# PaddlePaddle/Paddle

Hardware: AMD Instinct MI355X
Metric: tokens/sec (whole node) GPT-3-6.7B Fleet sharding-3 (higher is better)
Workload: dtype bf16; 1 GPU; model=gpt3-6.7b, global_batch=12, seq_len=2048, parallelism=sharding3_dp1

## Files before the change

csrc/bindings.cpp:

```cpp
#include <torch/extension.h>
#include <c10/hip/HIPStream.h>

#include "kernels/api.h"

namespace pa {
void mfma_probe(const void* a, const void* bt, float* c, hipStream_t s);
void mfma_probe32(const void* a, const void* bt, float* c, hipStream_t s);
void mfma_probe_fp8mx(const void* a, const void* bt, float* c, int sa, int sb,
                      hipStream_t s);
}

namespace pa_lt {
std::tuple<torch::Tensor, torch::Tensor> fc1_gelu_fwd(
    const torch::Tensor& x, const torch::Tensor& w, const torch::Tensor& bias);
std::tuple<torch::Tensor, torch::Tensor> fc2_dgrad_dgelu(
    const torch::Tensor& dy, const torch::Tensor& w2, const torch::Tensor& z);
int64_t lt_epilogue_probe(int64_t m, int64_t n, int64_t k, int64_t epi);
}

namespace {

using torch::Tensor;

hipStream_t cur_stream() {
  return (hipStream_t)c10::hip::getCurrentHIPStream().stream();
}

int dt_of(const Tensor& t) {
  switch (t.scalar_type()) {
    case torch::kBFloat16: return pa::kBF16;
    case torch::kFloat: return pa::kF32;
    default: TORCH_CHECK(false, "unsupported dtype ", t.scalar_type(),
                         " (native kernels take bfloat16 or float32)");
  }
  return -1;
}

#define CHECK_IN(t) \
  TORCH_CHECK(t.is_cuda() && t.is_contiguous(), #t " must be contiguous GPU tensor")

#define CHECK_LIKE(t, x)                                                      \
  TORCH_CHECK(t.is_cuda() && t.is_contiguous() &&                             \
              t.scalar_type() == x.scalar_type(),                             \
              #t " must be a contiguous GPU tensor with the dtype of " #x)
#define CHECK_SAME(t, x)                                                      \
  do { CHECK_LIKE(t, x);                                                      \
       TORCH_CHECK(t.numel() == x.numel(), #t " must have the size of " #x);  \
  } while (0)
#define CHECK_VEC(t, x, d)                                                    \
  do { CHECK_LIKE(t, x);                                                      \
       TORCH_CHECK(t.numel() == (d), #t " must have ", (d), " elements");     \
  } while (0)
#define CHECK_STAT(t, n)                                                      \
  TORCH_CHECK(t.is_cuda() && t.is_contiguous() &&                             \
              t.scalar_type() == torch::kFloat && t.numel() == (n),           \
              #t " must be a contiguous fp32 GPU tensor with ", (n), " elements")

static void check_rows(const Tensor& x, const char* op) {
  TORCH_CHECK(x.dim() >= 1 && x.numel() > 0, op, ": empty input");
  TORCH_CHECK(x.size(-1) % 8 == 0, op, ": D must be a multiple of 8");
}

std::vector<Tensor> layer_norm_fwd(const Tensor& x, const Tensor& w,
                                   const c10::optional<Tensor>& b, double eps) {
  CHECK_IN(x);
  check_rows(x, "layer_norm");
  int64_t d = x.size(-1), n = x.numel() / d;
  CHECK_VEC(w, x, d);
  if (b.has_value()) CHECK_VEC((*b), x, d);
  auto y = torch::empty_like(x);
  auto mean = torch::empty({n}, x.options().dtype(torch::kFloat));
  auto rstd = torch::empty({n}, x.options().dtype(torch::kFloat));
  pa::layer_norm_fwd(x.const_data_ptr(), w.const_data_ptr(),
                     b.has_value() ? b->const_data_ptr() : nullptr,
                     y.mutable_data_ptr(), mean.mutable_data_ptr<float>(),
                     rstd.mutable_data_ptr<float>(), n, d, (float)eps, dt_of(x),
                     cur_stream());
  return {y, mean, rstd};
}

std::vector<Tensor> layer_norm_bwd(const Tensor& dy, const Tensor& x,
                                   const Tensor& w, const Tensor& mean,
                                   const Tensor& rstd, bool has_bias) {
  CHECK_IN(x);
  check_rows(x, "layer_norm_bwd");
  int64_t d = x.size(-1), n = x.numel() / d;
  CHECK_SAME(dy, x); CHECK_VEC(w, x, d);
  CHECK_STAT(mean, n); CHECK_STAT(rstd, n);
  auto dx = torch::empty_like(x);
  auto dw = torch::zeros({d}, x.options().dtype(torch::kFloat));
  auto db = torch::zeros({d}, x.options().dtype(torch::kFloat));
  pa::layer_norm_bwd_dx(dy.const_data_ptr(), x.const_data_ptr(), w.const_data_ptr(),
                        mean.const_data_ptr<float>(), rstd.const_data_ptr<float>(),
                        dx.mutable_data_ptr(), n, d, dt_of(x), cur_stream());
  auto ws = torch::empty({(int64_t)2 * pa::ln_dwdb_chunks(n, d) * d},
                         x.options().dtype(torch::kFloat));
  pa::layer_norm_bwd_dwdb(dy.const_data_ptr(), x.const_data_ptr(),
                          mean.const_data_ptr<float>(), rstd.const_data_ptr<float>(),
                          dw.mutable_data_ptr<float>(), db.mutable_data_ptr<float>(),
                          n, d, dt_of(x), cur_stream(), ws.mutable_data_ptr<float>());
  return {dx, dw, db};
}

std::vector<Tensor> rms_norm_fwd(const Tensor& x, const c10::optional<Tensor>& residual,
                                 const Tensor& w, double eps) {
  CHECK_IN(x);
  check_rows(x, "rms_norm");
  int64_t d = x.size(-1), n = x.numel() / d;
  CHECK_VEC(w, x, d);
  auto y = torch::empty_like(x);
  auto rstd = torch::empty({n}, x.options().dtype(torch::kFloat));
  Tensor res_out;
  const void* resp = nullptr;
  void* res_outp = nullptr;
  if (residual.has_value()) {
    CHECK_SAME((*residual), x);
    res_out = torch::empty_like(x);
    resp = residual->const_data_ptr();
    res_outp = res_out.mutable_data_ptr();
  }
  pa::rms_norm_fwd(x.const_data_ptr(), resp, w.const_data_ptr(),
                   y.mutable_data_ptr(), res_outp, rstd.mutable_data_ptr<float>(),
                   n, d, (float)eps, dt_of(x), cur_stream());
  if (residual.has_value()) return {y, rstd, res_out};
  return {y, rstd};
}

std::vector<Tensor> rms_norm_bwd(const Tensor& dy, const Tensor& x, const Tensor& w,
                                 const Tensor& rstd) {
  CHECK_IN(x);
  check_rows(x, "rms_norm_bwd");
  int64_t d = x.size(-1), n = x.numel() / d;
  CHECK_SAME(dy, x); CHECK_VEC(w, x, d); CHECK_STAT(rstd, n);
  auto dx = torch::empty_like(x);
  auto dw = torch::zeros({d}, x.options().dtype(torch::kFloat));
  pa::rms_norm_bwd_dx(dy.const_data_ptr(), x.const_data_ptr(), w.const_data_ptr(),
                      rstd.const_data_ptr<float>(), dx.mutable_data_ptr(), n, d,
                      dt_of(x), cur_stream());
  auto ws = torch::empty({(int64_t)2 * pa::ln_dwdb_chunks(n, d) * d},
                         x.options().dtype(torch::kFloat));
  pa::rms_norm_bwd_dw(dy.const_data_ptr(), x.const_data_ptr(),
                      rstd.const_data_ptr<float>(), dw.mutable_data_ptr<float>(),
                      n, d, dt_of(x), cur_stream(), ws.mutable_data_ptr<float>());
  return {dx, dw};
}

std::vector<Tensor> softmax_ce_fwd(const Tensor& logits, const Tensor& labels,
                                   int64_t ignore_index) {
  CHECK_IN(logits); CHECK_IN(labels);
  TORCH_CHECK(logits.dim() >= 1 && logits.numel() > 0, "softmax_ce: empty logits");
  int64_t v = logits.size(-1), n = logits.numel() / v;
  TORCH_CHECK(labels.scalar_type() == torch::kLong && labels.numel() == n,
              "softmax_ce: labels must be int64 with one entry per row");
  auto loss = torch::empty({n}, logits.options().dtype(torch::kFloat));
  auto lse = torch::empty({n}, logits.options().dtype(torch::kFloat));
  pa::softmax_ce_fwd(logits.const_data_ptr(), labels.const_data_ptr<int64_t>(),
                     loss.mutable_data_ptr<float>(), lse.mutable_data_ptr<float>(),
                     n, v, ignore_index, dt_of(logits), cur_stream());
  return {loss, lse};
}

Tensor softmax_ce_bwd(const Tensor& dloss, const Tensor& logits,
                      const Tensor& labels, const Tensor& lse, int64_t ignore_index) {
  CHECK_IN(logits); CHECK_IN(labels);
  TORCH_CHECK(logits.dim() >= 1 && logits.numel() > 0, "softmax_ce_bwd: empty logits");
  int64_t v = logits.size(-1), n = logits.numel() / v;
  TORCH_CHECK(labels.scalar_type() == torch::kLong && labels.numel() == n,
              "softmax_ce_bwd: labels must be int64 with one entry per row");
  CHECK_STAT(dloss, n); CHECK_STAT(lse, n);
  auto dlogits = torch::empty_like(logits);
  pa::softmax_ce_bwd(dloss.const_data_ptr<float>(), logits.const_data_ptr(),
                     labels.const_data_ptr<int64_t>(), lse.const_data_ptr<float>(),
                     dlogits.mutable_data_ptr(), n, v, ignore_index, dt_of(logits),
                     cur_stream());
  return dlogits;
}

Tensor bias_gelu_fwd(const Tensor& x, const c10::optional<Tensor>& bias) {
  CHECK_IN(x);
  check_rows(x, "bias_gelu");
  int64_t d = x.size(-1), n = x.numel() / d;
  if (bias.has_value()) CHECK_VEC((*bias), x, d);
  auto y = torch::empty_like(x);
  pa::bias_gelu_fwd(x.const_data_ptr(), bias.has_value() ? bias->const_data_ptr() : nullptr,
                    y.mutable_data_ptr(), n, d, dt_of(x), cur_stream());
  return y;
}

Tensor bias_gelu_bwd(const Tensor& dy, const Tensor& x, const c10::optional<Tensor>& bias) {
  CHECK_IN(x);
  check_rows(x, "bias_gelu_bwd");
  int64_t d = x.size(-1), n = x.numel() / d;
  CHECK_SAME(dy, x);
  if (bias.has_value()) CHECK_VEC((*bias), x, d);
  auto dx = torch::empty_like(x);
  pa::bias_gelu_bwd(dy.const_data_ptr(), x.const_data_ptr(),
                    bias.has_value() ? bias->const_data_ptr() : nullptr,
                    dx.mutable_data_ptr(), n, d, dt_of(x), cur_stream());
  return dx;
}

Tensor swiglu_fwd(const Tensor& x) {
  CHECK_IN(x);
  TORCH_CHECK(x.dim() >= 1 && x.numel() > 0, "swiglu: empty input");
  int64_t d2 = x.size(-1), n = x.numel() / d2, d = d2 / 2;
  TORCH_CHECK(d2 % 16 == 0, "swiglu: last dim must be a multiple of 16");
  auto sizes = x.sizes().vec();
  sizes.back() = d;
  auto y = torch::empty(sizes, x.options());
  pa::swiglu_fwd(x.const_data_ptr(), y.mutable_data_ptr(), n, d, dt_of(x), cur_stream());
  return y;
}

Tensor swiglu_bwd(const Tensor& dy, const Tensor& x) {
  CHECK_IN(x);
  TORCH_CHECK(x.dim() >= 1 && x.numel() > 0, "swiglu_bwd: empty input");
  int64_t d2 = x.size(-1), n = x.numel() / d2, d = d2 / 2;
  TORCH_CHECK(d2 % 16 == 0, "swiglu_bwd: last dim must be a multiple of 16");
  CHECK_LIKE(dy, x);
  TORCH_CHECK(dy.numel() == n * d, "swiglu_bwd: dy must have half the size of x");
  auto dx = torch::empty_like(x);
  pa::swiglu_bwd(dy.const_data_ptr(), x.const_data_ptr(), dx.mutable_data_ptr(),
                 n, d, dt_of(x), cur_stream());
  return dx;
}

Tensor rope_fwd(const Tensor& x, const Tensor& cos_t, const Tensor& sin_t,
                int64_t pos_offset, bool conj) {
  CHECK_IN(x); CHECK_IN(cos_t); CHECK_IN(sin_t);
  TORCH_CHECK(x.dim() == 4, "rope expects [B,S,H,D]");
  int64_t b = x.size(0), sl = x.size(1), h = x.size(2), dh = x.size(3);
  TORCH_CHECK(dh % 2 == 0 && (dh / 2) % 4 == 0 && x.numel() > 0,
              "rope: head_dim/2 must be multiple of 4");
  TORCH_CHECK(pos_offset >= 0, "rope: pos_offset must be >= 0");
  TORCH_CHECK(cos_t.scalar_type() == torch::kFloat &&
              sin_t.scalar_type() == torch::kFloat &&
              cos_t.dim() == 2 && sin_t.dim() == 2 &&
              cos_t.size(1) == dh / 2 && sin_t.size(1) == dh / 2 &&
              cos_t.size(0) >= sl + pos_offset && sin_t.size(0) >= sl + pos_offset,
              "rope: cos/sin must be fp32 [>= seq_len + pos_offset, head_dim/2]");
  auto y = torch::empty_like(x);
  pa::rope_fwd(x.const_data_ptr(), cos_t.const_data_ptr<float>(),
               sin_t.const_data_ptr<float>(), y.mutable_data_ptr(), b, sl, h, dh,
               pos_offset, conj, dt_of(x), cur_stream());
  return y;
}

Tensor colsum(const Tensor& x) {
  CHECK_IN(x);
  TORCH_CHECK(x.dim() >= 1 && x.numel() > 0, "colsum: empty input");
  int64_t d = x.size(-1), n = x.numel() / d;
  auto out = torch::zeros({d}, x.options().dtype(torch::kFloat));
  pa::colsum(x.const_data_ptr(), out.mutable_data_ptr<float>(), n, d, dt_of(x),
             cur_stream());
  return out;
}

Tensor weight_only_gemv(const Tensor& x, const Tensor& qweight,
                        const Tensor& scale, const c10::optional<Tensor>& bias) {
  CHECK_IN(x); CHECK_IN(qweight); CHECK_IN(scale);
  TORCH_CHECK(qweight.scalar_type() == torch::kChar, "qweight must be int8");
  int64_t k = x.size(-1), m = x.numel() / k, n = qweight.size(0);
  TORCH_CHECK(qweight.size(1) == k && k % 8 == 0);
  auto sizes = x.sizes().vec();
  sizes.back() = n;
  auto out = torch::empty(sizes, x.options());
  const void* bp = bias.has_value() ? bias->const_data_ptr() : nullptr;
  pa::weight_only_gemv(x.const_data_ptr(), qweight.const_data_ptr(),
                       scale.const_data_ptr<float>(), bp,
                       out.mutable_data_ptr(), m, n, k, dt_of(x), cur_stream());
  return out;
}

void adamw(Tensor& master, c10::optional<Tensor> param_out, const Tensor& grad,
           Tensor& m, Tensor& v, double lr, double beta1, double beta2,
           double eps, double wd, double beta1_pow, double beta2_pow,
           double grad_scale) {
  CHECK_IN(master); CHECK_IN(grad); CHECK_IN(m); CHECK_IN(v);
  int64_t numel = master.numel();
  TORCH_CHECK(master.scalar_type() == torch::kFloat &&
              m.scalar_type() == torch::kFloat && v.scalar_type() == torch::kFloat,
              "adamw: master, m and v must be fp32");
  TORCH_CHECK(grad.numel() == numel && m.numel() == numel && v.numel() == numel,
              "adamw: grad, m and v must have the size of master");
  bool bf16out = false;
  void* pout = nullptr;
  if (param_out.has_value()) {
    TORCH_CHECK(param_out->is_cuda() && param_out->is_contiguous() &&
                param_out->numel() == numel &&
                (param_out->scalar_type() == torch::kBFloat16 ||
                 param_out->scalar_type() == torch::kFloat),
                "adamw: param_out must be a contiguous bf16 or fp32 GPU tensor "
                "with the size of master");
    bf16out = param_out->scalar_type() == torch::kBFloat16;
    pout = param_out->mutable_data_ptr();
  }
  pa::adamw(master.mutable_data_ptr<float>(), pout, grad.const_data_ptr(),
            m.mutable_data_ptr<float>(), v.mutable_data_ptr<float>(), numel,
            (float)lr, (float)beta1, (float)beta2, (float)eps, (float)wd,
            (float)beta1_pow, (float)beta2_pow, (float)grad_scale,
            dt_of(grad), bf16out, cur_stream());
}

Tensor l2norm_sq(const Tensor& x) {
  CHECK_IN(x);
  auto out = torch::zeros({1}, x.options().dtype(torch::kFloat));
  pa::l2norm_sq(x.const_data_ptr(), out.mutable_data_ptr<float>(), x.numel(),
                dt_of(x), cur_stream());
  return out;
}

static void fa_strides(const Tensor& t, int64_t* out) {
  TORCH_CHECK(t.stride(3) == 1, "flash_attn: head_dim must be contiguous");
  out[0] = t.stride(0);
  out[1] = t.stride(1);
  out[2] = t.stride(2);
  TORCH_CHECK(out[2] % 8 == 0, "flash_attn: seq stride must keep 16B alignment");
}

static void fa_mask_strides(const Tensor& m, int64_t b, int64_t h, int64_t sq,
                            int64_t skv, int64_t* ms) {
  TORCH_CHECK(m.dim() == 4 && m.size(3) == skv && m.size(2) == sq &&
              (m.size(1) == 1 || m.size(1) == h) &&
              (m.size(0) == 1 || m.size(0) == b),
              "flash_attn mask must be [B|1, H|1, Sq, Skv]");
  TORCH_CHECK(m.stride(3) == 1 && m.scalar_type() == torch::kBFloat16,
              "flash_attn mask: bf16 with contiguous last dim");
  ms[0] = m.size(0) == 1 ? 0 : m.stride(0);
  ms[1] = m.size(1) == 1 ? 0 : m.stride(1);
  ms[2] = m.stride(2);
}

std::vector<Tensor> flash_attn_fwd(const Tensor& q, const Tensor& k, const Tensor& v,
                                   c10::optional<Tensor> o_out,
                                   double scale, bool causal,
                                   c10::optional<Tensor> mask,
                                   double pdrop, int64_t seed, int64_t offset) {
  TORCH_CHECK(q.is_cuda() && q.scalar_type() == torch::kBFloat16, "flash_attn: bf16 GPU only");
  TORCH_CHECK(q.dim() == 4, "flash_attn expects [B,H,S,D]");
  int64_t b = q.size(0), h = q.size(1), sq = q.size(2), d = q.size(3);
  int64_t hkv = k.size(1), skv = k.size(2);
  TORCH_CHECK(d == 128 || d == 64, "flash_attn: head_dim must be 64/128");
  TORCH_CHECK(h % hkv == 0);
  int64_t qs[3], ks[3], vs[3], os[3];
  fa_strides(q, qs); fa_strides(k, ks); fa_strides(v, vs);
  TORCH_CHECK(ks[0] == vs[0] && ks[1] == vs[1] && ks[2] == vs[2],
              "flash_attn: k/v must share strides");
  auto o = o_out.has_value() ? *o_out : torch::empty({b, h, sq, d}, q.options());
  fa_strides(o, os);
  auto lse = torch::empty({b, h, sq}, q.options().dtype(torch::kFloat));
  int64_t ms[3] = {0, 0, 0};
  const void* mp = nullptr;
  if (mask.has_value()) {
    fa_mask_strides(*mask, b, h, sq, skv, ms);
    mp = mask->const_data_ptr();
  }
  pa::flash_attn_fwd32(q.const_data_ptr(), k.const_data_ptr(), v.const_data_ptr(),
                       o.mutable_data_ptr(), lse.mutable_data_ptr<float>(), b, h,
                       hkv, sq, skv, d, (float)scale, causal, qs, ks, os,
                       mp, ms, (float)pdrop, (uint64_t)seed, (uint64_t)offset,
                       cur_stream());
  return {o, lse};
}

std::vector<Tensor> flash_attn_bwd(const Tensor& dout, const Tensor& q, const Tensor& k,
                                   const Tensor& v, const Tensor& o, const Tensor& lse,
                                   c10::optional<Tensor> dq_out,
                                   c10::optional<Tensor> dk_out,
                                   c10::optional<Tensor> dv_out,
                                   double scale, bool causal,
                                   c10::optional<Tensor> mask,
                                   double pdrop, int64_t seed, int64_t offset) {
  int64_t b = q.size(0), h = q.size(1), sq = q.size(2), d = q.size(3);
  int64_t hkv = k.size(1), skv = k.size(2);
  TORCH_CHECK(hkv == h, "flash_attn_bwd kernel requires hkv==h (expand KV upstream)");
  auto dq = dq_out.has_value() ? *dq_out : torch::empty({b, h, sq, d}, q.options());
  auto dk = dk_out.has_value() ? *dk_out : torch::empty({b, hkv, skv, d}, k.options());
  auto dv = dv_out.has_value() ? *dv_out : torch::empty({b, hkv, skv, d}, v.options());
  auto delta = torch::empty({b, h, sq}, q.options().dtype(torch::kFloat));
  int64_t qs[3], ks[3], vs[3], dos[3], os[3], dqs[3], dks[3], dvs[3];
  fa_strides(q, qs); fa_strides(k, ks); fa_strides(v, vs);
  fa_strides(dout, dos); fa_strides(o, os);
  fa_strides(dq, dqs); fa_strides(dk, dks); fa_strides(dv, dvs);
  TORCH_CHECK(ks[0] == vs[0] && ks[1] == vs[1] && ks[2] == vs[2]);
  TORCH_CHECK(dks[0] == dvs[0] && dks[1] == dvs[1] && dks[2] == dvs[2],
              "dk/dv must share strides");
  int64_t ms[3] = {0, 0, 0};
  const void* mp = nullptr;
  if (mask.has_value()) {
    fa_mask_strides(*mask, b, h, sq, skv, ms);
    mp = mask->const_data_ptr();
  }
  pa::flash_attn_bwd(dout.const_data_ptr(), q.const_data_ptr(), k.const_data_ptr(),
                     v.const_data_ptr(), o.const_data_ptr(), lse.const_data_ptr<float>(),
                     dq.mutable_data_ptr(), dk.mutable_data_ptr(), dv.mutable_data_ptr(),
                     delta.mutable_data_ptr<float>(), b, h, hkv, sq, skv, d,
                     (float)scale, causal, qs, ks, dos, os, dqs, dks,
                     mp, ms, (float)pdrop, (uint64_t)seed, (uint64_t)offset,
                     cur_stream());
  return {dq, dk, dv};
}

static std::pair<Tensor, int64_t> make_bmap(const Tensor& cu_cpu, int64_t blk) {
  auto acc = cu_cpu.accessor<int, 1>();
  std::vector<int> map;
  for (int64_t i = 0; i + 1 < cu_cpu.size(0); ++i) {
    int len = acc[i + 1] - acc[i];
    for (int off = 0; off < len; off += (int)blk) {
      map.push_back((int)i);
      map.push_back(off);
    }
  }
  auto t = torch::from_blob(map.data(), {(int64_t)map.size()},
                            torch::dtype(torch::kInt32)).clone().cuda();
  return {t, (int64_t)map.size() / 2};
}

std::vector<Tensor> flash_attn_varlen_fwd(const Tensor& q, const Tensor& k,
                                          const Tensor& v, const Tensor& cu_q,
                                          const Tensor& cu_k, double scale,
                                          bool causal, double pdrop,
                                          int64_t seed, int64_t offset) {
  TORCH_CHECK(q.is_cuda() && q.scalar_type() == torch::kBFloat16 &&
              q.dim() == 3 && q.is_contiguous(), "varlen q: [total, H, D] bf16");
  TORCH_CHECK(cu_q.scalar_type() == torch::kInt32 && cu_k.scalar_type() == torch::kInt32);
  int64_t tq = q.size(0), h = q.size(1), d = q.size(2);
  int64_t tk = k.size(0), hkv = k.size(1);
  TORCH_CHECK(d == 128 || d == 64);
  auto cu_q_cpu = cu_q.cpu().contiguous();
  auto cu_k_cpu = cu_k.cpu().contiguous();
  auto cu_q_gpu = cu_q.is_cuda() ? cu_q.contiguous() : cu_q_cpu.cuda();
  auto cu_k_gpu = cu_k.is_cuda() ? cu_k.contiguous() : cu_k_cpu.cuda();
  auto [bmap, nblk] = make_bmap(cu_q_cpu, 128);
  auto o = torch::empty_like(q);
  auto lse = torch::empty({h, tq}, q.options().dtype(torch::kFloat));
  pa::flash_attn_varlen_fwd32(q.const_data_ptr(), k.const_data_ptr(),
                              v.const_data_ptr(), o.mutable_data_ptr(),
                              lse.mutable_data_ptr<float>(), h, hkv, tq, tk, d,
                              (float)scale, causal, nblk,
                              cu_q_gpu.const_data_ptr<int>(),
                              cu_k_gpu.const_data_ptr<int>(),
                              bmap.const_data_ptr<int>(), (float)pdrop,
                              (uint64_t)seed, (uint64_t)offset, cur_stream());
  return {o, lse};
}

std::vector<Tensor> flash_attn_varlen_bwd(const Tensor& dout, const Tensor& q,
                                          const Tensor& k, const Tensor& v,
                                          const Tensor& o, const Tensor& lse,
                                          const Tensor& cu_q, const Tensor& cu_k,
                                          double scale, bool causal,
                                          double pdrop, int64_t seed,
                                          int64_t offset) {
  int64_t tq = q.size(0), h = q.size(1), d = q.size(2);
  int64_t tk = k.size(0);
  TORCH_CHECK(k.size(1) == h, "varlen bwd requires hkv == h");
  auto cu_q_cpu = cu_q.cpu().contiguous();
  auto cu_k_cpu = cu_k.cpu().contiguous();
  auto cu_q_gpu = cu_q.is_cuda() ? cu_q.contiguous() : cu_q_cpu.cuda();
  auto cu_k_gpu = cu_k.is_cuda() ? cu_k.contiguous() : cu_k_cpu.cuda();
  auto [qbmap, nqb] = make_bmap(cu_q_cpu, 128);
  auto [kvbmap, nkb] = make_bmap(cu_k_cpu, 128);
  auto dq = torch::empty_like(q);
  auto dk = torch::empty_like(k);
  auto dv = torch::empty_like(v);
  auto delta = torch::empty({h, tq}, q.options().dtype(torch::kFloat));
  pa::flash_attn_varlen_bwd(dout.contiguous().const_data_ptr(), q.const_data_ptr(),
                            k.const_data_ptr(), v.const_data_ptr(),
                            o.const_data_ptr(), lse.const_data_ptr<float>(),
                            dq.mutable_data_ptr(), dk.mutable_data_ptr(),
                            dv.mutable_data_ptr(), delta.mutable_data_ptr<float>(),
                            h, tq, tk, d, (float)scale, causal, nqb, nkb,
                            cu_q_gpu.const_data_ptr<int>(),
                            cu_k_gpu.const_data_ptr<int>(),
                            qbmap.const_data_ptr<int>(),
                            kvbmap.const_data_ptr<int>(), (float)pdrop,
                            (uint64_t)seed, (uint64_t)offset, cur_stream());
  return {dq, dk, dv};
}

Tensor fa_dropout_mask(int64_t b, int64_t h, int64_t sq, int64_t skv,
                       double p, int64_t seed, int64_t offset) {
  auto out = torch::empty({b, h, sq, skv},
                          torch::dtype(torch::kUInt8).device(torch::kCUDA));
  pa::fa_dropout_mask(out.mutable_data_ptr(), out.numel(), (float)p,
                      (uint64_t)seed, (uint64_t)offset, cur_stream());
  return out;
}

std::vector<Tensor> dropout_add_fwd(const Tensor& x, const c10::optional<Tensor>& residual,
                                    double p, int64_t seed, int64_t offset) {
  CHECK_IN(x);
  TORCH_CHECK(x.numel() > 0 && x.numel() % 8 == 0,
              "dropout_add: numel must be a multiple of 8");
  TORCH_CHECK(p >= 0.0 && p < 1.0, "dropout_add: p must be in [0, 1)");
  if (residual.has_value()) CHECK_SAME((*residual), x);
  auto y = torch::empty_like(x);
  Tensor mask;
  uint8_t* maskp = nullptr;
  if (p > 0) {
    mask = torch::empty(x.sizes(), x.options().dtype(torch::kUInt8));
    maskp = mask.mutable_data_ptr<uint8_t>();
  }
  pa::dropout_add_fwd(x.const_data_ptr(),
                      residual.has_value() ? residual->const_data_ptr() : nullptr,
                      y.mutable_data_ptr(), maskp, x.numel(), (float)p,
                      (uint64_t)seed, (uint64_t)offset, dt_of(x), cur_stream());
  if (p > 0) return {y, mask};
  return {y};
}

Tensor dropout_add_bwd(const Tensor& dy, const Tensor& mask, double p) {
  CHECK_IN(dy); CHECK_IN(mask);
  TORCH_CHECK(dy.numel() > 0 && dy.numel() % 8 == 0,
              "dropout_add_bwd: numel must be a multiple of 8");
  TORCH_CHECK(mask.scalar_type() == torch::kUInt8 && mask.numel() == dy.numel(),
              "dropout_add_bwd: mask must be uint8 with the size of dy");
  TORCH_CHECK(p >= 0.0 && p < 1.0, "dropout_add_bwd: p must be in [0, 1)");
  auto dx = torch::empty_like(dy);
  pa::dropout_add_bwd(dy.const_data_ptr(), mask.const_data_ptr<uint8_t>(),
                      dx.mutable_data_ptr(), dy.numel(), (float)p, dt_of(dy),
                      cur_stream());
  return dx;
}

Tensor embedding_fwd(const Tensor& table, const Tensor& ids_in, int64_t padding_idx) {
  CHECK_IN(table);
  TORCH_CHECK(ids_in.is_cuda(), "ids must be on GPU");
  TORCH_CHECK(ids_in.scalar_type() == torch::kLong, "embedding: ids must be int64");
  TORCH_CHECK(table.dim() == 2 && table.numel() > 0, "embedding: table must be [vocab, D]");
  auto ids = ids_in.contiguous();
  int64_t vocab = table.size(0), d = table.size(1), n = ids.numel();
  TORCH_CHECK(d % 8 == 0, "embedding: D must be a multiple of 8");
  auto sizes = ids.sizes().vec();
  sizes.push_back(d);
  auto out = torch::empty(sizes, table.options());
  pa::embedding_fwd(table.const_data_ptr(), ids.const_data_ptr<int64_t>(),
                    out.mutable_data_ptr(), n, d, vocab, padding_idx,
                    dt_of(table), cur_stream());
  return out;
}

Tensor embedding_bwd(const Tensor& dout, const Tensor& ids_in, int64_t vocab,
                     int64_t padding_idx) {
  CHECK_IN(dout);
  TORCH_CHECK(ids_in.is_cuda(), "ids must be on GPU");
  TORCH_CHECK(ids_in.scalar_type() == torch::kLong, "embedding_bwd: ids must be int64");
  auto ids = ids_in.contiguous();
  TORCH_CHECK(dout.dim() >= 1 && dout.numel() > 0 && vocab > 0, "embedding_bwd: empty input");
  int64_t d = dout.size(-1), n = ids.numel();
  TORCH_CHECK(d % 8 == 0, "embedding_bwd: D must be a multiple of 8");
  TORCH_CHECK(dout.numel() == n * d, "embedding_bwd: dout must be [ids..., D]");
  auto dtable = torch::zeros({vocab, d}, dout.options().dtype(torch::kFloat));
  pa::embedding_bwd(dout.const_data_ptr(), ids.const_data_ptr<int64_t>(),
                    dtable.mutable_data_ptr<float>(), n, d, vocab, padding_idx,
                    dt_of(dout), cur_stream());
  return dtable;
}

Tensor decode_attention(const Tensor& q, const Tensor& kcache, const Tensor& vcache,
                        const Tensor& block_table, const Tensor& seq_lens,
                        double scale, int64_t blk_str, int64_t pos_str,
                        int64_t head_str, int64_t bs_override) {
  CHECK_IN(q); CHECK_IN(kcache); CHECK_IN(vcache);
  TORCH_CHECK(q.dim() == 3, "q: [B, H, D] (one decode step)");
  int64_t b = q.size(0), h = q.size(1), d = q.size(2);
  int64_t bs, hkv;
  if (blk_str == 0) {
    TORCH_CHECK(kcache.dim() == 4, "k_cache: [nblocks, block_size, HKV, D]");
    bs = kcache.size(1); hkv = kcache.size(2);
  } else {
    bs = bs_override; hkv = bs_override >= 0 ? h : h;
    hkv = kcache.size(1) == h ? h : kcache.size(1);
  }
  int64_t max_blocks = block_table.size(1);
  auto o = torch::empty_like(q);
  pa::decode_attention(q.const_data_ptr(), kcache.const_data_ptr(),
                       vcache.const_data_ptr(),
                       block_table.const_data_ptr<int>(),
                       seq_lens.const_data_ptr<int>(), o.mutable_data_ptr(),
                       b, h, hkv, bs, max_blocks, d, (float)scale,
                       blk_str, pos_str, head_str, cur_stream());
  return o;
}

Tensor gemm_bf16(const Tensor& a, const Tensor& b, bool b_is_nt) {
  TORCH_CHECK(a.is_cuda() && a.scalar_type() == torch::kBFloat16);
  TORCH_CHECK(a.dim() == 2 && b.dim() == 2);
  TORCH_CHECK(a.stride(1) == 1 && b.stride(1) == 1, "row-major inputs only");
  int64_t m = a.size(0), k = a.size(1);
  int64_t n = b_is_nt ? b.size(0) : b.size(1);
  TORCH_CHECK(b_is_nt ? b.size(1) == k : b.size(0) == k);
  TORCH_CHECK(k % 64 == 0 && k >= 128, "gemm_bf16: K must be multiple of 64");
  auto c = torch::empty({m, n}, a.options());
  pa::gemm_bf16(a.const_data_ptr(), b.const_data_ptr(), c.mutable_data_ptr(),
                m, n, k, a.stride(0), b.stride(0), c.stride(0), b_is_nt,
                cur_stream());
  return c;
}

std::vector<Tensor> gemm_bf16_ex(const Tensor& a, const Tensor& b,
                                 int64_t layout, int64_t epilogue,
                                 const c10::optional<Tensor>& bias,
                                 const c10::optional<Tensor>& aux_in,
                                 const c10::optional<Tensor>& c_in) {
  TORCH_CHECK(a.is_cuda() && a.scalar_type() == torch::kBFloat16);
  TORCH_CHECK(b.is_cuda() && b.scalar_type() == torch::kBFloat16);
  TORCH_CHECK(a.dim() == 2 && b.dim() == 2);
  TORCH_CHECK(a.stride(1) == 1 && b.stride(1) == 1, "row-major inputs only");
  int64_t m, n, k;
  if (layout == 0) {
    m = a.size(0); k = a.size(1); n = b.size(0);
    TORCH_CHECK(b.size(1) == k, "gemm NT: inner dims mismatch");
  } else if (layout == 1) {
    m = a.size(0); k = a.size(1); n = b.size(1);
    TORCH_CHECK(b.size(0) == k, "gemm NN: inner dims mismatch");
  } else {
    k = a.size(0); m = a.size(1); n = b.size(1);
    TORCH_CHECK(b.size(0) == k, "gemm TN: inner dims mismatch");
  }
  TORCH_CHECK(k >= 64, "gemm_bf16_ex: K must be >= 64");
  bool accumulate = c_in.has_value();
  Tensor c;
  if (accumulate) {
    c = c_in.value();
    TORCH_CHECK(c.size(0) == m && c.size(1) == n && c.stride(1) == 1 &&
                c.scalar_type() == torch::kBFloat16);
    TORCH_CHECK(epilogue == 0, "accumulate requires epilogue=none");
  } else {
    c = torch::empty({m, n}, a.options());
  }
  const void* bias_p = nullptr;
  if (epilogue == 1 || epilogue == 2) {
    TORCH_CHECK(bias.has_value() && bias->numel() == n &&
                bias->scalar_type() == torch::kBFloat16 && bias->is_contiguous());
    bias_p = bias->const_data_ptr();
  }
  Tensor aux;
  void* aux_p = nullptr;
  if (epilogue == 2) {
    aux = torch::empty({m, n}, a.options());
    aux_p = aux.mutable_data_ptr();
  } else if (epilogue == 3) {
    TORCH_CHECK(aux_in.has_value() && aux_in->size(0) == m &&
                aux_in->size(1) == n && aux_in->stride(1) == 1 &&
                aux_in->scalar_type() == torch::kBFloat16);
    aux_p = const_cast<void*>(aux_in->const_data_ptr());
  }
  pa::gemm_bf16_ex(a.const_data_ptr(), b.const_data_ptr(), c.mutable_data_ptr(),
                   bias_p, aux_p, m, n, k, a.stride(0), b.stride(0), c.stride(0),
                   (int)layout, (int)epilogue, accumulate, cur_stream());
  if (epilogue == 2) return {c, aux};
  return {c};
}

Tensor gemm_fp8_nt(const Tensor& a, const Tensor& bt, double scale_ab,
                   const c10::optional<Tensor>& bias) {
  TORCH_CHECK(a.is_cuda() && a.dim() == 2 && bt.dim() == 2);
  TORCH_CHECK(a.scalar_type() == torch::kFloat8_e4m3fn ||
              a.scalar_type() == torch::kUInt8, "gemm_fp8: e4m3/uint8 input");
  TORCH_CHECK(a.stride(1) == 1 && bt.stride(1) == 1, "row-major inputs");
  int64_t m = a.size(0), k = a.size(1), n = bt.size(0);
  TORCH_CHECK(bt.size(1) == k && k >= 128);
  auto c = torch::empty({m, n}, a.options().dtype(torch::kBFloat16));
  const void* bp = nullptr;
  if (bias.has_value()) {
    TORCH_CHECK(bias->scalar_type() == torch::kBFloat16 && bias->numel() == n);
    bp = bias->const_data_ptr();
  }
  pa::gemm_fp8_nt(a.const_data_ptr(), bt.const_data_ptr(), c.mutable_data_ptr(),
                  bp, (float)scale_ab, m, n, k, a.stride(0), bt.stride(0),
                  c.stride(0), cur_stream());
  return c;
}

Tensor decode_gemm(const Tensor& x, const Tensor& w,
                   const c10::optional<Tensor>& bias) {
  CHECK_IN(x);
  TORCH_CHECK(x.dim() == 2 && w.dim() == 2 && w.stride(1) == 1);
  TORCH_CHECK(x.scalar_type() == torch::kBFloat16);
  int64_t m = x.size(0), k = x.size(1), n = w.size(1);
  TORCH_CHECK(w.size(0) == k && m <= 32);
  int64_t ntiles = (n + 1023) / 1024;
  int64_t ksplit = std::min<int64_t>(std::max<int64_t>(1, 768 / std::max<int64_t>(ntiles, 1)),
                                     std::max<int64_t>(1, k / 128));
  int64_t mt = m <= 8 ? 8 : (m <= 16 ? 16 : 32);
  auto ws = torch::empty({ksplit, mt, n}, x.options().dtype(torch::kFloat));
  auto y = torch::empty({m, n}, x.options());
  pa::decode_gemm(x.const_data_ptr(), w.const_data_ptr(),
                  bias.has_value() ? bias->const_data_ptr() : nullptr,
                  y.mutable_data_ptr(), ws.mutable_data_ptr<float>(), m, n, k,
                  w.stride(0), ksplit, cur_stream());
  return y;
}

Tensor decode_gemm_int8(const Tensor& x, const Tensor& qw,
                        const Tensor& scale,
                        const c10::optional<Tensor>& bias) {
  CHECK_IN(x);
  TORCH_CHECK(x.dim() == 2 && qw.dim() == 2 && qw.is_contiguous());
  TORCH_CHECK(x.scalar_type() == torch::kBFloat16 &&
              qw.scalar_type() == torch::kChar &&
              scale.scalar_type() == torch::kFloat);
  int64_t m = x.size(0), k = x.size(1), n = qw.size(1);
  TORCH_CHECK(qw.size(0) == k && m <= 32 && n % 256 == 0 && k % 64 == 0);
  TORCH_CHECK(scale.numel() == n);
  int64_t nblk = n / 256;
  int64_t kmin = nblk <= 24 ? 256 : 512;
  int64_t ksplit = std::min<int64_t>(std::max<int64_t>(1, 1024 / nblk),
                                     std::max<int64_t>(1, k / kmin));
  int64_t mt = m <= 16 ? 16 : 32;
  auto ws = torch::empty({ksplit, mt, n}, x.options().dtype(torch::kFloat));
  auto y = torch::empty({m, n}, x.options());
  pa::decode_gemm_mfma(x.const_data_ptr(), qw.const_data_ptr(),
                       bias.has_value() ? bias->const_data_ptr() : nullptr,
                       y.mutable_data_ptr(), ws.mutable_data_ptr<float>(), m,
                       n, k, n, ksplit, cur_stream(),
                       scale.const_data_ptr<float>(), true);
  return y;
}

static int64_t check_int4_weight(const Tensor& qw, const Tensor& scale,
                                 int64_t group_size, const char* op) {
  TORCH_CHECK(qw.is_cuda() && scale.is_cuda(), op, ": qw and scale must be GPU tensors");
  TORCH_CHECK(qw.dim() == 2 && qw.is_contiguous(), op,
              ": qw must be a contiguous [K/2, N] tensor");
  TORCH_CHECK(qw.scalar_type() == torch::kChar, op, ": qw must be int8");
  TORCH_CHECK(scale.scalar_type() == torch::kFloat && scale.is_contiguous(),
              op, ": scale must be contiguous fp32");
  TORCH_CHECK(group_size == -1 || group_size == 64 || group_size == 128, op,
              ": group_size must be -1, 64 or 128, got ", group_size);
  const int64_t k = qw.size(0) * 2, n = qw.size(1);
  if (group_size == -1) {
    TORCH_CHECK(scale.dim() == 1 && scale.size(0) == n, op,
                ": per-channel scale must be [N]");
  } else {
    TORCH_CHECK(k % group_size == 0, op, ": K must be a multiple of group_size");
    TORCH_CHECK(scale.dim() == 2 && scale.size(0) == k / group_size &&
                scale.size(1) == n, op, ": group scale must be [K/group_size, N]");
  }
  return k;
}

Tensor decode_gemm_int4(const Tensor& x, const Tensor& qw, const Tensor& scale,
                        const c10::optional<Tensor>& bias, int64_t group_size,
                        int64_t ksplit) {
  CHECK_IN(x);
  TORCH_CHECK(x.dim() == 2 && x.scalar_type() == torch::kBFloat16,
              "decode_gemm_int4: x must be a 2-D bf16 tensor");
  const int64_t k = check_int4_weight(qw, scale, group_size, "decode_gemm_int4");
  const int64_t m = x.size(0), n = qw.size(1);
  TORCH_CHECK(x.size(1) == k, "decode_gemm_int4: qw.size(0)*2 must equal K");
  TORCH_CHECK(m >= 1 && m <= 32, "decode_gemm_int4: 1 <= M <= 32, got ", m);
  TORCH_CHECK(n > 0 && n % 256 == 0, "decode_gemm_int4: N % 256 == 0, got ", n);
  TORCH_CHECK(k > 0 && k % 64 == 0 && k <= (int64_t(1) << 24),
              "decode_gemm_int4: K % 64 == 0 (and K <= 2^24), got ", k);
  TORCH_CHECK(ksplit >= 0, "decode_gemm_int4: ksplit >= 0");
  const void* bp = nullptr;
  if (bias.has_value()) {
    TORCH_CHECK(bias->is_cuda() && bias->is_contiguous() &&
                bias->scalar_type() == torch::kBFloat16 && bias->numel() == n,
                "decode_gemm_int4: bias must be contiguous bf16 with N elements");
    bp = bias->const_data_ptr();
  }
  if (ksplit == 0) {
    const int64_t nblk = n / 256;
    const int64_t kmin = nblk <= 24 ? 256 : 512;
    ksplit = std::min<int64_t>(std::max<int64_t>(1, 1024 / nblk),
                               std::max<int64_t>(1, k / kmin));
  }
  const int64_t ks = pa::decode_gemm_int4_splits(k, ksplit);
  const int64_t mt = m <= 16 ? 16 : 32;
  auto ws = torch::empty({ks, mt, n}, x.options().dtype(torch::kFloat));
  auto y = torch::empty({m, n}, x.options());
  pa::decode_gemm_int4(x.const_data_ptr(), qw.const_data_ptr(),
                       scale.const_data_ptr<float>(), bp, y.mutable_data_ptr(),
                       ws.mutable_data_ptr<float>(), m, n, k, group_size,
                       ksplit, cur_stream());
  return y;
}

Tensor dequant_int4(const Tensor& qw, const Tensor& scale, int64_t group_size,
                    at::ScalarType out_dtype) {
  const int64_t k = check_int4_weight(qw, scale, group_size, "dequant_int4");
  const int64_t n = qw.size(1);
  TORCH_CHECK(n % 8 == 0, "dequant_int4: N % 8 == 0, got ", n);
  TORCH_CHECK(out_dtype == torch::kBFloat16 || out_dtype == torch::kFloat,
              "dequant_int4: out_dtype must be bfloat16 or float32");
  auto out = torch::empty({k, n}, qw.options().dtype(out_dtype));
  pa::dequant_int4(qw.const_data_ptr(), scale.const_data_ptr<float>(),
                   out.mutable_data_ptr(), k, n, group_size,
                   out_dtype == torch::kBFloat16 ? pa::kBF16 : pa::kF32,
                   cur_stream());
  return out;
}

Tensor decode_gemm_mfma(const Tensor& x, const Tensor& w,
                        const c10::optional<Tensor>& bias) {
  CHECK_IN(x);
  TORCH_CHECK(x.dim() == 2 && w.dim() == 2 && w.stride(1) == 1);
  TORCH_CHECK(x.scalar_type() == torch::kBFloat16);
  int64_t m = x.size(0), k = x.size(1), n = w.size(1);
  TORCH_CHECK(w.size(0) == k && m <= 32 && n % 256 == 0 && k % 64 == 0);
  int64_t nblk = n / 256;
  int64_t kmin = nblk <= 24 ? 256 : 512;
  int64_t ksplit = std::min<int64_t>(std::max<int64_t>(1, 1024 / nblk),
                                     std::max<int64_t>(1, k / kmin));
  int64_t mt = m <= 16 ? 16 : 32;
  auto ws = torch::empty({ksplit, mt, n}, x.options().dtype(torch::kFloat));
  auto y = torch::empty({m, n}, x.options());
  pa::decode_gemm_mfma(x.const_data_ptr(), w.const_data_ptr(),
                       bias.has_value() ? bias->const_data_ptr() : nullptr,
                       y.mutable_data_ptr(), ws.mutable_data_ptr<float>(), m,
                       n, k, w.stride(0), ksplit, cur_stream());
  return y;
}

std::vector<Tensor> moe_gate_topk(const Tensor& logits, int64_t k) {
  CHECK_IN(logits);
  TORCH_CHECK(logits.scalar_type() == torch::kFloat && logits.dim() == 2);
  int64_t t = logits.size(0), e = logits.size(1);
  TORCH_CHECK(e <= 64 && k <= 4);
  auto topv = torch::empty({t, k}, logits.options());
  auto topi = torch::empty({t, k}, logits.options().dtype(torch::kInt32));
  auto me = torch::zeros({e}, logits.options());
  auto ce = torch::zeros({e}, logits.options());
  pa::moe_gate_topk(logits.const_data_ptr<float>(), topv.mutable_data_ptr<float>(),
                    topi.mutable_data_ptr<int>(), me.mutable_data_ptr<float>(),
                    ce.mutable_data_ptr<float>(), t, e, k, cur_stream());
  return {topv, topi, me, ce};
}

std::vector<Tensor> moe_assign_slots(const Tensor& topi, int64_t num_experts,
                                     int64_t cap) {
  CHECK_IN(topi);
  TORCH_CHECK(topi.scalar_type() == torch::kInt32 && topi.dim() == 2);
  int64_t t = topi.size(0), k = topi.size(1);
  auto slot = torch::full({t, k}, -1, topi.options());
  auto counts = torch::zeros({num_experts}, topi.options());
  pa::moe_assign_slots(topi.const_data_ptr<int>(), slot.mutable_data_ptr<int>(),
                       counts.mutable_data_ptr<int>(), t, num_experts, k, cap,
                       cur_stream());
  return {slot, counts};
}

Tensor gemm_fp8_nt_batched(const Tensor& a, const Tensor& bt, double scale_ab,
                           const c10::optional<Tensor>& bias) {
  TORCH_CHECK(a.is_cuda() && a.dim() == 3 && bt.dim() == 3);
  TORCH_CHECK(a.is_contiguous() && bt.is_contiguous());
  int64_t e = a.size(0), m = a.size(1), k = a.size(2), n = bt.size(1);
  TORCH_CHECK(bt.size(0) == e && bt.size(2) == k && k >= 128);
  const void* bp = nullptr;
  int64_t bias_bs = 0;
  if (bias.has_value()) {
    TORCH_CHECK(bias->is_contiguous() && bias->scalar_type() == torch::kBFloat16);
    TORCH_CHECK(bias->dim() == 2 && bias->size(0) == e && bias->size(1) == n);
    bp = bias->const_data_ptr();
    bias_bs = n;
  }
  auto c = torch::empty({e, m, n}, a.options().dtype(torch::kBFloat16));
  pa::gemm_fp8_nt_batched(a.const_data_ptr(), bt.const_data_ptr(),
                          c.mutable_data_ptr(), bp, (float)scale_ab, e,
                          m, n, k, k, k, n, m * k, n * k, m * n, cur_stream(),
                          bias_bs);
  return c;
}

Tensor amax_abs(const Tensor& x) {
  CHECK_IN(x);
  auto out = torch::zeros({}, x.options().dtype(torch::kFloat));
  pa::amax_abs(x.const_data_ptr(), out.mutable_data_ptr<float>(), x.numel(),
               dt_of(x), cur_stream());
  return out;
}

Tensor gemm_bf16_8p_t(const Tensor& a, const Tensor& bt) {
  TORCH_CHECK(a.is_cuda() && a.dim() == 2 && bt.dim() == 2);
  TORCH_CHECK(a.is_contiguous() && bt.is_contiguous());
  int64_t m = a.size(0), k = a.size(1), n = bt.size(0);
  TORCH_CHECK(bt.size(1) == k && m % 256 == 0 && n % 256 == 0 && k % 32 == 0);
  auto c = torch::empty({m, n}, a.options());
  pa::gemm_bf16_8p(a.const_data_ptr(), bt.const_data_ptr(),
                   c.mutable_data_ptr(), m, n, k, k, k, n, cur_stream());
  return c;
}

Tensor gemm_bf16_nt_batched_t(const Tensor& a, const Tensor& bt) {
  TORCH_CHECK(a.is_cuda() && a.dim() == 3 && bt.dim() == 3);
  TORCH_CHECK(a.scalar_type() == torch::kBFloat16 &&
              bt.scalar_type() == torch::kBFloat16);
  TORCH_CHECK(a.is_contiguous() && bt.is_contiguous());
  int64_t e = a.size(0), m = a.size(1), k = a.size(2), n = bt.size(1);
  TORCH_CHECK(bt.size(0) == e && bt.size(2) == k && k % 8 == 0 && n % 8 == 0);
  auto c = torch::empty({e, m, n}, a.options());
  pa::gemm_bf16_nt_batched(a.const_data_ptr(), bt.const_data_ptr(),
                           c.mutable_data_ptr(), e, m, n, k, k, k, n,
                           m * k, n * k, m * n, cur_stream());
  return c;
}

Tensor quant_fp8(const Tensor& x, double scale) {
  CHECK_IN(x);
  TORCH_CHECK(x.scalar_type() == torch::kBFloat16 && x.numel() % 8 == 0);
  auto out = torch::empty(x.sizes(), x.options().dtype(torch::kFloat8_e4m3fn));
  pa::quant_fp8(x.const_data_ptr(), out.mutable_data_ptr(), (float)scale,
                x.numel(), cur_stream());
  return out;
}

Tensor mfma_probe_fp8mx(const Tensor& a, const Tensor& bt, int64_t sa, int64_t sb) {
  CHECK_IN(a); CHECK_IN(bt);
  TORCH_CHECK(a.scalar_type() == torch::kUInt8 && a.numel() == 16 * 128);
  auto c = torch::empty({16, 16}, a.options().dtype(torch::kFloat));
  pa::mfma_probe_fp8mx(a.const_data_ptr(), bt.const_data_ptr(),
                       c.mutable_data_ptr<float>(), (int)sa, (int)sb,
                       cur_stream());
  return c;
}

Tensor mfma_probe(const Tensor& a, const Tensor& bt) {
  CHECK_IN(a); CHECK_IN(bt);
  auto c = torch::empty({16, 16}, a.options().dtype(torch::kFloat));
  pa::mfma_probe(a.const_data_ptr(), bt.const_data_ptr(),
                 c.mutable_data_ptr<float>(), cur_stream());
  return c;
}

Tensor mfma_probe32(const Tensor& a, const Tensor& bt) {
  CHECK_IN(a); CHECK_IN(bt);
  auto c = torch::empty({32, 32}, a.options().dtype(torch::kFloat));
  pa::mfma_probe32(a.const_data_ptr(), bt.const_data_ptr(),
                   c.mutable_data_ptr<float>(), cur_stream());
  return c;
}

}

PYBIND11_MODULE(TORCH_EXTENSION_NAME, m) {
  m.def("layer_norm_fwd", &layer_norm_fwd);
  m.def("layer_norm_bwd", &layer_norm_bwd);
  m.def("rms_norm_fwd", &rms_norm_fwd);
  m.def("rms_norm_bwd", &rms_norm_bwd);
  m.def("softmax_ce_fwd", &softmax_ce_fwd);
  m.def("softmax_ce_bwd", &softmax_ce_bwd);
  m.def("bias_gelu_fwd", &bias_gelu_fwd);
  m.def("bias_gelu_bwd", &bias_gelu_bwd);
  m.def("swiglu_fwd", &swiglu_fwd);
  m.def("swiglu_bwd", &swiglu_bwd);
  m.def("rope_fwd", &rope_fwd);
  m.def("colsum", &colsum);
  m.def("adamw", &adamw);
  m.def("fc1_gelu_fwd", &pa_lt::fc1_gelu_fwd);
  m.def("fc2_dgrad_dgelu", &pa_lt::fc2_dgrad_dgelu);
  m.def("lt_epilogue_probe", &pa_lt::lt_epilogue_probe);
  m.def("weight_only_gemv", &weight_only_gemv);
  m.def("l2norm_sq", &l2norm_sq);
  m.def("flash_attn_fwd", &flash_attn_fwd, py::arg("q"), py::arg("k"),
        py::arg("v"), py::arg("o") = c10::nullopt, py::arg("scale"),
        py::arg("causal"), py::arg("mask") = c10::nullopt,
        py::arg("pdrop") = 0.0, py::arg("seed") = 0, py::arg("offset") = 0);
  m.def("fa_dropout_mask", &fa_dropout_mask);
  m.def("mfma_probe_fp8mx", &mfma_probe_fp8mx);
  m.def("decode_gemm", &decode_gemm, py::arg("x"), py::arg("w"),
        py::arg("bias") = c10::nullopt);
  m.def("decode_gemm_mfma", &decode_gemm_mfma, py::arg("x"), py::arg("w"),
        py::arg("bias") = c10::nullopt);
  m.def("decode_gemm_int8", &decode_gemm_int8, py::arg("x"), py::arg("qw"),
        py::arg("scale"), py::arg("bias") = c10::nullopt);
  m.def("decode_gemm_int4", &decode_gemm_int4, py::arg("x"), py::arg("qw"),
        py::arg("scale"), py::arg("bias") = c10::nullopt,
        py::arg("group_size") = -1, py::arg("ksplit") = 0);
  m.def("dequant_int4", &dequant_int4, py::arg("qw"), py::arg("scale"),
        py::arg("group_size"), py::arg("out_dtype"));
  m.def("moe_gate_topk", &moe_gate_topk);
  m.def("moe_assign_slots", &moe_assign_slots);
  m.def("gemm_fp8_nt", &gemm_fp8_nt, py::arg("a"), py::arg("bt"),
        py::arg("scale_ab") = 1.0, py::arg("bias") = c10::nullopt);
  m.def("gemm_fp8_nt_batched", &gemm_fp8_nt_batched, py::arg("a"),
        py::arg("bt"), py::arg("scale_ab"), py::arg("bias") = c10::nullopt);
  m.def("amax_abs", &amax_abs);
  m.def("quant_fp8", &quant_fp8);
  m.def("flash_attn_varlen_fwd", &flash_attn_varlen_fwd, py::arg("q"),
        py::arg("k"), py::arg("v"), py::arg("cu_q"), py::arg("cu_k"),
        py::arg("scale"), py::arg("causal"), py::arg("pdrop") = 0.0,
        py::arg("seed") = 0, py::arg("offset") = 0);
  m.def("flash_attn_varlen_bwd", &flash_attn_varlen_bwd);
  m.def("flash_attn_bwd", &flash_attn_bwd, py::arg("dout"), py::arg("q"),
        py::arg("k"), py::arg("v"), py::arg("o"), py::arg("lse"),
        py::arg("dq") = c10::nullopt, py::arg("dk") = c10::nullopt,
        py::arg("dv") = c10::nullopt, py::arg("scale"), py::arg("causal"),
        py::arg("mask") = c10::nullopt, py::arg("pdrop") = 0.0,
        py::arg("seed") = 0, py::arg("offset") = 0);
  m.def("dropout_add_fwd", &dropout_add_fwd);
  m.def("dropout_add_bwd", &dropout_add_bwd);
  m.def("embedding_fwd", &embedding_fwd);
  m.def("embedding_bwd", &embedding_bwd);
  m.def("gemm_bf16", &gemm_bf16);
  m.def("gemm_bf16_nt_batched", &gemm_bf16_nt_batched_t);
  m.def("gemm_bf16_8p", &gemm_bf16_8p_t);
  m.def("gemm_bf16_ex", &gemm_bf16_ex, py::arg("a"), py::arg("b"),
        py::arg("layout"), py::arg("epilogue") = 0,
        py::arg("bias") = c10::nullopt, py::arg("aux") = c10::nullopt,
        py::arg("c_in") = c10::nullopt);
  m.def("decode_attention", &decode_attention, py::arg("q"), py::arg("kcache"),
        py::arg("vcache"), py::arg("block_table"), py::arg("seq_lens"),
        py::arg("scale"), py::arg("blk_str") = 0, py::arg("pos_str") = 0,
        py::arg("head_str") = 0, py::arg("bs_override") = 0);
  m.def("mfma_probe", &mfma_probe);
  m.def("mfma_probe32", &mfma_probe32);
  m.attr("compiled_arch") = "gfx950";
}
```

csrc/kernels/api.h:

```cpp
#pragma once
#include <hip/hip_runtime.h>
#include <cstdint>

namespace pa {

enum DType : int { kBF16 = 0, kF32 = 1, kF16 = 2 };

void layer_norm_fwd(const void* x, const void* w, const void* b, void* y,
                    float* mean, float* rstd, int64_t n, int64_t d, float eps,
                    int dtype, hipStream_t s);
void layer_norm_bwd_dx(const void* dy, const void* x, const void* w,
                       const float* mean, const float* rstd, void* dx,
                       int64_t n, int64_t d, int dtype, hipStream_t s);
int ln_dwdb_chunks(int64_t n, int64_t d);
void layer_norm_bwd_dwdb(const void* dy, const void* x, const float* mean,
                         const float* rstd, float* dw, float* db, int64_t n,
                         int64_t d, int dtype, hipStream_t s,
                         float* ws = nullptr);

void rms_norm_fwd(const void* x, const void* residual, const void* w, void* y,
                  void* res_out, float* rstd, int64_t n, int64_t d, float eps,
                  int dtype, hipStream_t s);
void rms_norm_bwd_dx(const void* dy, const void* x, const void* w,
                     const float* rstd, void* dx, int64_t n, int64_t d,
                     int dtype, hipStream_t s);
void rms_norm_bwd_dw(const void* dy, const void* x, const float* rstd,
                     float* dw, int64_t n, int64_t d, int dtype, hipStream_t s,
                     float* ws = nullptr);

void softmax_ce_fwd(const void* logits, const int64_t* labels, float* loss,
                    float* lse, int64_t n, int64_t v, int64_t ignore_index,
                    int dtype, hipStream_t s);
void softmax_ce_bwd(const float* dloss, const void* logits,
                    const int64_t* labels, const float* lse, void* dlogits,
                    int64_t n, int64_t v, int64_t ignore_index, int dtype,
                    hipStream_t s);

void bias_gelu_fwd(const void* x, const void* bias, void* y, int64_t n,
                   int64_t d, int dtype, hipStream_t s);
void bias_gelu_bwd(const void* dy, const void* x, const void* bias, void* dx,
                   int64_t n, int64_t d, int dtype, hipStream_t s);

void swiglu_fwd(const void* x, void* y, int64_t n, int64_t d, int dtype,
                hipStream_t s);
void swiglu_bwd(const void* dy, const void* x, void* dx, int64_t n, int64_t d,
                int dtype, hipStream_t s);

void rope_fwd(const void* x, const float* cos_t, const float* sin_t, void* y,
              int64_t b, int64_t sl, int64_t h, int64_t dh, int64_t pos_offset,
              bool conj, int dtype, hipStream_t s);

void amax_abs(const void* x, float* out, int64_t n, int dtype, hipStream_t s);
void colsum(const void* x, float* out, int64_t n, int64_t d, int dtype,
            hipStream_t s);

void adamw(float* master, void* param_bf16, const void* grad, float* m,
           float* v, int64_t numel, float lr, float beta1, float beta2,
           float eps, float wd, float beta1_pow, float beta2_pow,
           float grad_scale, int grad_dtype, bool param_out_bf16, hipStream_t s);

void l2norm_sq(const void* x, float* out, int64_t numel, int dtype,
               hipStream_t s);

void flash_attn_fwd(const void* q, const void* k, const void* v, void* o,
                    float* lse, int64_t b, int64_t h, int64_t hkv, int64_t sq,
                    int64_t skv, int64_t dh, float scale, bool causal,
                    const int64_t* qs, const int64_t* ks, const int64_t* os,
                    hipStream_t s);
void flash_attn_fwd32(const void* q, const void* k, const void* v, void* o,
                      float* lse, int64_t b, int64_t h, int64_t hkv, int64_t sq,
                      int64_t skv, int64_t dh, float scale, bool causal,
                      const int64_t* qs, const int64_t* ks, const int64_t* os,
                      const void* mask, const int64_t* ms, float pdrop,
                      uint64_t seed, uint64_t offset, hipStream_t s);
void flash_attn_bwd_dq32(const void* dout, const void* q, const void* k,
                         const void* v, const float* lse, const float* delta,
                         void* dq, int64_t b, int64_t h, int64_t sq, int64_t skv,
                         int64_t dh, float scale, bool causal,
                         const int64_t* qs, const int64_t* ks, const int64_t* dos,
                         const int64_t* dqs, const void* mask, const int64_t* ms,
                         float pdrop, uint64_t seed, uint64_t offset,
                         hipStream_t s);
void flash_attn_bwd_dkv32(const void* dout, const void* q, const void* k,
                          const void* v, const float* lse, const float* delta,
                          void* dk, void* dv, int64_t b, int64_t h, int64_t sq,
                          int64_t skv, int64_t dh, float scale, bool causal,
                          const int64_t* qs, const int64_t* ks, const int64_t* dos,
                          const int64_t* dks, const void* mask, const int64_t* ms,
                          float pdrop, uint64_t seed, uint64_t offset,
                          hipStream_t s);
void flash_attn_bwd(const void* dout, const void* q, const void* k,
                    const void* v, const void* o, const float* lse,
                    void* dq, void* dk, void* dv, float* delta, int64_t b,
                    int64_t h, int64_t hkv, int64_t sq, int64_t skv,
                    int64_t dh, float scale, bool causal,
                    const int64_t* qs, const int64_t* ks, const int64_t* dos,
                    const int64_t* os, const int64_t* dqs, const int64_t* dks,
                    const void* mask, const int64_t* ms, float pdrop,
                    uint64_t seed, uint64_t offset, hipStream_t s);

void dropout_add_fwd(const void* x, const void* residual, void* y,
                     uint8_t* mask, int64_t numel, float p, uint64_t seed,
                     uint64_t offset, int dtype, hipStream_t s);
void dropout_add_bwd(const void* dy, const uint8_t* mask, void* dx,
                     int64_t numel, float p, int dtype, hipStream_t s);

void embedding_fwd(const void* table, const int64_t* ids, void* out,
                   int64_t n_ids, int64_t d, int64_t vocab, int64_t padding_idx,
                   int dtype, hipStream_t s);
void embedding_bwd(const void* dout, const int64_t* ids, float* dtable,
                   int64_t n_ids, int64_t d, int64_t vocab, int64_t padding_idx,
                   int dtype, hipStream_t s);

void decode_attention(const void* q, const void* kcache, const void* vcache,
                      const int* block_table, const int* seq_lens, void* o,
                      int64_t b, int64_t h, int64_t hkv, int64_t bs,
                      int64_t max_blocks, int64_t dh, float scale,
                      int64_t blk_str, int64_t pos_str, int64_t head_str,
                      hipStream_t s);

void gemm_bf16_8p(const void* a, const void* b, void* c, int64_t m, int64_t n,
                  int64_t k, int64_t lda, int64_t ldb, int64_t ldc,
                  hipStream_t s);
void gemm_bf16_nt_batched(const void* a, const void* b, void* c,
                          int64_t batch, int64_t m, int64_t n, int64_t k,
                          int64_t lda, int64_t ldb, int64_t ldc,
                          int64_t a_bs, int64_t b_bs, int64_t c_bs,
                          hipStream_t s);
void gemm_bf16(const void* a, const void* b, void* c, int64_t m, int64_t n,
               int64_t k, int64_t lda, int64_t ldb, int64_t ldc, bool b_is_nt,
               hipStream_t s);

void gemm_bf16_ex(const void* a, const void* b, void* c, const void* bias,
                  void* aux, int64_t m, int64_t n, int64_t k, int64_t lda,
                  int64_t ldb, int64_t ldc, int layout, int epilogue,
                  bool accumulate, hipStream_t s);

void weight_only_gemv(const void* x, const void* wq, const float* scale,
                      const void* bias, void* out, int64_t m, int64_t n,
                      int64_t k, int dtype, hipStream_t s);

void flash_attn_varlen_fwd32(const void* q, const void* k, const void* v,
                             void* o, float* lse, int64_t h, int64_t hkv,
                             int64_t total_q, int64_t total_k, int64_t dh,
                             float scale, bool causal, int64_t nblocks,
                             const int* cu_q, const int* cu_k, const int* bmap,
                             float pdrop, uint64_t seed, uint64_t offset,
                             hipStream_t s);
void flash_attn_varlen_bwd32(const void* dout, const void* q, const void* k,
                             const void* v, const float* lse, const float* delta,
                             void* dq, void* dk, void* dv, int64_t h,
                             int64_t total_q, int64_t total_k, int64_t dh,
                             float scale, bool causal, int64_t nqblocks,
                             int64_t nkvblocks, const int* cu_q, const int* cu_k,
                             const int* qbmap, const int* kvbmap, float pdrop,
                             uint64_t seed, uint64_t offset, hipStream_t s);
void flash_attn_varlen_bwd(const void* dout, const void* q, const void* k,
                           const void* v, const void* o, const float* lse,
                           void* dq, void* dk, void* dv, float* delta,
                           int64_t h, int64_t total_q, int64_t total_k,
                           int64_t dh, float scale, bool causal,
                           int64_t nqblocks, int64_t nkvblocks,
                           const int* cu_q, const int* cu_k, const int* qbmap,
                           const int* kvbmap, float pdrop, uint64_t seed,
                           uint64_t offset, hipStream_t s);

void fa_dropout_mask(void* out, int64_t total, float p, uint64_t seed,
                     uint64_t offset, hipStream_t s);

void gemm_fp8_nt(const void* a, const void* bt, void* c, const void* bias,
                 float scale_ab, int64_t m, int64_t n, int64_t k, int64_t lda,
                 int64_t ldb, int64_t ldc, hipStream_t s);
void gemm_fp8_nt_batched(const void* a, const void* bt, void* c,
                         const void* bias, float scale_ab, int64_t batch,
                         int64_t m, int64_t n, int64_t k, int64_t lda,
                         int64_t ldb, int64_t ldc, int64_t a_bs, int64_t b_bs,
                         int64_t c_bs, hipStream_t s,
                         int64_t bias_bs = 0);
void quant_fp8(const void* x, void* out, float scale, int64_t numel,
               hipStream_t s);

void decode_gemm(const void* x, const void* w, const void* bias, void* y,
                 float* workspace, int64_t m, int64_t n, int64_t k,
                 int64_t ldw, int64_t ksplit, hipStream_t s);
void decode_gemm_mfma(const void* x, const void* w, const void* bias, void* y,
                 float* workspace, int64_t m, int64_t n, int64_t k,
                 int64_t ldw, int64_t ksplit, hipStream_t s,
                 const float* chscale = nullptr, bool int8w = false);

int64_t decode_gemm_int4_splits(int64_t k, int64_t ksplit);
void decode_gemm_int4(const void* x, const void* qw, const float* scale,
                      const void* bias, void* y, float* workspace, int64_t m,
                      int64_t n, int64_t k, int64_t group_size, int64_t ksplit,
                      hipStream_t s);
void dequant_int4(const void* qw, const float* scale, void* out, int64_t k,
                  int64_t n, int64_t group_size, int dtype, hipStream_t s);

void moe_gate_topk(const float* logits, float* topv, int* topi, float* me,
                   float* ce, int64_t t, int64_t e, int64_t k, hipStream_t s);
void moe_assign_slots(const int* topi, int* slot_of, int* counts, int64_t t,
                      int64_t e, int64_t k, int64_t cap, hipStream_t s);

}
```

csrc/kernels/elementwise.hip:

```cpp
#include "common.h"
#include "api.h"

namespace pa {

template <int DT> struct LS8;
template <> struct LS8<kBF16> {
  static __device__ __forceinline__ void load8(const void* p, int64_t idx, float* f) {
    shortx8 v = *reinterpret_cast<const shortx8*>((const short*)p + idx);
#pragma unroll
    for (int i = 0; i < 8; ++i) f[i] = bf2f(v[i]);
  }
  static __device__ __forceinline__ void store8(void* p, int64_t idx, const float* f) {
    shortx8 v;
#pragma unroll
    for (int i = 0; i < 8; ++i) v[i] = f2bf(f[i]);
    *reinterpret_cast<shortx8*>((short*)p + idx) = v;
  }
};
template <> struct LS8<kF32> {
  static __device__ __forceinline__ void load8(const void* p, int64_t idx, float* f) {
    const float4* q = reinterpret_cast<const float4*>((const float*)p + idx);
    float4 a = q[0], b = q[1];
    f[0]=a.x; f[1]=a.y; f[2]=a.z; f[3]=a.w; f[4]=b.x; f[5]=b.y; f[6]=b.z; f[7]=b.w;
  }
  static __device__ __forceinline__ void store8(void* p, int64_t idx, const float* f) {
    float4* q = reinterpret_cast<float4*>((float*)p + idx);
    q[0] = make_float4(f[0],f[1],f[2],f[3]); q[1] = make_float4(f[4],f[5],f[6],f[7]);
  }
};

__device__ __forceinline__ float erf_fast(float z) {
  float az = fabsf(z);
  float t = 1.f / (1.f + 0.3275911f * az);
  float p = t * (0.254829592f + t * (-0.284496736f + t * (1.421413741f +
            t * (-1.453152027f + t * 1.061405429f))));
  float r = 1.f - p * __expf(-az * az);
  return copysignf(r, z);
}
__device__ __forceinline__ float gelu_f(float x) {
  return 0.5f * x * (1.f + erf_fast(x * 0.70710678118654752440f));
}
__device__ __forceinline__ float gelu_grad_f(float x) {
  const float kInvSqrt2 = 0.70710678118654752440f;
  const float kInvSqrt2Pi = 0.3989422804014327f;
  float cdf = 0.5f * (1.f + erf_fast(x * kInvSqrt2));
  float pdf = kInvSqrt2Pi * __expf(-0.5f * x * x);
  return cdf + x * pdf;
}
__device__ __forceinline__ float silu_f(float x) {
  return x / (1.f + __expf(-x));
}
__device__ __forceinline__ float silu_grad_f(float x) {
  float sig = 1.f / (1.f + __expf(-x));
  return sig * (1.f + x * (1.f - sig));
}

template <int DT, bool FWD, int W>
__global__ void bias_gelu_kernel(const void* __restrict__ a, const void* __restrict__ x,
                                 const void* __restrict__ bias, void* __restrict__ out,
                                 int64_t n, int64_t d) {
  int64_t total = n * d;
  int64_t i0 = ((int64_t)blockIdx.x * blockDim.x + threadIdx.x) * W;
  int64_t stride = (int64_t)gridDim.x * blockDim.x * W;
  int64_t c = i0 % d, cstep = stride % d;
  for (int64_t i = i0; i < total; i += stride, c = (c + cstep >= d ? c + cstep - d : c + cstep)) {
    float xf[W], bf[W], af[W];
#pragma unroll
    for (int v8 = 0; v8 < W / 8; ++v8) {
      LS8<DT>::load8(x, i + 8 * v8, xf + 8 * v8);
      if (bias) LS8<DT>::load8(bias, c + 8 * v8, bf + 8 * v8);
      if (!FWD) LS8<DT>::load8(a, i + 8 * v8, af + 8 * v8);
    }
#pragma unroll
    for (int k = 0; k < W; ++k) {
      float v = xf[k] + (bias ? bf[k] : 0.f);
      xf[k] = FWD ? gelu_f(v) : af[k] * gelu_grad_f(v);
    }
#pragma unroll
    for (int v8 = 0; v8 < W / 8; ++v8)
      LS8<DT>::store8(out, i + 8 * v8, xf + 8 * v8);
  }
}

template <int DT>
__global__ void swiglu_fwd_kernel(const void* __restrict__ x, void* __restrict__ y,
                                  int64_t n, int64_t d) {
  int64_t total = n * d;
  for (int64_t i = ((int64_t)blockIdx.x * blockDim.x + threadIdx.x) * 8; i < total;
       i += (int64_t)gridDim.x * blockDim.x * 8) {
    int64_t row = i / d, col = i % d;
    float g[8], u[8];
    LS8<DT>::load8(x, row * 2 * d + col, g);
    LS8<DT>::load8(x, row * 2 * d + d + col, u);
#pragma unroll
    for (int k = 0; k < 8; ++k) g[k] = silu_f(g[k]) * u[k];
    LS8<DT>::store8(y, i, g);
  }
}

template <int DT>
__global__ void swiglu_bwd_kernel(const void* __restrict__ dy, const void* __restrict__ x,
                                  void* __restrict__ dx, int64_t n, int64_t d) {
  int64_t total = n * d;
  for (int64_t i = ((int64_t)blockIdx.x * blockDim.x + threadIdx.x) * 8; i < total;
       i += (int64_t)gridDim.x * blockDim.x * 8) {
    int64_t row = i / d, col = i % d;
    float g[8], u[8], dyf[8], dg[8];
    LS8<DT>::load8(x, row * 2 * d + col, g);
    LS8<DT>::load8(x, row * 2 * d + d + col, u);
    LS8<DT>::load8(dy, i, dyf);
#pragma unroll
    for (int k = 0; k < 8; ++k) {
      dg[k] = dyf[k] * u[k] * silu_grad_f(g[k]);
      u[k] = dyf[k] * silu_f(g[k]);
    }
    LS8<DT>::store8(dx, row * 2 * d + col, dg);
    LS8<DT>::store8(dx, row * 2 * d + d + col, u);
  }
}

template <int DT>
__global__ void rope_kernel(const void* __restrict__ x, const float* __restrict__ cos_t,
                            const float* __restrict__ sin_t, void* __restrict__ y,
                            int64_t b, int64_t sl, int64_t h, int64_t dh,
                            int64_t pos_offset, float sin_sign) {
  int64_t rows = b * sl * h;
  int64_t wid = ((int64_t)blockIdx.x * blockDim.x + threadIdx.x) >> 6;
  int lane = threadIdx.x & 63;
  int64_t nwaves = ((int64_t)gridDim.x * blockDim.x) >> 6;
  int64_t half = dh / 2;
  for (int64_t r = wid; r < rows; r += nwaves) {
    int64_t srow = (r / h) % sl + pos_offset;
    const int64_t base = r * dh;
    for (int64_t j = lane * 4; j < half; j += 64 * 4) {
      float x1[4], x2[4];
      if (DT == kBF16) {
        shortx4 v1 = *reinterpret_cast<const shortx4*>((const short*)x + base + j);
        shortx4 v2 = *reinterpret_cast<const shortx4*>((const short*)x + base + half + j);
#pragma unroll
        for (int k = 0; k < 4; ++k) { x1[k] = bf2f(v1[k]); x2[k] = bf2f(v2[k]); }
      } else {
        const float* xf = (const float*)x;
#pragma unroll
        for (int k = 0; k < 4; ++k) { x1[k] = xf[base + j + k]; x2[k] = xf[base + half + j + k]; }
      }
      const float4 c = *reinterpret_cast<const float4*>(&cos_t[srow * half + j]);
      const float4 sn = *reinterpret_cast<const float4*>(&sin_t[srow * half + j]);
      float cc[4] = {c.x, c.y, c.z, c.w};
      float ss[4] = {sn.x * sin_sign, sn.y * sin_sign, sn.z * sin_sign, sn.w * sin_sign};
      float y1[4], y2[4];
#pragma unroll
      for (int k = 0; k < 4; ++k) {
        y1[k] = x1[k] * cc[k] - x2[k] * ss[k];
        y2[k] = x2[k] * cc[k] + x1[k] * ss[k];
      }
      if (DT == kBF16) {
        shortx4 o1, o2;
#pragma unroll
        for (int k = 0; k < 4; ++k) { o1[k] = f2bf(y1[k]); o2[k] = f2bf(y2[k]); }
        *reinterpret_cast<shortx4*>((short*)y + base + j) = o1;
        *reinterpret_cast<shortx4*>((short*)y + base + half + j) = o2;
      } else {
        float* yf = (float*)y;
#pragma unroll
        for (int k = 0; k < 4; ++k) { yf[base + j + k] = y1[k]; yf[base + half + j + k] = y2[k]; }
      }
    }
  }
}

template <int DT>
__global__ void colsum_kernel(const void* __restrict__ x, float* __restrict__ out,
                              int64_t n, int64_t d) {
  int64_t c0 = ((int64_t)blockIdx.x * blockDim.x + threadIdx.x) * 8;
  if (c0 >= d) return;
  int64_t rows_per = (n + gridDim.y - 1) / gridDim.y;
  int64_t r0 = (int64_t)blockIdx.y * rows_per, r1 = min(n, r0 + rows_per);
  float acc[8] = {0.f};
  if (c0 + 8 <= d) {
    for (int64_t r = r0; r < r1; ++r) {
      float v[8];
      LS8<DT>::load8(x, r * d + c0, v);
#pragma unroll
      for (int k = 0; k < 8; ++k) acc[k] += v[k];
    }
  } else {
    for (int64_t r = r0; r < r1; ++r)
      for (int64_t c = c0; c < d; ++c)
        acc[c - c0] += (DT == kBF16) ? bf2f(((const short*)x)[r * d + c])
                                     : ((const float*)x)[r * d + c];
  }
#pragma unroll
  for (int k = 0; k < 8; ++k)
    if (c0 + k < d) atomicAdd(&out[c0 + k], acc[k]);
}

__device__ __forceinline__ float rand_uniform(uint64_t seed, uint64_t idx) {
  uint64_t z = seed + idx * 0x9E3779B97F4A7C15ull;
  z = (z ^ (z >> 30)) * 0xBF58476D1CE4E5B9ull;
  z = (z ^ (z >> 27)) * 0x94D049BB133111EBull;
  z = z ^ (z >> 31);
  return (float)(z >> 40) * (1.f / 16777216.f);
}

template <int DT>
__global__ void dropout_add_fwd_kernel(const void* __restrict__ x, const void* __restrict__ res,
                                       void* __restrict__ y, uint8_t* __restrict__ mask,
                                       int64_t numel, float p, uint64_t seed, uint64_t offset) {
  const float scale_ = 1.f / (1.f - p);
  for (int64_t i = ((int64_t)blockIdx.x * blockDim.x + threadIdx.x) * 8; i < numel;
       i += (int64_t)gridDim.x * blockDim.x * 8) {
    float xf[8], rf[8];
    LS8<DT>::load8(x, i, xf);
    if (res) LS8<DT>::load8(res, i, rf);
    uchar2 mk[4];
#pragma unroll
    for (int k = 0; k < 8; ++k) {
      bool keep = p == 0.f || rand_uniform(seed, offset + i + k) >= p;
      ((uint8_t*)mk)[k] = keep;
      xf[k] = (keep ? xf[k] * scale_ : 0.f) + (res ? rf[k] : 0.f);
    }
    if (mask) *reinterpret_cast<uint2*>(mask + i) = *reinterpret_cast<uint2*>(mk);
    LS8<DT>::store8(y, i, xf);
  }
}

template <int DT>
__global__ void dropout_add_bwd_kernel(const void* __restrict__ dy, const uint8_t* __restrict__ mask,
                                       void* __restrict__ dx, int64_t numel, float p) {
  const float scale_ = 1.f / (1.f - p);
  for (int64_t i = ((int64_t)blockIdx.x * blockDim.x + threadIdx.x) * 8; i < numel;
       i += (int64_t)gridDim.x * blockDim.x * 8) {
    float f[8];
    LS8<DT>::load8(dy, i, f);
#pragma unroll
    for (int k = 0; k < 8; ++k) f[k] = mask[i + k] ? f[k] * scale_ : 0.f;
    LS8<DT>::store8(dx, i, f);
  }
}

#define EDT(dtype, KERNEL_CALL_BF16, KERNEL_CALL_F32) \
  if (dtype == kBF16) { KERNEL_CALL_BF16; } else { KERNEL_CALL_F32; }

static dim3 egrid(int64_t numel) {
  return dim3((unsigned)elementwise_grid(cdiv((int)hmin<int64_t>(numel / 8 + 1, 1 << 30), 256)));
}

void bias_gelu_fwd(const void* x, const void* bias, void* y, int64_t n,
                   int64_t d, int dtype, hipStream_t s) {
  if (d % 16 == 0) {
    dim3 g = egrid(n * d / 2);
    EDT(dtype,
        hipLaunchKernelGGL((bias_gelu_kernel<kBF16, true, 16>), g, dim3(256), 0, s, x, x, bias, y, n, d),
        hipLaunchKernelGGL((bias_gelu_kernel<kF32, true, 16>), g, dim3(256), 0, s, x, x, bias, y, n, d));
  } else {
    dim3 g = egrid(n * d);
    EDT(dtype,
        hipLaunchKernelGGL((bias_gelu_kernel<kBF16, true, 8>), g, dim3(256), 0, s, x, x, bias, y, n, d),
        hipLaunchKernelGGL((bias_gelu_kernel<kF32, true, 8>), g, dim3(256), 0, s, x, x, bias, y, n, d));
  }
}

void bias_gelu_bwd(const void* dy, const void* x, const void* bias, void* dx,
                   int64_t n, int64_t d, int dtype, hipStream_t s) {
  if (d % 16 == 0) {
    dim3 g = egrid(n * d / 2);
    EDT(dtype,
        hipLaunchKernelGGL((bias_gelu_kernel<kBF16, false, 16>), g, dim3(256), 0, s, dy, x, bias, dx, n, d),
        hipLaunchKernelGGL((bias_gelu_kernel<kF32, false, 16>), g, dim3(256), 0, s, dy, x, bias, dx, n, d));
  } else {
    dim3 g = egrid(n * d);
    EDT(dtype,
        hipLaunchKernelGGL((bias_gelu_kernel<kBF16, false, 8>), g, dim3(256), 0, s, dy, x, bias, dx, n, d),
        hipLaunchKernelGGL((bias_gelu_kernel<kF32, false, 8>), g, dim3(256), 0, s, dy, x, bias, dx, n, d));
  }
}

void swiglu_fwd(const void* x, void* y, int64_t n, int64_t d, int dtype, hipStream_t s) {
  dim3 g = egrid(n * d);
  EDT(dtype,
      hipLaunchKernelGGL((swiglu_fwd_kernel<kBF16>), g, dim3(256), 0, s, x, y, n, d),
      hipLaunchKernelGGL((swiglu_fwd_kernel<kF32>), g, dim3(256), 0, s, x, y, n, d));
}

void swiglu_bwd(const void* dy, const void* x, void* dx, int64_t n, int64_t d,
                int dtype, hipStream_t s) {
  dim3 g = egrid(n * d);
  EDT(dtype,
      hipLaunchKernelGGL((swiglu_bwd_kernel<kBF16>), g, dim3(256), 0, s, dy, x, dx, n, d),
      hipLaunchKernelGGL((swiglu_bwd_kernel<kF32>), g, dim3(256), 0, s, dy, x, dx, n, d));
}

void rope_fwd(const void* x, const float* cos_t, const float* sin_t, void* y,
              int64_t b, int64_t sl, int64_t h, int64_t dh, int64_t pos_offset,
              bool conj, int dtype, hipStream_t s) {
  int64_t rows = b * sl * h;
  dim3 g((unsigned)hmin<int64_t>(cdiv((int)hmin<int64_t>(rows, 1 << 24), 4), 2048));
  float ssign = conj ? -1.f : 1.f;
  EDT(dtype,
      hipLaunchKernelGGL((rope_kernel<kBF16>), g, dim3(256), 0, s, x, cos_t, sin_t, y, b, sl, h, dh, pos_offset, ssign),
      hipLaunchKernelGGL((rope_kernel<kF32>), g, dim3(256), 0, s, x, cos_t, sin_t, y, b, sl, h, dh, pos_offset, ssign));
}

void colsum(const void* x, float* out, int64_t n, int64_t d, int dtype, hipStream_t s) {
  int xblocks = cdiv((int)d, 256 * 8);
  int chunks = (int)hmin<int64_t>(hmax<int64_t>(1, n / 32),
                                  hmax<int64_t>(1, 2048 / xblocks));
  dim3 grid((unsigned)xblocks, chunks);
  EDT(dtype,
      hipLaunchKernelGGL((colsum_kernel<kBF16>), grid, dim3(256), 0, s, x, out, n, d),
      hipLaunchKernelGGL((colsum_kernel<kF32>), grid, dim3(256), 0, s, x, out, n, d));
}

void dropout_add_fwd(const void* x, const void* residual, void* y,
                     uint8_t* mask, int64_t numel, float p, uint64_t seed,
                     uint64_t offset, int dtype, hipStream_t s) {
  dim3 g = egrid(numel);
  EDT(dtype,
      hipLaunchKernelGGL((dropout_add_fwd_kernel<kBF16>), g, dim3(256), 0, s, x, residual, y, mask, numel, p, seed, offset),
      hipLaunchKernelGGL((dropout_add_fwd_kernel<kF32>), g, dim3(256), 0, s, x, residual, y, mask, numel, p, seed, offset));
}

void dropout_add_bwd(const void* dy, const uint8_t* mask, void* dx,
                     int64_t numel, float p, int dtype, hipStream_t s) {
  dim3 g = egrid(numel);
  EDT(dtype,
      hipLaunchKernelGGL((dropout_add_bwd_kernel<kBF16>), g, dim3(256), 0, s, dy, mask, dx, numel, p),
      hipLaunchKernelGGL((dropout_add_bwd_kernel<kF32>), g, dim3(256), 0, s, dy, mask, dx, numel, p));
}

}

namespace pa {
template <int DT>
__global__ void amax_abs_kernel(const void* __restrict__ x, float* __restrict__ out,
                                int64_t n) {
  float m = 0.f;
  int64_t i0 = ((int64_t)blockIdx.x * blockDim.x + threadIdx.x) * 8;
  int64_t stride = (int64_t)gridDim.x * blockDim.x * 8;
  for (int64_t i = i0; i + 8 <= n; i += stride) {
    float v[8];
    LS8<DT>::load8(x, i, v);
#pragma unroll
    for (int k = 0; k < 8; ++k) m = fmaxf(m, fabsf(v[k]));
  }
  int64_t tail = n & ~7ll;
  if (i0 == 0)
    for (int64_t i = tail; i < n; ++i)
      m = fmaxf(m, fabsf(DT == kBF16
          ? bf2f(reinterpret_cast<const short*>(x)[i])
          : reinterpret_cast<const float*>(x)[i]));
#pragma unroll
  for (int off = 32; off; off >>= 1) m = fmaxf(m, __shfl_xor(m, off, 64));
  if ((threadIdx.x & 63) == 0)
    atomicMax(reinterpret_cast<int*>(out), __float_as_int(m));
}

void amax_abs(const void* x, float* out, int64_t n, int dtype, hipStream_t s) {
  int64_t waves = (n + 8 * 256 - 1) / (8 * 256);
  unsigned g = (unsigned)hmin<int64_t>(hmax<int64_t>(waves, 1), 4096);
  EDT(dtype,
      hipLaunchKernelGGL((amax_abs_kernel<kBF16>), dim3(g), dim3(256), 0, s, x, out, n),
      hipLaunchKernelGGL((amax_abs_kernel<kF32>), dim3(g), dim3(256), 0, s, x, out, n));
}
}
```

csrc/kernels/flash_attn.hip:

```cpp
#include "common.h"
#include "api.h"

namespace pa {

#define LGKM0() asm volatile("s_waitcnt lgkmcnt(0)" ::: "memory")

__device__ __forceinline__ unsigned lds_off(unsigned row, unsigned col_bytes,
                                            unsigned row_stride) {
  return row * row_stride + (col_bytes ^ ((row & 7u) << 4));
}

__device__ __forceinline__ shortx8 lds_read8(const char* lds, unsigned row,
                                             unsigned col_elem, unsigned row_stride) {
  return *reinterpret_cast<const shortx8*>(lds + lds_off(row, col_elem * 2, row_stride));
}

template <int D, bool CAUSAL>
__launch_bounds__(512)
__global__ void fa_fwd_kernel(const short* __restrict__ qg, const short* __restrict__ kg,
                              const short* __restrict__ vg, short* __restrict__ og,
                              float* __restrict__ lseg, int B, int H, int HKV,
                              int Sq, int Skv, float scale,
                              long long q_sb, long long q_sh, long long q_ss,
                              long long k_sb, long long k_sh, long long k_ss,
                              long long o_sb, long long o_sh, long long o_ss) {
  constexpr int NW = 8;
  constexpr int QB = 16 * NW, KB = 64;
  constexpr int NT = NW * 64;
  constexpr int NKK = D / 32;
  constexpr int NDT = D / 16;
  constexpr unsigned K_RS = D * 2;
  constexpr unsigned VT_RS = KB * 2;
  __shared__ char k_lds[KB * D * 2];
  __shared__ char vt_lds[D * KB * 2];
  __shared__ char p_lds[NW * 16 * KB * 2];

  const int qblk = blockIdx.x;
  const int bh = blockIdx.y;
  const int b = bh / H, h = bh % H;
  const int hkv = h / (H / HKV);
  const int q0 = qblk * QB;
  const long long qbase = (long long)b * q_sb + (long long)h * q_sh;
  const long long kbase = (long long)b * k_sb + (long long)hkv * k_sh;
  const long long obase = (long long)b * o_sb + (long long)h * o_sh;

  const int tid = threadIdx.x;
  const int lane = tid & 63;
  const int wq = tid >> 6;
  const int l16 = lane & 15;
  const int lg = lane >> 4;

  shortx8 qf[NKK];
  {
    int row = q0 + wq * 16 + l16;
    bool ok = row < Sq;
#pragma unroll
    for (int kk = 0; kk < NKK; ++kk) {
      if (ok)
        qf[kk] = *reinterpret_cast<const shortx8*>(qg + qbase + (long long)row * q_ss + kk * 32 + lg * 8);
      else
        for (int i = 0; i < 8; ++i) qf[kk][i] = 0;
    }
  }

  floatx4 oacc[NDT];
#pragma unroll
  for (int dt = 0; dt < NDT; ++dt) oacc[dt] = {0.f, 0.f, 0.f, 0.f};
  float m_run[4], l_run[4];
#pragma unroll
  for (int r = 0; r < 4; ++r) { m_run[r] = -INFINITY; l_run[r] = 0.f; }

  const int kv_end = CAUSAL ? min(Skv, q0 + QB) : Skv;

  int k_row[KB * D / (NT * 8)], k_colp[KB * D / (NT * 8)];
#pragma unroll
  for (int it = 0; it < KB * D / (NT * 8); ++it) {
    int flat = it * NT * 8 + tid * 8;
    int row = flat / D, col = flat % D;
    k_row[it] = row;
    k_colp[it] = col ^ ((row & 7) << 3);
  }

  for (int kv0 = 0; kv0 < kv_end; kv0 += KB) {
    if (kv0 + KB <= Skv) {
#pragma unroll
      for (int it = 0; it < KB * D / (NT * 8); ++it) {
        const short* src = kg + kbase + (long long)(kv0 + k_row[it]) * k_ss + k_colp[it];
        char* dst = k_lds + it * NT * 16 + (tid >> 6) * 64 * 16;
        __builtin_amdgcn_global_load_lds((const __attribute__((address_space(1))) unsigned int*)src,
                                         (__attribute__((address_space(3))) unsigned int*)dst,
                                         16, 0, 0);
      }
    } else {
      constexpr int elems = KB * D;
      for (int flat = tid * 8; flat < elems; flat += NT * 8) {
        int row = flat / D, col = flat % D;
        shortx8 val;
        if (kv0 + row < Skv)
          val = *reinterpret_cast<const shortx8*>(kg + kbase + (long long)(kv0 + row) * k_ss + col);
        else
          for (int i = 0; i < 8; ++i) val[i] = 0;
        *reinterpret_cast<shortx8*>(k_lds + lds_off(row, col * 2, K_RS)) = val;
      }
    }
    {
      constexpr int elems = KB * D;
      for (int flat = tid * 8; flat < elems; flat += NT * 8) {
        int row = flat / D, col = flat % D;
        shortx8 val;
        if (kv0 + row < Skv)
          val = *reinterpret_cast<const shortx8*>(vg + kbase + (long long)(kv0 + row) * k_ss + col);
        else
          for (int i = 0; i < 8; ++i) val[i] = 0;
        const int rot = threadIdx.x & 7;
#pragma unroll
        for (int j = 0; j < 8; ++j) {
          int i = (j + rot) & 7;
          *reinterpret_cast<short*>(vt_lds + lds_off(col + i, row * 2, VT_RS)) = val[i];
        }
      }
    }
    __syncthreads();

    floatx4 sacc[4];
#pragma unroll
    for (int nt = 0; nt < 4; ++nt) {
      sacc[nt] = {0.f, 0.f, 0.f, 0.f};
#pragma unroll
      for (int kk = 0; kk < NKK; ++kk) {
        shortx8 kf = lds_read8(k_lds, nt * 16 + l16, kk * 32 + lg * 8, K_RS);
        sacc[nt] = mfma_bf16(qf[kk], kf, sacc[nt]);
      }
    }

    const int q_abs = q0 + wq * 16 + lg * 4;
    const bool boundary = (kv0 + KB > Skv) || (CAUSAL && kv0 + KB > q_abs);
    float mx[4] = {-INFINITY, -INFINITY, -INFINITY, -INFINITY};
    if (boundary) {
#pragma unroll
      for (int nt = 0; nt < 4; ++nt) {
        const int kv_abs = kv0 + nt * 16 + l16;
#pragma unroll
        for (int r = 0; r < 4; ++r) {
          float val = sacc[nt][r] * scale;
          if (kv_abs >= Skv || (CAUSAL && kv_abs > q_abs + r)) val = -INFINITY;
          sacc[nt][r] = val;
          mx[r] = fmaxf(mx[r], val);
        }
      }
    } else {
#pragma unroll
      for (int nt = 0; nt < 4; ++nt)
#pragma unroll
        for (int r = 0; r < 4; ++r) {
          float val = sacc[nt][r] * scale;
          sacc[nt][r] = val;
          mx[r] = fmaxf(mx[r], val);
        }
    }
    float psum[4];
#pragma unroll
    for (int r = 0; r < 4; ++r) {
      mx[r] = group16_reduce(mx[r], MaxOp());
      const float THR = 8.f;
      if (mx[r] > m_run[r] + THR || m_run[r] == -INFINITY) {
        float m_new = fmaxf(m_run[r], mx[r]);
        float corr = (m_run[r] == -INFINITY) ? 0.f : __expf(m_run[r] - m_new);
        l_run[r] *= corr;
#pragma unroll
        for (int dt = 0; dt < NDT; ++dt) oacc[dt][r] *= corr;
        m_run[r] = m_new;
      }
      psum[r] = 0.f;
    }
#pragma unroll
    for (int nt = 0; nt < 4; ++nt) {
#pragma unroll
      for (int r = 0; r < 4; ++r) {
        float p = (sacc[nt][r] == -INFINITY) ? 0.f : __expf(sacc[nt][r] - m_run[r]);
        sacc[nt][r] = p;
        psum[r] += p;
      }
    }
#pragma unroll
    for (int r = 0; r < 4; ++r) {
      psum[r] = group16_reduce(psum[r], SumOp());
      l_run[r] += psum[r];
    }

    char* pw = p_lds + wq * (16 * KB * 2);
#pragma unroll
    for (int nt = 0; nt < 4; ++nt) {
#pragma unroll
      for (int r = 0; r < 4; ++r) {
        unsigned row = lg * 4 + r, col = nt * 16 + l16;
        *reinterpret_cast<short*>(pw + lds_off(row, col * 2, KB * 2)) = f2bf(sacc[nt][r]);
      }
    }
    LGKM0();

#pragma unroll
    for (int kk = 0; kk < KB / 32; ++kk) {
      shortx8 pf = lds_read8(pw, l16, kk * 32 + lg * 8, KB * 2);
#pragma unroll
      for (int dt = 0; dt < NDT; ++dt) {
        shortx8 vf = lds_read8(vt_lds, dt * 16 + l16, kk * 32 + lg * 8, VT_RS);
        oacc[dt] = mfma_bf16(pf, vf, oacc[dt]);
      }
    }
    __syncthreads();
  }

#pragma unroll
  for (int r = 0; r < 4; ++r) {
    int row = q0 + wq * 16 + lg * 4 + r;
    if (row >= Sq) continue;
    float inv_l = (l_run[r] > 0.f) ? 1.f / l_run[r] : 0.f;
#pragma unroll
    for (int dt = 0; dt < NDT; ++dt)
      og[obase + (long long)row * o_ss + dt * 16 + l16] = f2bf(oacc[dt][r] * inv_l);
    if (l16 == 0)
      lseg[(long long)(b * H + h) * Sq + row] =
          (l_run[r] > 0.f) ? m_run[r] + __logf(l_run[r]) : -INFINITY;
  }
}

template <int D>
__global__ void fa_bwd_delta_kernel(const short* __restrict__ dog, const short* __restrict__ og,
                                    float* __restrict__ delta, int H, int Sq,
                                    long long rows,
                                    long long do_sb, long long do_sh, long long do_ss,
                                    long long o_sb, long long o_sh, long long o_ss) {
  long long wid = ((long long)blockIdx.x * blockDim.x + threadIdx.x) >> 6;
  int lane = threadIdx.x & 63;
  long long nwaves = ((long long)gridDim.x * blockDim.x) >> 6;
  for (long long r = wid; r < rows; r += nwaves) {
    int sq = (int)(r % Sq);
    int h = (int)((r / Sq) % H);
    int b = (int)(r / ((long long)Sq * H));
    const long long dob = b * do_sb + h * do_sh + sq * do_ss;
    const long long ob = b * o_sb + h * o_sh + sq * o_ss;
    float acc = 0.f;
    for (int j = lane * 8; j < D; j += 64 * 8) {
      shortx8 a = *reinterpret_cast<const shortx8*>(dog + dob + j);
      shortx8 bb = *reinterpret_cast<const shortx8*>(og + ob + j);
#pragma unroll
      for (int k = 0; k < 8; ++k) acc += bf2f(a[k]) * bf2f(bb[k]);
    }
    acc = wave_reduce(acc, SumOp());
    if (lane == 0) delta[r] = acc;
  }
}

template <int D, bool CAUSAL>
__launch_bounds__(512)
__global__ void fa_bwd_dkv_kernel(const short* __restrict__ dog, const short* __restrict__ qg,
                                  const short* __restrict__ kg, const short* __restrict__ vg,
                                  const float* __restrict__ lseg, const float* __restrict__ deltag,
                                  short* __restrict__ dkg, short* __restrict__ dvg,
                                  int B, int H, int Sq, int Skv, float scale,
                                  long long q_sb, long long q_sh, long long q_ss,
                                  long long k_sb, long long k_sh, long long k_ss,
                                  long long do_sb, long long do_sh, long long do_ss,
                                  long long dk_sb, long long dk_sh, long long dk_ss) {
  constexpr int NW = 8;
  constexpr int NT = NW * 64;
  constexpr int KVEXT = NW * 16;
  constexpr int QB = 64;
  constexpr int NKK = D / 32;
  constexpr int NDT = D / 16;
  constexpr unsigned NAT_RS = D * 2;
  constexpr unsigned TR_RS = QB * 2;
  __shared__ char q_lds[QB * D * 2];
  __shared__ char qt_lds[D * QB * 2];
  __shared__ char do_lds[QB * D * 2];
  __shared__ char dot_lds[D * QB * 2];
  __shared__ char ps_lds[NW * 16 * QB * 2];

  const int kvblk = blockIdx.y;
  const int bh = blockIdx.x;
  const int kv0 = kvblk * KVEXT;
  const int b = bh / H, h = bh % H;
  const long long qbase = (long long)b * q_sb + (long long)h * q_sh;
  const long long dobase = (long long)b * do_sb + (long long)h * do_sh;
  const long long kvbase = (long long)b * k_sb + (long long)h * k_sh;
  const long long dkbase = (long long)b * dk_sb + (long long)h * dk_sh;
  const long long lse_base = ((long long)bh) * Sq;

  const int tid = threadIdx.x;
  const int lane = tid & 63;
  const int wq = tid >> 6;
  const int l16 = lane & 15;
  const int lg = lane >> 4;

  shortx8 kf[NKK], vf[NKK];
  {
    int row = kv0 + wq * 16 + l16;
    bool ok = row < Skv;
#pragma unroll
    for (int kk = 0; kk < NKK; ++kk) {
      if (ok) {
        kf[kk] = *reinterpret_cast<const shortx8*>(kg + kvbase + (long long)row * k_ss + kk * 32 + lg * 8);
        vf[kk] = *reinterpret_cast<const shortx8*>(vg + kvbase + (long long)row * k_ss + kk * 32 + lg * 8);
      } else {
        for (int i = 0; i < 8; ++i) { kf[kk][i] = 0; vf[kk][i] = 0; }
      }
    }
  }

  floatx4 dk_acc[NDT], dv_acc[NDT];
#pragma unroll
  for (int dt = 0; dt < NDT; ++dt) {
    dk_acc[dt] = {0.f, 0.f, 0.f, 0.f};
    dv_acc[dt] = {0.f, 0.f, 0.f, 0.f};
  }

  const int q_start = CAUSAL ? (kv0 / QB) * QB : 0;

  int n_row[QB * D / (NT * 8)], n_colp[QB * D / (NT * 8)];
#pragma unroll
  for (int it = 0; it < QB * D / (NT * 8); ++it) {
    int flat = it * NT * 8 + tid * 8;
    int row = flat / D, col = flat % D;
    n_row[it] = row;
    n_colp[it] = col ^ ((row & 7) << 3);
  }

  for (int q0 = q_start; q0 < Sq; q0 += QB) {
    if (q0 + QB <= Sq) {
#pragma unroll
      for (int it = 0; it < QB * D / (NT * 8); ++it) {
        const short* qsrc = qg + qbase + (long long)(q0 + n_row[it]) * q_ss + n_colp[it];
        const short* dsrc = dog + dobase + (long long)(q0 + n_row[it]) * do_ss + n_colp[it];
        __builtin_amdgcn_global_load_lds(
            (const __attribute__((address_space(1))) unsigned int*)qsrc,
            (__attribute__((address_space(3))) unsigned int*)(q_lds + it * NT * 16 + (tid >> 6) * 64 * 16),
            16, 0, 0);
        __builtin_amdgcn_global_load_lds(
            (const __attribute__((address_space(1))) unsigned int*)dsrc,
            (__attribute__((address_space(3))) unsigned int*)(do_lds + it * NT * 16 + (tid >> 6) * 64 * 16),
            16, 0, 0);
      }
      __syncthreads();
      constexpr int elems = QB * D;
      const int rot = threadIdx.x & 7;
      for (int flat = tid * 8; flat < elems; flat += NT * 8) {
        int row = flat / D, col = flat % D;
        shortx8 qv = lds_read8(q_lds, row, col, NAT_RS);
        shortx8 dv = lds_read8(do_lds, row, col, NAT_RS);
#pragma unroll
        for (int j = 0; j < 8; ++j) {
          int i = (j + rot) & 7;
          *reinterpret_cast<short*>(qt_lds + lds_off(col + i, row * 2, TR_RS)) = qv[i];
          *reinterpret_cast<short*>(dot_lds + lds_off(col + i, row * 2, TR_RS)) = dv[i];
        }
      }
    } else {
      constexpr int elems = QB * D;
      for (int flat = tid * 8; flat < elems; flat += NT * 8) {
        int row = flat / D, col = flat % D;
        shortx8 qv, dv;
        if (q0 + row < Sq) {
          qv = *reinterpret_cast<const shortx8*>(qg + qbase + (long long)(q0 + row) * q_ss + col);
          dv = *reinterpret_cast<const shortx8*>(dog + dobase + (long long)(q0 + row) * do_ss + col);
        } else {
          for (int i = 0; i < 8; ++i) { qv[i] = 0; dv[i] = 0; }
        }
        *reinterpret_cast<shortx8*>(q_lds + lds_off(row, col * 2, NAT_RS)) = qv;
        *reinterpret_cast<shortx8*>(do_lds + lds_off(row, col * 2, NAT_RS)) = dv;
        const int rot = threadIdx.x & 7;
#pragma unroll
        for (int j = 0; j < 8; ++j) {
          int i = (j + rot) & 7;
          *reinterpret_cast<short*>(qt_lds + lds_off(col + i, row * 2, TR_RS)) = qv[i];
          *reinterpret_cast<short*>(dot_lds + lds_off(col + i, row * 2, TR_RS)) = dv[i];
        }
      }
    }
    __syncthreads();

    float lse_v[4], delta_v[4];
#pragma unroll
    for (int nt = 0; nt < 4; ++nt) {
      int q_abs = q0 + nt * 16 + l16;
      lse_v[nt] = (q_abs < Sq) ? lseg[lse_base + q_abs] : INFINITY;
      delta_v[nt] = (q_abs < Sq) ? deltag[lse_base + q_abs] : 0.f;
    }

    floatx4 pt[4];
    const int kv_abs0 = kv0 + wq * 16 + lg * 4;
#pragma unroll
    for (int nt = 0; nt < 4; ++nt) {
      floatx4 st = {0.f, 0.f, 0.f, 0.f};
#pragma unroll
      for (int kk = 0; kk < NKK; ++kk) {
        shortx8 qfr = lds_read8(q_lds, nt * 16 + l16, kk * 32 + lg * 8, NAT_RS);
        st = mfma_bf16(kf[kk], qfr, st);
      }
      const int q_abs = q0 + nt * 16 + l16;
      const bool bnd = (q0 + QB > Sq) || (kv0 + KVEXT > Skv) ||
                       (CAUSAL && q0 < kv0 + KVEXT);
      if (bnd) {
#pragma unroll
        for (int r = 0; r < 4; ++r) {
          int kv_abs = kv_abs0 + r;
          float p = __expf(st[r] * scale - lse_v[nt]);
          if (q_abs >= Sq || kv_abs >= Skv || (CAUSAL && kv_abs > q_abs)) p = 0.f;
          pt[nt][r] = p;
        }
      } else {
#pragma unroll
        for (int r = 0; r < 4; ++r)
          pt[nt][r] = __expf(st[r] * scale - lse_v[nt]);
      }
    }

    char* pw = ps_lds + wq * (16 * QB * 2);
#pragma unroll
    for (int nt = 0; nt < 4; ++nt)
#pragma unroll
      for (int r = 0; r < 4; ++r)
        *reinterpret_cast<short*>(pw + lds_off(lg * 4 + r, (nt * 16 + l16) * 2, QB * 2)) =
            f2bf(pt[nt][r]);
    LGKM0();

#pragma unroll
    for (int kk = 0; kk < QB / 32; ++kk) {
      shortx8 pa = lds_read8(pw, l16, kk * 32 + lg * 8, QB * 2);
#pragma unroll
      for (int dt = 0; dt < NDT; ++dt) {
        shortx8 bfr = lds_read8(dot_lds, dt * 16 + l16, kk * 32 + lg * 8, TR_RS);
        dv_acc[dt] = mfma_bf16(pa, bfr, dv_acc[dt]);
      }
    }

#pragma unroll
    for (int nt = 0; nt < 4; ++nt) {
      floatx4 dp = {0.f, 0.f, 0.f, 0.f};
#pragma unroll
      for (int kk = 0; kk < NKK; ++kk) {
        shortx8 bfr = lds_read8(do_lds, nt * 16 + l16, kk * 32 + lg * 8, NAT_RS);
        dp = mfma_bf16(vf[kk], bfr, dp);
      }
#pragma unroll
      for (int r = 0; r < 4; ++r)
        pt[nt][r] = pt[nt][r] * (dp[r] - delta_v[nt]) * scale;
    }
    LGKM0();
#pragma unroll
    for (int nt = 0; nt < 4; ++nt)
#pragma unroll
      for (int r = 0; r < 4; ++r)
        *reinterpret_cast<short*>(pw + lds_off(lg * 4 + r, (nt * 16 + l16) * 2, QB * 2)) =
            f2bf(pt[nt][r]);
    LGKM0();

#pragma unroll
    for (int kk = 0; kk < QB / 32; ++kk) {
      shortx8 pa = lds_read8(pw, l16, kk * 32 + lg * 8, QB * 2);
#pragma unroll
      for (int dt = 0; dt < NDT; ++dt) {
        shortx8 bfr = lds_read8(qt_lds, dt * 16 + l16, kk * 32 + lg * 8, TR_RS);
        dk_acc[dt] = mfma_bf16(pa, bfr, dk_acc[dt]);
      }
    }
    __syncthreads();
  }

#pragma unroll
  for (int r = 0; r < 4; ++r) {
    int row = kv0 + wq * 16 + lg * 4 + r;
    if (row >= Skv) continue;
#pragma unroll
    for (int dt = 0; dt < NDT; ++dt) {
      dkg[dkbase + (long long)row * dk_ss + dt * 16 + l16] = f2bf(dk_acc[dt][r]);
      dvg[dkbase + (long long)row * dk_ss + dt * 16 + l16] = f2bf(dv_acc[dt][r]);
    }
  }
}

template <int D, bool CAUSAL>
__launch_bounds__(512)
__global__ void fa_bwd_dq_kernel(const short* __restrict__ dog, const short* __restrict__ qg,
                                 const short* __restrict__ kg, const short* __restrict__ vg,
                                 const float* __restrict__ lseg, const float* __restrict__ deltag,
                                 short* __restrict__ dqg, int B, int H, int Sq, int Skv,
                                 float scale,
                                 long long q_sb, long long q_sh, long long q_ss,
                                 long long k_sb, long long k_sh, long long k_ss,
                                 long long do_sb, long long do_sh, long long do_ss,
                                 long long dq_sb, long long dq_sh, long long dq_ss) {
  constexpr int NW = 8;
  constexpr int NT = NW * 64;
  constexpr int QEXT = NW * 16;
  constexpr int KB = 64;
  constexpr int NKK = D / 32;
  constexpr int NDT = D / 16;
  constexpr unsigned NAT_RS = D * 2;
  constexpr unsigned TR_RS = KB * 2;
  __shared__ char k_lds[KB * D * 2];
  __shared__ char v_lds[KB * D * 2];
  __shared__ char kt_lds[D * KB * 2];
  __shared__ char ps_lds[NW * 16 * KB * 2];

  const int qblk = blockIdx.x;
  const int bh = blockIdx.y;
  const int b = bh / H, h = bh % H;
  const int q0 = qblk * QEXT;
  const long long qbase = (long long)b * q_sb + (long long)h * q_sh;
  const long long dobase = (long long)b * do_sb + (long long)h * do_sh;
  const long long dqbase = (long long)b * dq_sb + (long long)h * dq_sh;
  const long long kvbase = (long long)b * k_sb + (long long)h * k_sh;
  const long long lse_base = ((long long)bh) * Sq;

  const int tid = threadIdx.x;
  const int lane = tid & 63;
  const int wq = tid >> 6;
  const int l16 = lane & 15;
  const int lg = lane >> 4;

  shortx8 qf[NKK], dof[NKK];
  {
    int row = q0 + wq * 16 + l16;
    bool ok = row < Sq;
#pragma unroll
    for (int kk = 0; kk < NKK; ++kk) {
      if (ok) {
        qf[kk] = *reinterpret_cast<const shortx8*>(qg + qbase + (long long)row * q_ss + kk * 32 + lg * 8);
        dof[kk] = *reinterpret_cast<const shortx8*>(dog + dobase + (long long)row * do_ss + kk * 32 + lg * 8);
      } else {
        for (int i = 0; i < 8; ++i) { qf[kk][i] = 0; dof[kk][i] = 0; }
      }
    }
  }
  float lse_r[4], delta_r[4];
#pragma unroll
  for (int r = 0; r < 4; ++r) {
    int row = q0 + wq * 16 + lg * 4 + r;
    lse_r[r] = (row < Sq) ? lseg[lse_base + row] : INFINITY;
    delta_r[r] = (row < Sq) ? deltag[lse_base + row] : 0.f;
  }

  floatx4 dq_acc[NDT];
#pragma unroll
  for (int dt = 0; dt < NDT; ++dt) dq_acc[dt] = {0.f, 0.f, 0.f, 0.f};

  const int kv_end = CAUSAL ? min(Skv, q0 + QEXT) : Skv;
  int n_row[KB * D / (NT * 8)], n_colp[KB * D / (NT * 8)];
#pragma unroll
  for (int it = 0; it < KB * D / (NT * 8); ++it) {
    int flat = it * NT * 8 + tid * 8;
    int row = flat / D, col = flat % D;
    n_row[it] = row;
    n_colp[it] = col ^ ((row & 7) << 3);
  }
  for (int kv0 = 0; kv0 < kv_end; kv0 += KB) {
    if (kv0 + KB <= Skv) {
#pragma unroll
      for (int it = 0; it < KB * D / (NT * 8); ++it) {
        const short* ksrc = kg + kvbase + (long long)(kv0 + n_row[it]) * k_ss + n_colp[it];
        const short* vsrc = vg + kvbase + (long long)(kv0 + n_row[it]) * k_ss + n_colp[it];
        __builtin_amdgcn_global_load_lds(
            (const __attribute__((address_space(1))) unsigned int*)ksrc,
            (__attribute__((address_space(3))) unsigned int*)(k_lds + it * NT * 16 + (tid >> 6) * 64 * 16),
            16, 0, 0);
        __builtin_amdgcn_global_load_lds(
            (const __attribute__((address_space(1))) unsigned int*)vsrc,
            (__attribute__((address_space(3))) unsigned int*)(v_lds + it * NT * 16 + (tid >> 6) * 64 * 16),
            16, 0, 0);
      }
      constexpr int elems = KB * D;
      const int rot = threadIdx.x & 7;
      for (int flat = tid * 8; flat < elems; flat += NT * 8) {
        int row = flat / D, col = flat % D;
        shortx8 kv_ = *reinterpret_cast<const shortx8*>(kg + kvbase + (long long)(kv0 + row) * k_ss + col);
#pragma unroll
        for (int j = 0; j < 8; ++j) {
          int i = (j + rot) & 7;
          *reinterpret_cast<short*>(kt_lds + lds_off(col + i, row * 2, TR_RS)) = kv_[i];
        }
      }
    } else {
      constexpr int elems = KB * D;
      for (int flat = tid * 8; flat < elems; flat += NT * 8) {
        int row = flat / D, col = flat % D;
        shortx8 kv_, vv;
        if (kv0 + row < Skv) {
          kv_ = *reinterpret_cast<const shortx8*>(kg + kvbase + (long long)(kv0 + row) * k_ss + col);
          vv = *reinterpret_cast<const shortx8*>(vg + kvbase + (long long)(kv0 + row) * k_ss + col);
        } else {
          for (int i = 0; i < 8; ++i) { kv_[i] = 0; vv[i] = 0; }
        }
        *reinterpret_cast<shortx8*>(k_lds + lds_off(row, col * 2, NAT_RS)) = kv_;
        *reinterpret_cast<shortx8*>(v_lds + lds_off(row, col * 2, NAT_RS)) = vv;
        const int rot = threadIdx.x & 7;
#pragma unroll
        for (int j = 0; j < 8; ++j) {
          int i = (j + rot) & 7;
          *reinterpret_cast<short*>(kt_lds + lds_off(col + i, row * 2, TR_RS)) = kv_[i];
        }
      }
    }
    __syncthreads();

    const int q_abs0 = q0 + wq * 16 + lg * 4;
    floatx4 ds[4];
#pragma unroll
    for (int nt = 0; nt < 4; ++nt) {
      floatx4 s = {0.f, 0.f, 0.f, 0.f}, dp = {0.f, 0.f, 0.f, 0.f};
#pragma unroll
      for (int kk = 0; kk < NKK; ++kk) {
        shortx8 kfr = lds_read8(k_lds, nt * 16 + l16, kk * 32 + lg * 8, NAT_RS);
        s = mfma_bf16(qf[kk], kfr, s);
        shortx8 vfr = lds_read8(v_lds, nt * 16 + l16, kk * 32 + lg * 8, NAT_RS);
        dp = mfma_bf16(dof[kk], vfr, dp);
      }
      const int kv_abs = kv0 + nt * 16 + l16;
      const bool bnd = (kv0 + KB > Skv) || (CAUSAL && kv0 + KB > q_abs0);
      if (bnd) {
#pragma unroll
        for (int r = 0; r < 4; ++r) {
          float p = __expf(s[r] * scale - lse_r[r]);
          if (kv_abs >= Skv || (CAUSAL && kv_abs > q_abs0 + r)) p = 0.f;
          ds[nt][r] = p * (dp[r] - delta_r[r]) * scale;
        }
      } else {
#pragma unroll
        for (int r = 0; r < 4; ++r) {
          float p = __expf(s[r] * scale - lse_r[r]);
          ds[nt][r] = p * (dp[r] - delta_r[r]) * scale;
        }
      }
    }

    char* pw = ps_lds + wq * (16 * KB * 2);
#pragma unroll
    for (int nt = 0; nt < 4; ++nt)
#pragma unroll
      for (int r = 0; r < 4; ++r)
        *reinterpret_cast<short*>(pw + lds_off(lg * 4 + r, (nt * 16 + l16) * 2, KB * 2)) =
            f2bf(ds[nt][r]);
    LGKM0();

#pragma unroll
    for (int kk = 0; kk < KB / 32; ++kk) {
      shortx8 pa = lds_read8(pw, l16, kk * 32 + lg * 8, KB * 2);
#pragma unroll
      for (int dt = 0; dt < NDT; ++dt) {
        shortx8 bfr = lds_read8(kt_lds, dt * 16 + l16, kk * 32 + lg * 8, TR_RS);
        dq_acc[dt] = mfma_bf16(pa, bfr, dq_acc[dt]);
      }
    }
    __syncthreads();
  }

#pragma unroll
  for (int r = 0; r < 4; ++r) {
    int row = q0 + wq * 16 + lg * 4 + r;
    if (row >= Sq) continue;
#pragma unroll
    for (int dt = 0; dt < NDT; ++dt)
      dqg[dqbase + (long long)row * dq_ss + dt * 16 + l16] = f2bf(dq_acc[dt][r]);
  }
}

void flash_attn_fwd(const void* q, const void* k, const void* v, void* o,
                    float* lse, int64_t b, int64_t h, int64_t hkv, int64_t sq,
                    int64_t skv, int64_t dh, float scale, bool causal,
                    const int64_t* qs, const int64_t* ks, const int64_t* os,
                    hipStream_t s) {
  dim3 grid((unsigned)cdiv((int)sq, 128), (unsigned)(b * h));
  dim3 blk(512);
#define FAF(D, C)                                                             \
  hipLaunchKernelGGL((fa_fwd_kernel<D, C>), grid, blk, 0, s, (const short*)q, \
                     (const short*)k, (const short*)v, (short*)o, lse,        \
                     (int)b, (int)h, (int)hkv, (int)sq, (int)skv, scale,      \
                     qs[0], qs[1], qs[2], ks[0], ks[1], ks[2],                \
                     os[0], os[1], os[2])
  if (dh == 128) { if (causal) FAF(128, true); else FAF(128, false); }
  else           { if (causal) FAF(64, true);  else FAF(64, false); }
#undef FAF
}

void flash_attn_bwd(const void* dout, const void* q, const void* k,
                    const void* v, const void* o, const float* lse,
                    void* dq, void* dk, void* dv, float* delta, int64_t b,
                    int64_t h, int64_t hkv, int64_t sq, int64_t skv,
                    int64_t dh, float scale, bool causal,
                    const int64_t* qs, const int64_t* ks, const int64_t* dos,
                    const int64_t* os, const int64_t* dqs, const int64_t* dks,
                    const void* mask, const int64_t* ms, float pdrop,
                    uint64_t seed, uint64_t offset, hipStream_t s) {
  long long rows = b * h * sq;
  dim3 dgrid((unsigned)hmin<long long>(2048LL, (rows + 3) / 4));
  if (dh == 128)
    hipLaunchKernelGGL((fa_bwd_delta_kernel<128>), dgrid, dim3(256), 0, s,
                       (const short*)dout, (const short*)o, delta, (int)h,
                       (int)sq, rows, dos[0], dos[1], dos[2], os[0], os[1], os[2]);
  else
    hipLaunchKernelGGL((fa_bwd_delta_kernel<64>), dgrid, dim3(256), 0, s,
                       (const short*)dout, (const short*)o, delta, (int)h,
                       (int)sq, rows, dos[0], dos[1], dos[2], os[0], os[1], os[2]);

  dim3 gkv((unsigned)(b * h), (unsigned)cdiv((int)skv, 128));
  dim3 gq((unsigned)cdiv((int)sq, 128), (unsigned)(b * h));
  static const bool dkv16_env = [] {
    const char* e = getenv("PA_FA_DKV32");
    return !(e && e[0] == '1');
  }();
  const bool use_dkv16 = dkv16_env && mask == nullptr && pdrop <= 0.f;
#define FAB(D, C)                                                              \
  do {                                                                         \
    if (use_dkv16)                                                             \
      hipLaunchKernelGGL((fa_bwd_dkv_kernel<D, C>), gkv, dim3(512), 0, s,      \
                         (const short*)dout, (const short*)q, (const short*)k, \
                         (const short*)v, lse, delta, (short*)dk, (short*)dv,  \
                         (int)b, (int)h, (int)sq, (int)skv, scale,             \
                         qs[0], qs[1], qs[2], ks[0], ks[1], ks[2],             \
                         dos[0], dos[1], dos[2], dks[0], dks[1], dks[2]);      \
    else                                                                       \
      flash_attn_bwd_dkv32(dout, q, k, v, lse, delta, dk, dv, b, h, sq, skv,   \
                           dh, scale, causal, qs, ks, dos, dks, mask, ms,      \
                           pdrop, seed, offset, s);                            \
    flash_attn_bwd_dq32(dout, q, k, v, lse, delta, dq, b, h, sq, skv, dh,     \
                        scale, causal, qs, ks, dos, dqs, mask, ms, pdrop,      \
                        seed, offset, s);                                      \
  } while (0)
  if (dh == 128) { if (causal) FAB(128, true); else FAB(128, false); }
  else           { if (causal) FAB(64, true);  else FAB(64, false); }
#undef FAB
}

void flash_attn_varlen_bwd(const void* dout, const void* q, const void* k,
                           const void* v, const void* o, const float* lse,
                           void* dq, void* dk, void* dv, float* delta,
                           int64_t h, int64_t total_q, int64_t total_k,
                           int64_t dh, float scale, bool causal,
                           int64_t nqblocks, int64_t nkvblocks,
                           const int* cu_q, const int* cu_k, const int* qbmap,
                           const int* kvbmap, float pdrop, uint64_t seed,
                           uint64_t offset, hipStream_t s) {
  long long rows = h * total_q;
  dim3 dgrid((unsigned)hmin<long long>(2048LL, (rows + 3) / 4));
  const long long ss = h * dh;
  if (dh == 128)
    hipLaunchKernelGGL((fa_bwd_delta_kernel<128>), dgrid, dim3(256), 0, s,
                       (const short*)dout, (const short*)o, delta, (int)h,
                       (int)total_q, rows, 0, dh, ss, 0, dh, ss);
  else
    hipLaunchKernelGGL((fa_bwd_delta_kernel<64>), dgrid, dim3(256), 0, s,
                       (const short*)dout, (const short*)o, delta, (int)h,
                       (int)total_q, rows, 0, dh, ss, 0, dh, ss);
  flash_attn_varlen_bwd32(dout, q, k, v, lse, delta, dq, dk, dv, h, total_q,
                          total_k, dh, scale, causal, nqblocks, nkvblocks,
                          cu_q, cu_k, qbmap, kvbmap, pdrop, seed, offset, s);
}

}
```

csrc/kernels/norms.hip:

```cpp
#include "common.h"
#include "api.h"

namespace pa {

template <int DT> struct VIO;

template <> struct VIO<kBF16> {
  using ST = short;
  static __device__ __forceinline__ void load8(const void* p, int64_t idx, float* f) {
    shortx8 v = *reinterpret_cast<const shortx8*>((const short*)p + idx);
#pragma unroll
    for (int i = 0; i < 8; ++i) f[i] = bf2f(v[i]);
  }
  static __device__ __forceinline__ void store8(void* p, int64_t idx, const float* f) {
    shortx8 v;
#pragma unroll
    for (int i = 0; i < 8; ++i) v[i] = f2bf(f[i]);
    *reinterpret_cast<shortx8*>((short*)p + idx) = v;
  }
  static __device__ __forceinline__ float load1(const void* p, int64_t idx) {
    return bf2f(((const short*)p)[idx]);
  }
  static __device__ __forceinline__ void store1(void* p, int64_t idx, float f) {
    ((short*)p)[idx] = f2bf(f);
  }
};

template <> struct VIO<kF32> {
  using ST = float;
  static __device__ __forceinline__ void load8(const void* p, int64_t idx, float* f) {
    const float4* q = reinterpret_cast<const float4*>((const float*)p + idx);
    float4 a = q[0], b = q[1];
    f[0] = a.x; f[1] = a.y; f[2] = a.z; f[3] = a.w;
    f[4] = b.x; f[5] = b.y; f[6] = b.z; f[7] = b.w;
  }
  static __device__ __forceinline__ void store8(void* p, int64_t idx, const float* f) {
    float4* q = reinterpret_cast<float4*>((float*)p + idx);
    q[0] = make_float4(f[0], f[1], f[2], f[3]);
    q[1] = make_float4(f[4], f[5], f[6], f[7]);
  }
  static __device__ __forceinline__ float load1(const void* p, int64_t idx) {
    return ((const float*)p)[idx];
  }
  static __device__ __forceinline__ void store1(void* p, int64_t idx, float f) {
    ((float*)p)[idx] = f;
  }
};

template <int DT>
__global__ void ln_fwd_kernel(const void* __restrict__ x, const void* __restrict__ w,
                              const void* __restrict__ b, void* __restrict__ y,
                              float* __restrict__ mean_out, float* __restrict__ rstd_out,
                              int64_t n, int64_t d, float eps) {
  __shared__ float red[12];
  for (int64_t row = blockIdx.x; row < n; row += gridDim.x) {
    const int64_t base = row * d;
    float shift;
    {
      float f0[8];
      VIO<DT>::load8(x, base, f0);
      shift = ((f0[0] + f0[1]) + (f0[2] + f0[3]) + (f0[4] + f0[5]) + (f0[6] + f0[7])) * 0.125f;
    }
    float sum = 0.f, sumc = 0.f, sumsq = 0.f;
    for (int64_t i = threadIdx.x * 8; i < d; i += blockDim.x * 8) {
      float f[8];
      VIO<DT>::load8(x, base + i, f);
#pragma unroll
      for (int k = 0; k < 8; ++k) {
#pragma clang fp reassociate(off)
        float c = f[k] - shift;
        sum += f[k];
        sumc += c;
        sumsq += c * c;
      }
    }
    float ts = block_reduce_256(sum, SumOp(), red, 0.f);
    float tsc = block_reduce_256(sumc, SumOp(), red + 4, 0.f);
    float tss = block_reduce_256(sumsq, SumOp(), red + 8, 0.f);
    float mu = ts / d;
    float dmu = tsc / d;
    float var = fmaxf(tss / d - dmu * dmu, 0.f);
    float rstd = rsqrtf(var + eps);
    if (threadIdx.x == 0) { mean_out[row] = mu; rstd_out[row] = rstd; }
    for (int64_t i = threadIdx.x * 8; i < d; i += blockDim.x * 8) {
      float f[8], wf[8], bf[8];
      VIO<DT>::load8(x, base + i, f);
      VIO<DT>::load8(w, i, wf);
      if (b) VIO<DT>::load8(b, i, bf);
#pragma unroll
      for (int k = 0; k < 8; ++k)
        f[k] = (f[k] - mu) * rstd * wf[k] + (b ? bf[k] : 0.f);
      VIO<DT>::store8(y, base + i, f);
    }
    __syncthreads();
  }
}

template <int DT>
__global__ void ln_bwd_dx_kernel(const void* __restrict__ dy, const void* __restrict__ x,
                                 const void* __restrict__ w, const float* __restrict__ mean,
                                 const float* __restrict__ rstd, void* __restrict__ dx,
                                 int64_t n, int64_t d) {
  __shared__ float red[8];
  for (int64_t row = blockIdx.x; row < n; row += gridDim.x) {
    const int64_t base = row * d;
    const float mu = mean[row], rs = rstd[row];
    float s1 = 0.f, s2 = 0.f;
    for (int64_t i = threadIdx.x * 8; i < d; i += blockDim.x * 8) {
      float gy[8], xf[8], wf[8];
      VIO<DT>::load8(dy, base + i, gy);
      VIO<DT>::load8(x, base + i, xf);
      VIO<DT>::load8(w, i, wf);
#pragma unroll
      for (int k = 0; k < 8; ++k) {
        float g = gy[k] * wf[k];
        float xh = (xf[k] - mu) * rs;
        s1 += g * xh;
        s2 += g;
      }
    }
    float t1 = block_reduce_256(s1, SumOp(), red, 0.f);
    __syncthreads();
    float t2 = block_reduce_256(s2, SumOp(), red + 4, 0.f);
    const float inv_d = 1.f / d;
    for (int64_t i = threadIdx.x * 8; i < d; i += blockDim.x * 8) {
      float gy[8], xf[8], wf[8];
      VIO<DT>::load8(dy, base + i, gy);
      VIO<DT>::load8(x, base + i, xf);
      VIO<DT>::load8(w, i, wf);
#pragma unroll
      for (int k = 0; k < 8; ++k) {
        float g = gy[k] * wf[k];
        float xh = (xf[k] - mu) * rs;
        gy[k] = rs * (g - t2 * inv_d - xh * t1 * inv_d);
      }
      VIO<DT>::store8(dx, base + i, gy);
    }
    __syncthreads();
  }
}

template <int DT, bool RMS>
__global__ void ln_bwd_dwdb_kernel(const void* __restrict__ dy, const void* __restrict__ x,
                                   const float* __restrict__ mean, const float* __restrict__ rstd,
                                   float* __restrict__ dw, float* __restrict__ db,
                                   int64_t n, int64_t d,
                                   float* __restrict__ ws = nullptr) {
  int64_t c0 = ((int64_t)blockIdx.x * blockDim.x + threadIdx.x) * 8;
  if (c0 >= d) return;
  int64_t rows_per = (n + gridDim.y - 1) / gridDim.y;
  int64_t r0 = (int64_t)blockIdx.y * rows_per;
  int64_t r1 = min(n, r0 + rows_per);
  float aw[8] = {0.f}, ab[8] = {0.f};
  if (c0 + 8 <= d) {
    for (int64_t r = r0; r < r1; ++r) {
      float g[8], xf[8];
      VIO<DT>::load8(dy, r * d + c0, g);
      VIO<DT>::load8(x, r * d + c0, xf);
      float mu = RMS ? 0.f : mean[r], rs = rstd[r];
#pragma unroll
      for (int k = 0; k < 8; ++k) {
        aw[k] += g[k] * (xf[k] - mu) * rs;
        ab[k] += g[k];
      }
    }
  } else {
    for (int64_t r = r0; r < r1; ++r) {
      float mu = RMS ? 0.f : mean[r], rs = rstd[r];
      for (int64_t c = c0; c < d; ++c) {
        float g = VIO<DT>::load1(dy, r * d + c);
        float xf = VIO<DT>::load1(x, r * d + c);
        aw[c - c0] += g * (xf - mu) * rs;
        ab[c - c0] += g;
      }
    }
  }
  if (ws) {
    float* wrow = ws + (int64_t)(2 * blockIdx.y) * d;
#pragma unroll
    for (int k = 0; k < 8; ++k)
      if (c0 + k < d) {
        wrow[c0 + k] = aw[k];
        wrow[d + c0 + k] = ab[k];
      }
    return;
  }
#pragma unroll
  for (int k = 0; k < 8; ++k)
    if (c0 + k < d) {
      atomicAdd(&dw[c0 + k], aw[k]);
      if (db) atomicAdd(&db[c0 + k], ab[k]);
    }
}

__global__ void dwdb_reduce_kernel(const float* __restrict__ ws, float* __restrict__ dw,
                                   float* __restrict__ db, int chunks, int64_t d) {
  int64_t c = (int64_t)blockIdx.x * blockDim.x + threadIdx.x;
  if (c >= d) return;
  float sw = 0.f, sb = 0.f;
  for (int ch = 0; ch < chunks; ++ch) {
    sw += ws[(int64_t)(2 * ch) * d + c];
    sb += ws[(int64_t)(2 * ch) * d + d + c];
  }
  dw[c] = sw;
  if (db) db[c] = sb;
}

template <int DT, bool HAS_RES>
__global__ void rms_fwd_kernel(const void* __restrict__ x, const void* __restrict__ res,
                               const void* __restrict__ w, void* __restrict__ y,
                               void* __restrict__ res_out, float* __restrict__ rstd_out,
                               int64_t n, int64_t d, float eps) {
  __shared__ float red[4];
  for (int64_t row = blockIdx.x; row < n; row += gridDim.x) {
    const int64_t base = row * d;
    float sumsq = 0.f;
    for (int64_t i = threadIdx.x * 8; i < d; i += blockDim.x * 8) {
      float f[8];
      VIO<DT>::load8(x, base + i, f);
      if (HAS_RES) {
        float r[8];
        VIO<DT>::load8(res, base + i, r);
#pragma unroll
        for (int k = 0; k < 8; ++k) f[k] += r[k];
        VIO<DT>::store8(res_out, base + i, f);
      }
#pragma unroll
      for (int k = 0; k < 8; ++k) sumsq += f[k] * f[k];
    }
    if (HAS_RES) __syncthreads();
    float tss = block_reduce_256(sumsq, SumOp(), red, 0.f);
    float rstd = rsqrtf(tss / d + eps);
    if (threadIdx.x == 0) rstd_out[row] = rstd;
    const void* src = HAS_RES ? res_out : x;
    for (int64_t i = threadIdx.x * 8; i < d; i += blockDim.x * 8) {
      float f[8], wf[8];
      VIO<DT>::load8(src, base + i, f);
      VIO<DT>::load8(w, i, wf);
#pragma unroll
      for (int k = 0; k < 8; ++k) f[k] = f[k] * rstd * wf[k];
      VIO<DT>::store8(y, base + i, f);
    }
    __syncthreads();
  }
}

template <int DT>
__global__ void rms_bwd_dx_kernel(const void* __restrict__ dy, const void* __restrict__ x,
                                  const void* __restrict__ w, const float* __restrict__ rstd,
                                  void* __restrict__ dx, int64_t n, int64_t d) {
  __shared__ float red[4];
  for (int64_t row = blockIdx.x; row < n; row += gridDim.x) {
    const int64_t base = row * d;
    const float rs = rstd[row];
    float s1 = 0.f;
    for (int64_t i = threadIdx.x * 8; i < d; i += blockDim.x * 8) {
      float gy[8], xf[8], wf[8];
      VIO<DT>::load8(dy, base + i, gy);
      VIO<DT>::load8(x, base + i, xf);
      VIO<DT>::load8(w, i, wf);
#pragma unroll
      for (int k = 0; k < 8; ++k) s1 += gy[k] * wf[k] * xf[k] * rs;
    }
    float t1 = block_reduce_256(s1, SumOp(), red, 0.f);
    const float c = t1 / d;
    for (int64_t i = threadIdx.x * 8; i < d; i += blockDim.x * 8) {
      float gy[8], xf[8], wf[8];
      VIO<DT>::load8(dy, base + i, gy);
      VIO<DT>::load8(x, base + i, xf);
      VIO<DT>::load8(w, i, wf);
#pragma unroll
      for (int k = 0; k < 8; ++k)
        gy[k] = rs * (gy[k] * wf[k] - xf[k] * rs * c);
      VIO<DT>::store8(dx, base + i, gy);
    }
    __syncthreads();
  }
}

static int norm_grid(int64_t n) {
  int64_t cap = 256 * 8;
  return (int)(n < cap ? n : cap);
}

#define DT_SWITCH(dtype, ...)                         \
  if (dtype == kBF16) {                               \
    constexpr int DT = kBF16;                         \
    __VA_ARGS__;                                      \
  } else {                                            \
    constexpr int DT = kF32;                          \
    __VA_ARGS__;                                      \
  }

void layer_norm_fwd(const void* x, const void* w, const void* b, void* y,
                    float* mean, float* rstd, int64_t n, int64_t d, float eps,
                    int dtype, hipStream_t s) {
  DT_SWITCH(dtype, hipLaunchKernelGGL((ln_fwd_kernel<DT>), dim3(norm_grid(n)),
                                      dim3(256), 0, s, x, w, b, y, mean, rstd, n, d, eps));
}

void layer_norm_bwd_dx(const void* dy, const void* x, const void* w,
                       const float* mean, const float* rstd, void* dx,
                       int64_t n, int64_t d, int dtype, hipStream_t s) {
  DT_SWITCH(dtype, hipLaunchKernelGGL((ln_bwd_dx_kernel<DT>), dim3(norm_grid(n)),
                                      dim3(256), 0, s, dy, x, w, mean, rstd, dx, n, d));
}

int ln_dwdb_chunks(int64_t n, int64_t d) {
  int xblocks = cdiv((int)d, 256 * 8);
  return (int)hmin<int64_t>(hmax<int64_t>(1, n / 32),
                            hmax<int64_t>(1, 2048 / xblocks));
}

void layer_norm_bwd_dwdb(const void* dy, const void* x, const float* mean,
                         const float* rstd, float* dw, float* db, int64_t n,
                         int64_t d, int dtype, hipStream_t s, float* ws) {
  int xblocks = cdiv((int)d, 256 * 8);
  int chunks = ln_dwdb_chunks(n, d);
  dim3 grid((unsigned)xblocks, chunks);
  DT_SWITCH(dtype, hipLaunchKernelGGL((ln_bwd_dwdb_kernel<DT, false>), grid,
                                      dim3(256), 0, s, dy, x, mean, rstd, dw, db, n, d, ws));
  if (ws)
    hipLaunchKernelGGL(dwdb_reduce_kernel, dim3((unsigned)cdiv((int)d, 256)),
                       dim3(256), 0, s, ws, dw, db, chunks, d);
}

void rms_norm_fwd(const void* x, const void* residual, const void* w, void* y,
                  void* res_out, float* rstd, int64_t n, int64_t d, float eps,
                  int dtype, hipStream_t s) {
  if (residual) {
    DT_SWITCH(dtype, hipLaunchKernelGGL((rms_fwd_kernel<DT, true>), dim3(norm_grid(n)),
                                        dim3(256), 0, s, x, residual, w, y, res_out, rstd, n, d, eps));
  } else {
    DT_SWITCH(dtype, hipLaunchKernelGGL((rms_fwd_kernel<DT, false>), dim3(norm_grid(n)),
                                        dim3(256), 0, s, x, nullptr, w, y, nullptr, rstd, n, d, eps));
  }
}

void rms_norm_bwd_dx(const void* dy, const void* x, const void* w,
                     const float* rstd, void* dx, int64_t n, int64_t d,
                     int dtype, hipStream_t s) {
  DT_SWITCH(dtype, hipLaunchKernelGGL((rms_bwd_dx_kernel<DT>), dim3(norm_grid(n)),
                                      dim3(256), 0, s, dy, x, w, rstd, dx, n, d));
}

void rms_norm_bwd_dw(const void* dy, const void* x, const float* rstd,
                     float* dw, int64_t n, int64_t d, int dtype, hipStream_t s,
                     float* ws) {
  int xblocks = cdiv((int)d, 256 * 8);
  int chunks = ln_dwdb_chunks(n, d);
  dim3 grid((unsigned)xblocks, chunks);
  DT_SWITCH(dtype, hipLaunchKernelGGL((ln_bwd_dwdb_kernel<DT, true>), grid,
                                      dim3(256), 0, s, dy, x, nullptr, rstd, dw, nullptr, n, d, ws));
  if (ws)
    hipLaunchKernelGGL(dwdb_reduce_kernel, dim3((unsigned)cdiv((int)d, 256)),
                       dim3(256), 0, s, ws, dw, nullptr, chunks, d);
}

}
```

paddle_amd/models/gpt.py:

```python
from __future__ import annotations

import math
from dataclasses import dataclass

import torch

from .. import nn
from ..nn.initializer import Constant, Normal
from ..ops import functional as hot


@dataclass
class GPTConfig:
    vocab_size: int = 50304
    hidden_size: int = 1024
    num_layers: int = 24
    num_heads: int = 16
    max_seq_len: int = 2048
    intermediate_size: int = 0
    hidden_dropout: float = 0.0
    attn_dropout: float = 0.0
    initializer_range: float = 0.02
    use_recompute: bool = False

    def __post_init__(self):
        if self.intermediate_size == 0:
            self.intermediate_size = 4 * self.hidden_size


PRESETS = {
    "gpt3-125m": GPTConfig(hidden_size=768, num_layers=12, num_heads=12),
    "gpt3-350m": GPTConfig(hidden_size=1024, num_layers=24, num_heads=16),
    "gpt3-1.3b": GPTConfig(hidden_size=2048, num_layers=24, num_heads=16),
    "gpt3-2.7b": GPTConfig(hidden_size=2560, num_layers=32, num_heads=20),
    "gpt3-6.7b": GPTConfig(hidden_size=4096, num_layers=32, num_heads=32),
    "gpt3-13b": GPTConfig(hidden_size=5120, num_layers=40, num_heads=40),
    "gpt3-tiny": GPTConfig(vocab_size=1024, hidden_size=128, num_layers=2,
                           num_heads=4, max_seq_len=256),
}


class GPTEmbeddings(nn.Layer):
    def __init__(self, cfg: GPTConfig):
        super().__init__()
        init = Normal(0.0, cfg.initializer_range)
        self.word_embeddings = nn.Embedding(cfg.vocab_size, cfg.hidden_size)
        self.position_embeddings = nn.Embedding(cfg.max_seq_len, cfg.hidden_size)
        from ..nn.initializer import _apply_initializer
        _apply_initializer(init, self.word_embeddings.weight)
        _apply_initializer(init, self.position_embeddings.weight)
        self.dropout = nn.Dropout(cfg.hidden_dropout)

    def forward(self, input_ids, position_ids=None):
        if position_ids is None:
            position_ids = torch.arange(input_ids.shape[1], device=input_ids.device)
            position_ids = position_ids.unsqueeze(0).expand_as(input_ids)
        x = self.word_embeddings(input_ids) + self.position_embeddings(position_ids)
        return self.dropout(x)


class GPTAttention(nn.Layer):
    def __init__(self, cfg: GPTConfig):
        super().__init__()
        h = cfg.hidden_size
        init = Normal(0.0, cfg.initializer_range)
        out_init = Normal(0.0, cfg.initializer_range / math.sqrt(2 * cfg.num_layers))
        self.num_heads = cfg.num_heads
        self.head_dim = h // cfg.num_heads
        self.qkv_proj = nn.Linear(h, 3 * h)
        self.out_proj = nn.Linear(h, h)
        from ..nn.initializer import _apply_initializer
        _apply_initializer(init, self.qkv_proj.weight)
        _apply_initializer(out_init, self.out_proj.weight)
        self.attn_dropout = cfg.attn_dropout

    def forward(self, x):
        b, s, h = x.shape
        qkv = self.qkv_proj(x).reshape(b, s, 3, self.num_heads, self.head_dim)
        out = hot.qkv_flash_attention(qkv, causal=True, dropout=self.attn_dropout,
                                      training=self.training)
        return self.out_proj(out)


class GPTMLP(nn.Layer):
    def __init__(self, cfg: GPTConfig):
        super().__init__()
        init = Normal(0.0, cfg.initializer_range)
        out_init = Normal(0.0, cfg.initializer_range / math.sqrt(2 * cfg.num_layers))
        self.fc1 = nn.Linear(cfg.hidden_size, cfg.intermediate_size, bias_attr=False)
        self.fc1_bias = self.create_parameter([cfg.intermediate_size], is_bias=True)
        self.fc2 = nn.Linear(cfg.intermediate_size, cfg.hidden_size)
        from ..nn.initializer import _apply_initializer
        _apply_initializer(init, self.fc1.weight)
        _apply_initializer(out_init, self.fc2.weight)

    def forward(self, x):
        w1 = getattr(self.fc1, "weight", None)
        if w1 is not None and hot._own_linear_ok(x, w1):
            return hot.fused_ffn_own(x, w1, self.fc1_bias,
                                     self.fc2.weight, self.fc2.bias)
        if w1 is not None and hot._fused_ffn_available(x):
            return hot.fused_ffn(x, w1, self.fc1_bias,
                                 self.fc2.weight, self.fc2.bias)
        return self.fc2(hot.bias_gelu(self.fc1(x), self.fc1_bias))


class GPTDecoderLayer(nn.Layer):
    def __init__(self, cfg: GPTConfig):
        super().__init__()
        self.ln1 = nn.LayerNorm(cfg.hidden_size)
        self.attn = GPTAttention(cfg)
        self.ln2 = nn.LayerNorm(cfg.hidden_size)
        self.mlp = GPTMLP(cfg)
        self.dropout = cfg.hidden_dropout

    def forward(self, x):
        h = hot.dropout_add(self.attn(self.ln1(x)), x, self.dropout, self.training)
        return hot.dropout_add(self.mlp(self.ln2(h)), h, self.dropout, self.training)


class GPTModel(nn.Layer):
    def __init__(self, cfg: GPTConfig):
        super().__init__()
        self.cfg = cfg
        self.embeddings = GPTEmbeddings(cfg)
        self.layers = nn.LayerList([GPTDecoderLayer(cfg) for _ in range(cfg.num_layers)])
        self.final_norm = nn.LayerNorm(cfg.hidden_size)

    def forward(self, input_ids, position_ids=None):
        x = self.embeddings(input_ids, position_ids)
        use_rc = self.cfg.use_recompute and self.training
        if use_rc:
            from ..distributed.fleet.recompute import recompute
        for layer in self.layers:
            if use_rc and x.requires_grad:
                x = recompute(layer, x)
            else:
                x = layer(x)
        return self.final_norm(x)


class GPTForPretraining(nn.Layer):
    def __init__(self, cfg: GPTConfig):
        super().__init__()
        self.cfg = cfg
        self.gpt = GPTModel(cfg)
        self.lm_head = nn.Linear(cfg.hidden_size, cfg.vocab_size, bias_attr=False)
        from ..nn.initializer import Normal, _apply_initializer
        _apply_initializer(Normal(0.0, cfg.initializer_range), self.lm_head.weight)

    def forward(self, input_ids, position_ids=None):
        x = self.gpt(input_ids, position_ids)
        return self.lm_head(x)

    def sharding_units(self):
        return [self.gpt.embeddings, *self.gpt.layers,
                self.gpt.final_norm, self.lm_head]


class GPTPretrainingCriterion(nn.Layer):
    def __init__(self, ignore_index=-100):
        super().__init__()
        self.ignore_index = ignore_index

    def forward(self, logits, labels):
        loss = hot.softmax_cross_entropy(logits, labels, self.ignore_index,
                                         reduction="none")
        n_valid = (labels != self.ignore_index).sum().clamp(min=1)
        return loss.sum() / n_valid.to(loss.dtype)


def build_gpt(preset="gpt3-tiny", **overrides):
    import dataclasses
    cfg = dataclasses.replace(PRESETS[preset], **overrides)
    return GPTForPretraining(cfg)
```

paddle_amd/ops/functional.py:

```python
from __future__ import annotations

import math
from typing import Optional

import torch

from .. import _ext

_TRACE_SUBSTRATE = False


def _tracing():
    return _TRACE_SUBSTRATE


_NATIVE_DTYPES = (torch.bfloat16, torch.float32)


def _kernel_ok(x, *, last_mult=1, numel_mult=1, same=(), vecs=(),
               contiguous=()):
    if not isinstance(x, torch.Tensor) or x.dtype not in _NATIVE_DTYPES:
        return False
    if x.dim() < 1 or x.numel() == 0:
        return False
    if x.shape[-1] % last_mult or x.numel() % numel_mult:
        return False
    for t in same:
        if t is not None and (t.dtype != x.dtype or t.shape != x.shape):
            return False
    for t in vecs:
        if t is not None and not (t.is_floating_point()
                                  and t.numel() == x.shape[-1]):
            return False
    return all(t is None or t.is_contiguous() for t in contiguous)


def _norm_native_ok(x, w, b=None, residual=None):
    return _kernel_ok(x, last_mult=8, same=(residual,), vecs=(w, b))


def _bias_gelu_native_ok(x, bias=None):
    return _kernel_ok(x, last_mult=8, vecs=(bias,))


def _swiglu_native_ok(x):
    return _kernel_ok(x, last_mult=16)


def _rope_native_ok(x, cos_t, sin_t, pos_offset=0):
    if not (_kernel_ok(x, last_mult=8, contiguous=(cos_t, sin_t))
            and x.dim() == 4 and pos_offset >= 0):
        return False
    half = x.shape[-1] // 2
    return all(t.dtype == torch.float32 and t.dim() == 2
               and t.shape[1] == half and t.shape[0] >= x.shape[1] + pos_offset
               for t in (cos_t, sin_t))


def _dropout_add_native_ok(x, residual=None):
    return _kernel_ok(x, numel_mult=8, same=(residual,))


def _embedding_native_ok(table, ids):
    return (_kernel_ok(table, last_mult=8) and table.dim() == 2
            and not ids.is_floating_point() and ids.dtype != torch.bool)


def _ce_native_ok(logits, labels):
    return (_kernel_ok(logits) and not labels.is_floating_point()
            and labels.dtype != torch.bool
            and labels.numel() == logits.numel() // logits.shape[-1])


def _reduce_native_ok(x):
    return _kernel_ok(x)


def _adamw_native_ok(master, param_out, grad, m, v):
    if not all(t.dtype == torch.float32 and t.numel() == master.numel()
               for t in (master, m, v)):
        return False
    if param_out is not None and not (param_out.dtype in _NATIVE_DTYPES
                                      and param_out.numel() == master.numel()):
        return False
    return (_kernel_ok(grad) and grad.numel() == master.numel()
            and all(t is None or t.is_contiguous()
                    for t in (master, m, v, param_out)))


def _as_dtype(t, dtype):
    if t is None:
        return None
    return (t if t.dtype == dtype else t.to(dtype)).contiguous()


class _LayerNorm(torch.autograd.Function):
    @staticmethod
    def forward(ctx, x, w, b, eps):
        ctx.native = _ext.use_native(x) and _norm_native_ok(x, w, b)
        ctx.w_dtype = w.dtype
        ctx.b_dtype = b.dtype if b is not None else w.dtype
        if ctx.native:
            C = _ext.get_ext()
            x, w = x.contiguous(), _as_dtype(w, x.dtype)
            y, mean, rstd = C.layer_norm_fwd(x, w, _as_dtype(b, x.dtype), eps)
        else:
            xf = x.float()
            mean = xf.mean(-1).reshape(-1)
            var = xf.var(-1, unbiased=False).reshape(-1)
            rstd = torch.rsqrt(var + eps)
            d = x.shape[-1]
            xhat = (xf - mean.view(*x.shape[:-1], 1)) * rstd.view(*x.shape[:-1], 1)
            y = xhat * w.float() + (b.float() if b is not None else 0.0)
            y = y.to(x.dtype)
        ctx.save_for_backward(x, w, mean, rstd)
        ctx.has_bias = b is not None
        return y

    @staticmethod
    def backward(ctx, dy):
        x, w, mean, rstd = ctx.saved_tensors
        if ctx.native:
            C = _ext.get_ext()
            dx, dw, db = C.layer_norm_bwd(dy.to(x.dtype).contiguous(), x, w,
                                          mean, rstd, ctx.has_bias)
            dw, db = dw.to(ctx.w_dtype), db.to(ctx.b_dtype)
        else:
            d = x.shape[-1]
            xf = x.float()
            dyf = dy.float()
            mu = mean.view(*x.shape[:-1], 1)
            rs = rstd.view(*x.shape[:-1], 1)
            xhat = (xf - mu) * rs
            g = dyf * w.float()
            s1 = (g * xhat).mean(-1, keepdim=True)
            s2 = g.mean(-1, keepdim=True)
            dx = (rs * (g - s2 - xhat * s1)).to(x.dtype)
            dw = (dyf * xhat).reshape(-1, d).sum(0).to(w.dtype)
            db = dyf.reshape(-1, d).sum(0).to(ctx.b_dtype)
        return dx, dw, (db if ctx.has_bias else None), None


def layer_norm(x, weight, bias=None, epsilon=1e-5):
    if _tracing():
        return torch.nn.functional.layer_norm(x, (x.shape[-1],), weight, bias,
                                              epsilon)
    return _LayerNorm.apply(x, weight, bias, epsilon)


class _RMSNorm(torch.autograd.Function):
    @staticmethod
    def forward(ctx, x, w, eps):
        ctx.native = _ext.use_native(x) and _norm_native_ok(x, w)
        ctx.w_dtype = w.dtype
        if ctx.native:
            C = _ext.get_ext()
            x, w = x.contiguous(), _as_dtype(w, x.dtype)
            y, rstd = C.rms_norm_fwd(x, None, w, eps)
        else:
            xf = x.float()
            rstd = torch.rsqrt(xf.square().mean(-1) + eps).reshape(-1)
            y = (xf * rstd.view(*x.shape[:-1], 1) * w.float()).to(x.dtype)
        ctx.save_for_backward(x, w, rstd)
        return y

    @staticmethod
    def backward(ctx, dy):
        x, w, rstd = ctx.saved_tensors
        if ctx.native:
            C = _ext.get_ext()
            dx, dw = C.rms_norm_bwd(dy.to(x.dtype).contiguous(), x, w, rstd)
            dw = dw.to(ctx.w_dtype)
        else:
            d = x.shape[-1]
            xf, dyf = x.float(), dy.float()
            rs = rstd.view(*x.shape[:-1], 1)
            xhat = xf * rs
            g = dyf * w.float()
            s1 = (g * xhat).mean(-1, keepdim=True)
            dx = (rs * (g - xhat * s1)).to(x.dtype)
            dw = (dyf * xhat).reshape(-1, d).sum(0).to(w.dtype)
        return dx, dw, None


def rms_norm(x, weight, epsilon=1e-6):
    if _tracing():
        xf = x.float()
        y = xf * torch.rsqrt(xf.square().mean(-1, keepdim=True) + epsilon)
        return (y * weight.float()).to(x.dtype)
    return _RMSNorm.apply(x, weight, epsilon)


class _FusedRMSNormResidual(torch.autograd.Function):

    @staticmethod
    def forward(ctx, x, residual, w, eps):
        ctx.native = _ext.use_native(x) and _norm_native_ok(x, w, residual=residual)
        ctx.w_dtype = w.dtype
        if ctx.native:
            C = _ext.get_ext()
            w = _as_dtype(w, x.dtype)
            y, rstd, xr = C.rms_norm_fwd(x.contiguous(), residual.contiguous(), w, eps)
        else:
            xr = x + residual
            xf = xr.float()
            rstd = torch.rsqrt(xf.square().mean(-1) + eps).reshape(-1)
            y = (xf * rstd.view(*x.shape[:-1], 1) * w.float()).to(x.dtype)
        ctx.save_for_backward(xr, w, rstd)
        return y, xr

    @staticmethod
    def backward(ctx, dy, dxr):
        xr, w, rstd = ctx.saved_tensors
        if ctx.native:
            C = _ext.get_ext()
            dx, dw = C.rms_norm_bwd(dy.to(xr.dtype).contiguous(), xr, w, rstd)
            dw = dw.to(ctx.w_dtype)
        else:
            d = xr.shape[-1]
            xf, dyf = xr.float(), dy.float()
            rs = rstd.view(*xr.shape[:-1], 1)
            xhat = xf * rs
            g = dyf * w.float()
            s1 = (g * xhat).mean(-1, keepdim=True)
            dx = (rs * (g - xhat * s1)).to(xr.dtype)
            dw = (dyf * xhat).reshape(-1, d).sum(0).to(w.dtype)
        if dxr is not None:
            dx = dx + dxr
        return dx, dx, dw, None


def fused_rms_norm(x, norm_weight, residual=None, epsilon=1e-6):
    if _tracing() and residual is not None:
        xr = x + residual
        return rms_norm(xr, norm_weight, epsilon), xr
    if residual is None:
        return rms_norm(x, norm_weight, epsilon)
    return _FusedRMSNormResidual.apply(x, residual, norm_weight, epsilon)


class _SoftmaxCE(torch.autograd.Function):
    @staticmethod
    def forward(ctx, logits, labels, ignore_index):
        shp = logits.shape
        v = shp[-1]
        l2 = logits.reshape(-1, v)
        lab = labels.reshape(-1)
        ctx.native = _ext.use_native(logits) and _ce_native_ok(logits, labels)
        if ctx.native:
            C = _ext.get_ext()
            l2, lab = l2.contiguous(), lab.long().contiguous()
            loss, lse = C.softmax_ce_fwd(l2, lab, ignore_index)
        else:
            lab = lab.long()
            lf = l2.float()
            lse = torch.logsumexp(lf, -1)
            skip = (lab == ignore_index) | (lab < 0) | (lab >= v)
            safe = lab.masked_fill(skip, 0)
            picked = lf.gather(1, safe.unsqueeze(1)).squeeze(1)
            loss = torch.where(skip, torch.zeros_like(lse), lse - picked)
        ctx.save_for_backward(l2, lab, lse)
        ctx.ignore_index = ignore_index
        ctx.in_shape = shp
        return loss.reshape(shp[:-1])

    @staticmethod
    def backward(ctx, dloss):
        l2, lab, lse = ctx.saved_tensors
        dl = dloss.reshape(-1).float().contiguous()
        if ctx.native:
            C = _ext.get_ext()
            dlogits = C.softmax_ce_bwd(dl, l2, lab, lse, ctx.ignore_index)
        else:
            p = torch.exp(l2.float() - lse.unsqueeze(1))
            onehot = torch.zeros_like(p)
            skip = (lab == ctx.ignore_index) | (lab < 0) | (lab >= l2.shape[-1])
            safe = lab.masked_fill(skip, 0)
            onehot.scatter_(1, safe.unsqueeze(1), 1.0)
            g = torch.where(skip.unsqueeze(1),
                            torch.zeros_like(dl).unsqueeze(1), dl.unsqueeze(1))
            dlogits = (g * (p - onehot)).to(l2.dtype)
        return dlogits.reshape(ctx.in_shape), None, None


def softmax_cross_entropy(logits, labels, ignore_index=-100, reduction="none"):
    if _tracing():
        v = logits.shape[-1]
        loss = torch.nn.functional.cross_entropy(
            logits.reshape(-1, v).float(), labels.reshape(-1),
            ignore_index=ignore_index, reduction="none").reshape(labels.shape)
    else:
        loss = _SoftmaxCE.apply(logits, labels, ignore_index)
    if reduction == "mean":
        n_valid = (labels != ignore_index).sum().clamp(min=1)
        return loss.sum() / n_valid.to(loss.dtype)
    if reduction == "sum":
        return loss.sum()
    return loss


class _BiasGelu(torch.autograd.Function):
    @staticmethod
    def forward(ctx, x, bias):
        ctx.save_for_backward(x, bias if bias is not None else torch.empty(0))
        ctx.has_bias = bias is not None
        ctx.native = _ext.use_native(x) and _bias_gelu_native_ok(x, bias)
        if ctx.native:
            C = _ext.get_ext()
            return C.bias_gelu_fwd(x.contiguous(), _as_dtype(bias, x.dtype))
        v = x.float() + (bias.float() if bias is not None else 0.0)
        return torch.nn.functional.gelu(v).to(x.dtype)

    @staticmethod
    def backward(ctx, dy):
        x, bias = ctx.saved_tensors
        b = bias if ctx.has_bias else None
        if ctx.native:
            C = _ext.get_ext()
            dx = C.bias_gelu_bwd(dy.to(x.dtype).contiguous(), x.contiguous(),
                                 _as_dtype(b, x.dtype))
            db = C.colsum(dx).to(b.dtype) if ctx.has_bias else None
        else:
            v = x.float() + (b.float() if b is not None else 0.0)
            cdf = 0.5 * (1.0 + torch.erf(v * 0.7071067811865476))
            pdf = 0.3989422804014327 * torch.exp(-0.5 * v * v)
            dx = (dy.float() * (cdf + v * pdf)).to(x.dtype)
            db = dx.float().reshape(-1, dx.shape[-1]).sum(0).to(b.dtype) if ctx.has_bias else None
        return dx, db


def bias_gelu(x, bias=None):
    if _tracing():
        return torch.nn.functional.gelu(x + bias if bias is not None else x)
    return _BiasGelu.apply(x, bias)


class _SwiGLU(torch.autograd.Function):
    @staticmethod
    def forward(ctx, x):
        ctx.native = _ext.use_native(x) and _swiglu_native_ok(x)
        if ctx.native:
            x = x.contiguous()
        ctx.save_for_backward(x)
        if ctx.native:
            C = _ext.get_ext()
            return C.swiglu_fwd(x)
        d = x.shape[-1] // 2
        g, u = x[..., :d].float(), x[..., d:].float()
        return (torch.nn.functional.silu(g) * u).to(x.dtype)

    @staticmethod
    def backward(ctx, dy):
        (x,) = ctx.saved_tensors
        if ctx.native:
            C = _ext.get_ext()
            return C.swiglu_bwd(dy.to(x.dtype).contiguous(), x)
        d = x.shape[-1] // 2
        g, u = x[..., :d].float(), x[..., d:].float()
        sig = torch.sigmoid(g)
        silu = g * sig
        dg = dy.float() * u * (sig * (1 + g * (1 - sig)))
        du = dy.float() * silu
        return torch.cat([dg, du], dim=-1).to(x.dtype)


def swiglu(x, y=None):
    if _tracing():
        if y is None:
            g, u = x.chunk(2, -1)
        else:
            g, u = x, y
        return torch.nn.functional.silu(g) * u
    if y is not None:
        x = torch.cat([x, y], dim=-1)
    return _SwiGLU.apply(x)


_rope_cache = {}


def build_rope_cache(seq_len, head_dim, base=10000.0, device=None, dtype=torch.float32):
    key = (seq_len, head_dim, base, str(device))
    if key not in _rope_cache:
        half = head_dim // 2
        inv = 1.0 / (base ** (torch.arange(0, half, dtype=torch.float32, device=device) / half))
        t = torch.arange(seq_len, dtype=torch.float32, device=device)
        freqs = torch.outer(t, inv)
        _rope_cache[key] = (freqs.cos().contiguous(), freqs.sin().contiguous())
    return _rope_cache[key]


class _Rope(torch.autograd.Function):
    @staticmethod
    def forward(ctx, x, cos_t, sin_t, pos_offset):
        ctx.save_for_backward(cos_t, sin_t)
        ctx.pos_offset = pos_offset
        ctx.native = _ext.use_native(x) and _rope_native_ok(x, cos_t, sin_t, pos_offset)
        if ctx.native:
            C = _ext.get_ext()
            return C.rope_fwd(x.contiguous(), cos_t, sin_t, pos_offset, False)
        return _rope_ref(x, cos_t, sin_t, pos_offset, conj=False)

    @staticmethod
    def backward(ctx, dy):
        cos_t, sin_t = ctx.saved_tensors
        if ctx.native and _rope_native_ok(dy, cos_t, sin_t, ctx.pos_offset):
            C = _ext.get_ext()
            return C.rope_fwd(dy.contiguous(), cos_t, sin_t, ctx.pos_offset, True), None, None, None
        return _rope_ref(dy, cos_t, sin_t, ctx.pos_offset, conj=True), None, None, None


def _rope_ref(x, cos_t, sin_t, pos_offset, conj):
    b, s, h, d = x.shape
    half = d // 2
    c = cos_t[pos_offset:pos_offset + s].view(1, s, 1, half).float()
    sn = sin_t[pos_offset:pos_offset + s].view(1, s, 1, half).float()
    if conj:
        sn = -sn
    x1, x2 = x[..., :half].float(), x[..., half:].float()
    y1 = x1 * c - x2 * sn
    y2 = x2 * c + x1 * sn
    return torch.cat([y1, y2], dim=-1).to(x.dtype)


def fused_rotary_position_embedding(q, k=None, v=None, sin=None, cos=None,
                                    position_ids=None, use_neox_rotary_style=True,
                                    base=10000.0, pos_offset=0):
    if _tracing():
        b, s, h, d = q.shape
        if cos is None or sin is None:
            cos_t, sin_t = build_rope_cache(s + pos_offset, d, base, q.device)
        else:
            cos_t = cos.float().reshape(-1, d)[..., : d // 2]
            sin_t = sin.float().reshape(-1, d)[..., : d // 2]
        outs = [_rope_ref(q.float(), cos_t, sin_t, pos_offset, False).to(q.dtype)]
        if k is not None:
            outs.append(_rope_ref(k.float(), cos_t, sin_t, pos_offset, False).to(k.dtype))
        if v is not None:
            outs.append(v)
        return tuple(outs) if len(outs) > 1 else outs[0]
    """paddle.incubate.nn.functional.fused_rotary_position_embedding parity
    (SURVEY.md A.7).  q/k/v: [B, S, H, D]."""
    bq, s, hq, d = q.shape
    if cos is None or sin is None:
        cos_t, sin_t = build_rope_cache(s + pos_offset, d, base, q.device)
    else:
        cos_t, sin_t = cos.float().reshape(-1, d)[..., : d // 2].contiguous(), \
                       sin.float().reshape(-1, d)[..., : d // 2].contiguous()
    if pos_offset < 0 or min(cos_t.shape[0], sin_t.shape[0]) < s + pos_offset:
        raise ValueError(
            f"fused_rotary_position_embedding: cos/sin hold "
            f"{min(cos_t.shape[0], sin_t.shape[0])} positions, need seq_len + "
            f"pos_offset = {s + pos_offset}")
    outs = [_Rope.apply(q, cos_t, sin_t, pos_offset)]
    if k is not None:
        outs.append(_Rope.apply(k, cos_t, sin_t, pos_offset))
    if v is not None:
        outs.append(v)
    return tuple(outs) if len(outs) > 1 else outs[0]


def _fa_native_ok(q):
    return (_ext.use_native(q) and q.dtype == torch.bfloat16
            and q.shape[-1] in (64, 128) and q.stride(-1) == 1)


def _fa_seed_offset(fixed_seed_offset=None):
    if fixed_seed_offset is not None:
        return int(fixed_seed_offset[0]), int(fixed_seed_offset[1])
    seed = int(torch.initial_seed()) & 0x7FFFFFFFFFFFFFFF
    offset = int(torch.randint(0, 2 ** 31, (1,)).item())
    return seed, offset


class _FlashAttn(torch.autograd.Function):
    @staticmethod
    def forward(ctx, q, k, v, scale, causal, mask=None, dropout=0.0,
                seed=0, offset=0):
        if _fa_native_ok(q):
            C = _ext.get_ext()
            mk = mask.to(torch.bfloat16) if mask is not None else None
            o, lse = C.flash_attn_fwd(q, k, v, None, scale, causal, mk,
                                      dropout, seed, offset)
            ctx.native = True
            ctx.mask = mk
        else:
            dm = None
            if dropout > 0.0:
                g = torch.Generator(device="cpu").manual_seed(
                    (seed * 1000003 + offset) & 0x7FFFFFFFFFFFFFFF)
                dm = (torch.rand(q.shape[0], q.shape[1], q.shape[2], k.shape[2],
                                 generator=g) >= dropout).to(q.device)
            o, lse = _sdpa_ref(q, k, v, scale, causal, mask, dm, dropout)
            ctx.native = False
            ctx.mask = mask
            ctx.drop_mask = dm
        ctx.save_for_backward(q, k, v, o, lse)
        ctx.scale, ctx.causal = scale, causal
        ctx.dropout, ctx.seed, ctx.offset = dropout, seed, offset
        ctx.mark_non_differentiable(lse)
        return o, lse

    @staticmethod
    def backward(ctx, do, _dlse):
        q, k, v, o, lse = ctx.saved_tensors
        if ctx.native:
            C = _ext.get_ext()
            if do.stride(-1) != 1:
                do = do.contiguous()
            kw = dict(scale=ctx.scale, causal=ctx.causal, mask=ctx.mask,
                      pdrop=ctx.dropout, seed=ctx.seed, offset=ctx.offset)
            if k.shape[1] != q.shape[1]:
                rep = q.shape[1] // k.shape[1]
                ke = k.repeat_interleave(rep, dim=1)
                ve = v.repeat_interleave(rep, dim=1)
                dq, dke, dve = C.flash_attn_bwd(do, q, ke.contiguous(), ve.contiguous(),
                                                o, lse, **kw)
                hkv = k.shape[1]
                dk = dke.view(k.shape[0], hkv, rep, k.shape[2], k.shape[3]).sum(2)
                dv = dve.view(v.shape[0], hkv, rep, v.shape[2], v.shape[3]).sum(2)
            else:
                dq, dk, dv = C.flash_attn_bwd(do, q, k, v, o, lse, **kw)
        else:
            dq, dk, dv = _sdpa_ref_bwd(do, q, k, v, lse, ctx.scale, ctx.causal,
                                       ctx.mask, getattr(ctx, "drop_mask", None),
                                       ctx.dropout)
        return dq, dk, dv, None, None, None, None, None, None


class _QKVFlashAttn(torch.autograd.Function):

    @staticmethod
    def forward(ctx, qkv, scale, causal, dropout=0.0, seed=0, offset=0):
        b, s, three, h, d = qkv.shape
        q = qkv[:, :, 0].permute(0, 2, 1, 3)
        k = qkv[:, :, 1].permute(0, 2, 1, 3)
        v = qkv[:, :, 2].permute(0, 2, 1, 3)
        if _fa_native_ok(q):
            C = _ext.get_ext()
            out = torch.empty(b, s, h, d, dtype=qkv.dtype, device=qkv.device)
            o_view = out.permute(0, 2, 1, 3)
            _, lse = C.flash_attn_fwd(q, k, v, o_view, scale, causal, None,
                                      dropout, seed, offset)
            ctx.native = True
            ctx.save_for_backward(qkv, out, lse)
            ctx.drop_mask = None
        else:
            dm = None
            if dropout > 0.0:
                g = torch.Generator(device="cpu").manual_seed(
                    (seed * 1000003 + offset) & 0x7FFFFFFFFFFFFFFF)
                dm = (torch.rand(b, h, s, s, generator=g) >= dropout).to(qkv.device)
            o, lse = _sdpa_ref(q.contiguous(), k.contiguous(), v.contiguous(),
                               scale, causal, None, dm, dropout)
            out = o.permute(0, 2, 1, 3).reshape(b, s, h, d)
            ctx.native = False
            ctx.save_for_backward(qkv, out, lse)
            ctx.drop_mask = dm
        ctx.scale, ctx.causal = scale, causal
        ctx.dropout, ctx.seed, ctx.offset = dropout, seed, offset
        return out.reshape(b, s, h * d)

    @staticmethod
    def backward(ctx, do):
        qkv, out, lse = ctx.saved_tensors
        b, s, three, h, d = qkv.shape
        q = qkv[:, :, 0].permute(0, 2, 1, 3)
        k = qkv[:, :, 1].permute(0, 2, 1, 3)
        v = qkv[:, :, 2].permute(0, 2, 1, 3)
        o_view = out.permute(0, 2, 1, 3)
        do_view = do.reshape(b, s, h, d).permute(0, 2, 1, 3)
        if ctx.native:
            C = _ext.get_ext()
            if do_view.stride(-1) != 1:
                do_view = do.contiguous().reshape(b, s, h, d).permute(0, 2, 1, 3)
            dqkv = torch.empty_like(qkv)
            dq = dqkv[:, :, 0].permute(0, 2, 1, 3)
            dk = dqkv[:, :, 1].permute(0, 2, 1, 3)
            dv = dqkv[:, :, 2].permute(0, 2, 1, 3)
            C.flash_attn_bwd(do_view, q, k, v, o_view, lse, dq, dk, dv,
                             ctx.scale, ctx.causal, None, ctx.dropout,
                             ctx.seed, ctx.offset)
        else:
            dq, dk, dv = _sdpa_ref_bwd(do_view.contiguous(), q.contiguous(),
                                       k.contiguous(), v.contiguous(), lse,
                                       ctx.scale, ctx.causal, None,
                                       ctx.drop_mask, ctx.dropout)
            dqkv = torch.stack([dq, dk, dv], dim=0).permute(1, 3, 0, 2, 4).contiguous()
        return dqkv, None, None, None, None, None


def qkv_flash_attention(qkv, scale=None, causal=True, dropout=0.0,
                        training=True):
    if scale is None:
        scale = 1.0 / math.sqrt(qkv.shape[-1])
    if _tracing():
        b, s, three, h, d = qkv.shape
        q = qkv[:, :, 0].permute(0, 2, 1, 3)
        k = qkv[:, :, 1].permute(0, 2, 1, 3)
        v = qkv[:, :, 2].permute(0, 2, 1, 3)
        o = torch.nn.functional.scaled_dot_product_attention(
            q, k, v, is_causal=causal, scale=scale)
        return o.permute(0, 2, 1, 3).reshape(b, s, h * d)
    p = dropout if training else 0.0
    seed, offset = _fa_seed_offset() if p > 0 else (0, 0)
    return _QKVFlashAttn.apply(qkv, scale, causal, p, seed, offset)


def _sdpa_ref(q, k, v, scale, causal, attn_mask=None, drop_mask=None,
              dropout=0.0):
    qf, kf, vf = q.float(), k.float(), v.float()
    if k.shape[1] != q.shape[1]:
        rep = q.shape[1] // k.shape[1]
        kf = kf.repeat_interleave(rep, dim=1)
        vf = vf.repeat_interleave(rep, dim=1)
    s = torch.matmul(qf, kf.transpose(-1, -2)) * scale
    if attn_mask is not None:
        s = s + attn_mask.float()
    if causal:
        sq, skv = s.shape[-2], s.shape[-1]
        mask = torch.ones(sq, skv, dtype=torch.bool, device=s.device).tril()
        s = s.masked_fill(~mask, float("-inf"))
    lse = torch.logsumexp(s, -1)
    p = torch.exp(s - lse.unsqueeze(-1))
# ... 456 lines not shown
```

Before: 24040 tokens/s.

## Fuse residual add into LayerNorm, fuse GELU bias-grad, and rework attention delta kernel

Adds a fused residual-add plus LayerNorm forward kernel and a fused LayerNorm backward. The backward computes dx, folds in the residual gradient, and writes per-block dw/db partials that a separate workspace kernel reduces, replacing the separate dx and dwdb passes plus the zero-fill. The GPT decoder is restructured to defer each residual add into the next layer's LayerNorm. Separately, the bias-GELU backward accumulates the bias gradient inside the elementwise kernel instead of running a second colsum pass, and the flash-attention delta kernel is rewritten to use sub-wave row groups with unrolled vector loads. The aim is fewer memory passes over activations, at the cost of more complex kernels; the fused add-LN path falls back to the old ops when dropout is active in training.

```diff
diff --git a/csrc/bindings.cpp b/csrc/bindings.cpp
--- a/csrc/bindings.cpp
+++ b/csrc/bindings.cpp
@@ -79,14 +79,70 @@
   return {y, mean, rstd};
 }
 
+std::vector<Tensor> add_layer_norm_fwd(const Tensor& x, const Tensor& residual,
+                                       const Tensor& w,
+                                       const c10::optional<Tensor>& b, double eps) {
+  CHECK_IN(x);
+  check_rows(x, "add_layer_norm");
+  int64_t d = x.size(-1), n = x.numel() / d;
+  CHECK_SAME(residual, x);
+  TORCH_CHECK(residual.sizes() == x.sizes(), "residual must have the shape of x");
+  CHECK_VEC(w, x, d);
+  if (b.has_value()) CHECK_VEC((*b), x, d);
+  auto h = torch::empty_like(x);
+  auto y = torch::empty_like(x);
+  auto mean = torch::empty({n}, x.options().dtype(torch::kFloat));
+  auto rstd = torch::empty({n}, x.options().dtype(torch::kFloat));
+  const void* bp = b.has_value() ? b->const_data_ptr() : nullptr;
+  if (pa::ln_fused_ok(d)) {
+    pa::add_layer_norm_fwd(x.const_data_ptr(), residual.const_data_ptr(),
+                           w.const_data_ptr(), bp, h.mutable_data_ptr(),
+                           y.mutable_data_ptr(), mean.mutable_data_ptr<float>(),
+                           rstd.mutable_data_ptr<float>(), n, d, (float)eps,
+                           dt_of(x), cur_stream());
+  } else {
+    pa::dropout_add_fwd(x.const_data_ptr(), residual.const_data_ptr(),
+                        h.mutable_data_ptr(), nullptr, x.numel(), 0.f, 0, 0,
+                        dt_of(x), cur_stream());
+    pa::layer_norm_fwd(h.const_data_ptr(), w.const_data_ptr(), bp,
+                       y.mutable_data_ptr(), mean.mutable_data_ptr<float>(),
+                       rstd.mutable_data_ptr<float>(), n, d, (float)eps, dt_of(x),
+                       cur_stream());
+  }
+  return {h, y, mean, rstd};
+}
+
+int64_t ln_bwd_grid_cap() { return pa::kLnBwdGridCap; }
+bool ln_fused_ok(int64_t d) { return pa::ln_fused_ok(d); }
+
 std::vector<Tensor> layer_norm_bwd(const Tensor& dy, const Tensor& x,
                                    const Tensor& w, const Tensor& mean,
-                                   const Tensor& rstd, bool has_bias) {
+                                   const Tensor& rstd, bool has_bias,
+                                   const c10::optional<Tensor>& dres,
+                                   bool fused, int64_t grid_cap) {
   CHECK_IN(x);
   check_rows(x, "layer_norm_bwd");
   int64_t d = x.size(-1), n = x.numel() / d;
   CHECK_SAME(dy, x); CHECK_VEC(w, x, d);
   CHECK_STAT(mean, n); CHECK_STAT(rstd, n);
+  if (dres.has_value()) CHECK_SAME((*dres), x);
+  TORCH_CHECK(grid_cap >= 0 && grid_cap <= 65536, "layer_norm_bwd: bad grid_cap");
+  if (fused && pa::ln_fused_ok(d)) {
+    auto dx = torch::empty_like(x);
+    auto dw = torch::empty({d}, x.options().dtype(torch::kFloat));
+    auto db = torch::empty({d}, x.options().dtype(torch::kFloat));
+    int grid = pa::ln_bwd_fused_grid(n, (int)grid_cap);
+    auto ws = torch::empty({(int64_t)grid * 2 * d}, x.options().dtype(torch::kFloat));
+    pa::layer_norm_bwd_fused(dy.const_data_ptr(), x.const_data_ptr(),
+                             w.const_data_ptr(), mean.const_data_ptr<float>(),
+                             rstd.const_data_ptr<float>(),
+                             dres.has_value() ? dres->const_data_ptr() : nullptr,
+                             dx.mutable_data_ptr(), dw.mutable_data_ptr<float>(),
+                             db.mutable_data_ptr<float>(),
+                             ws.mutable_data_ptr<float>(), grid, n, d, dt_of(x),
+                             cur_stream());
+    return {dx, dw, db};
+  }
   auto dx = torch::empty_like(x);
   auto dw = torch::zeros({d}, x.options().dtype(torch::kFloat));
   auto db = torch::zeros({d}, x.options().dtype(torch::kFloat));
@@ -99,6 +155,7 @@
                           mean.const_data_ptr<float>(), rstd.const_data_ptr<float>(),
                           dw.mutable_data_ptr<float>(), db.mutable_data_ptr<float>(),
                           n, d, dt_of(x), cur_stream(), ws.mutable_data_ptr<float>());
+  if (dres.has_value()) dx.add_(dres->view_as(dx));
   return {dx, dw, db};
 }
 
@@ -198,6 +255,38 @@
                     bias.has_value() ? bias->const_data_ptr() : nullptr,
                     dx.mutable_data_ptr(), n, d, dt_of(x), cur_stream());
   return dx;
+}
+
+std::vector<Tensor> bias_gelu_bwd_db(const Tensor& dy, const Tensor& x,
+                                     const c10::optional<Tensor>& bias, bool fused) {
+  CHECK_IN(x);
+  check_rows(x, "bias_gelu_bwd_db");
+  int64_t d = x.size(-1), n = x.numel() / d;
+  CHECK_SAME(dy, x);
+  if (bias.has_value()) CHECK_VEC((*bias), x, d);
+  const void* bp = bias.has_value() ? bias->const_data_ptr() : nullptr;
+  auto dx = torch::empty_like(x);
+  int grid = fused ? pa::bias_gelu_bwd_db_grid(n, d) : 0;
+  if (grid > 0) {
+    const int64_t w = d % 16 == 0 ? 16 : 8;
+    auto db = torch::empty({d}, x.options().dtype(torch::kFloat));
+    auto ws = torch::empty({(int64_t)grid * 256 * w}, x.options().dtype(torch::kFloat));
+    pa::bias_gelu_bwd_db(dy.const_data_ptr(), x.const_data_ptr(), bp,
+                         dx.mutable_data_ptr(), db.mutable_data_ptr<float>(),
+                         ws.mutable_data_ptr<float>(), grid, n, d, dt_of(x),
+                         cur_stream());
+    return {dx, db};
+  }
+  pa::bias_gelu_bwd(dy.const_data_ptr(), x.const_data_ptr(), bp,
+                    dx.mutable_data_ptr(), n, d, dt_of(x), cur_stream());
+  auto db = torch::zeros({d}, x.options().dtype(torch::kFloat));
+  pa::colsum(dx.const_data_ptr(), db.mutable_data_ptr<float>(), n, d, dt_of(x),
+             cur_stream());
+  return {dx, db};
+}
+
+bool bias_gelu_bwd_db_fused(int64_t n, int64_t d) {
+  return pa::bias_gelu_bwd_db_grid(n, d) > 0;
 }
 
 Tensor swiglu_fwd(const Tensor& x) {
@@ -399,6 +488,29 @@
                      mp, ms, (float)pdrop, (uint64_t)seed, (uint64_t)offset,
                      cur_stream());
   return {dq, dk, dv};
+}
+
+Tensor flash_attn_bwd_delta(const Tensor& dout, const Tensor& o) {
+  TORCH_CHECK(dout.is_cuda() && o.is_cuda() &&
+              dout.scalar_type() == torch::kBFloat16 &&
+              o.scalar_type() == torch::kBFloat16 && dout.dim() == 4 &&
+              dout.sizes() == o.sizes() && dout.numel() > 0,
+              "flash_attn_bwd_delta: dout / o must be bf16 [b, h, sq, d] GPU tensors of one shape");
+  int64_t b = o.size(0), h = o.size(1), sq = o.size(2), d = o.size(3);
+  TORCH_CHECK(d == 128 || d == 64, "flash_attn_bwd_delta: head_dim must be 64 or 128");
+  int64_t dos[3], os[3];
+  fa_strides(dout, dos); fa_strides(o, os);
+  for (int i = 0; i < 3; ++i)
+    TORCH_CHECK(dos[i] % 8 == 0 && os[i] % 8 == 0 && dos[i] >= 0 && os[i] >= 0,
+                "flash_attn_bwd_delta: strides must keep rows 16-byte aligned");
+  TORCH_CHECK(reinterpret_cast<uintptr_t>(dout.const_data_ptr()) % 16 == 0 &&
+              reinterpret_cast<uintptr_t>(o.const_data_ptr()) % 16 == 0,
+              "flash_attn_bwd_delta: 16-byte aligned data required");
+  auto delta = torch::empty({b, h, sq}, o.options().dtype(torch::kFloat));
+  pa::flash_attn_bwd_delta(dout.const_data_ptr(), o.const_data_ptr(),
+                           delta.mutable_data_ptr<float>(), b, h, sq, d, dos, os,
+                           cur_stream());
+  return delta;
 }
 
 static std::pair<Tensor, int64_t> make_bmap(const Tensor& cu_cpu, int64_t blk) {
@@ -938,7 +1050,19 @@
 
 PYBIND11_MODULE(TORCH_EXTENSION_NAME, m) {
   m.def("layer_norm_fwd", &layer_norm_fwd);
-  m.def("layer_norm_bwd", &layer_norm_bwd);
+  m.def("layer_norm_bwd", &layer_norm_bwd, py::arg("dy"), py::arg("x"),
+        py::arg("w"), py::arg("mean"), py::arg("rstd"), py::arg("has_bias"),
+        py::arg("dres") = c10::nullopt, py::arg("fused") = true,
+        py::arg("grid_cap") = 0);
+  m.def("add_layer_norm_fwd", &add_layer_norm_fwd, py::arg("x"),
+        py::arg("residual"), py::arg("w"), py::arg("b") = c10::nullopt,
+        py::arg("eps") = 1e-5);
+  m.def("ln_bwd_grid_cap", &ln_bwd_grid_cap);
+  m.def("ln_fused_ok", &ln_fused_ok);
+  m.def("bias_gelu_bwd_db", &bias_gelu_bwd_db, py::arg("dy"), py::arg("x"),
+        py::arg("bias") = c10::nullopt, py::arg("fused") = true);
+  m.def("bias_gelu_bwd_db_fused", &bias_gelu_bwd_db_fused);
+  m.def("flash_attn_bwd_delta", &flash_attn_bwd_delta);
   m.def("rms_norm_fwd", &rms_norm_fwd);
   m.def("rms_norm_bwd", &rms_norm_bwd);
   m.def("softmax_ce_fwd", &softmax_ce_fwd);
diff --git a/csrc/kernels/api.h b/csrc/kernels/api.h
--- a/csrc/kernels/api.h
+++ b/csrc/kernels/api.h
@@ -18,6 +18,22 @@
                          int64_t d, int dtype, hipStream_t s,
                          float* ws = nullptr);
 
+constexpr int64_t kLnFusedMaxD = 8192;
+constexpr int kLnBwdGridCap = 1024;
+bool ln_fused_ok(int64_t d);
+int ln_bwd_fused_grid(int64_t n, int cap);
+void add_layer_norm_fwd(const void* x, const void* residual, const void* w,
+                        const void* b, void* h, void* y, float* mean,
+                        float* rstd, int64_t n, int64_t d, float eps, int dtype,
+                        hipStream_t s);
+void layer_norm_bwd_fused(const void* dy, const void* x, const void* w,
+                          const float* mean, const float* rstd,
+                          const void* dres, void* dx, float* dw, float* db,
+                          float* ws, int grid, int64_t n, int64_t d, int dtype,
+                          hipStream_t s);
+void ws_reduce(const float* ws, float* out0, float* out1, int parts, int nout,
+               int64_t d, hipStream_t s);
+
 void rms_norm_fwd(const void* x, const void* residual, const void* w, void* y,
                   void* res_out, float* rstd, int64_t n, int64_t d, float eps,
                   int dtype, hipStream_t s);
@@ -40,6 +56,10 @@
                    int64_t d, int dtype, hipStream_t s);
 void bias_gelu_bwd(const void* dy, const void* x, const void* bias, void* dx,
                    int64_t n, int64_t d, int dtype, hipStream_t s);
+int bias_gelu_bwd_db_grid(int64_t n, int64_t d);
+void bias_gelu_bwd_db(const void* dy, const void* x, const void* bias, void* dx,
+                      float* db, float* ws, int grid, int64_t n, int64_t d,
+                      int dtype, hipStream_t s);
 
 void swiglu_fwd(const void* x, void* y, int64_t n, int64_t d, int dtype,
                 hipStream_t s);
@@ -98,6 +118,9 @@
                     const int64_t* os, const int64_t* dqs, const int64_t* dks,
                     const void* mask, const int64_t* ms, float pdrop,
                     uint64_t seed, uint64_t offset, hipStream_t s);
+void flash_attn_bwd_delta(const void* dout, const void* o, float* delta,
+                          int64_t b, int64_t h, int64_t sq, int64_t dh,
+                          const int64_t* dos, const int64_t* os, hipStream_t s);
 
 void dropout_add_fwd(const void* x, const void* residual, void* y,
                      uint8_t* mask, int64_t numel, float p, uint64_t seed,
diff --git a/csrc/kernels/elementwise.hip b/csrc/kernels/elementwise.hip
--- a/csrc/kernels/elementwise.hip
+++ b/csrc/kernels/elementwise.hip
@@ -55,10 +55,15 @@
   return sig * (1.f + x * (1.f - sig));
 }
 
-template <int DT, bool FWD, int W>
+template <int DT, bool FWD, int W, bool BGRAD = false>
 __global__ void bias_gelu_kernel(const void* __restrict__ a, const void* __restrict__ x,
                                  const void* __restrict__ bias, void* __restrict__ out,
-                                 int64_t n, int64_t d) {
+                                 int64_t n, int64_t d, float* __restrict__ ws = nullptr) {
+  float acc[W];
+  if (BGRAD) {
+#pragma unroll
+    for (int k = 0; k < W; ++k) acc[k] = 0.f;
+  }
   int64_t total = n * d;
   int64_t i0 = ((int64_t)blockIdx.x * blockDim.x + threadIdx.x) * W;
   int64_t stride = (int64_t)gridDim.x * blockDim.x * W;
@@ -75,10 +80,16 @@
     for (int k = 0; k < W; ++k) {
       float v = xf[k] + (bias ? bf[k] : 0.f);
       xf[k] = FWD ? gelu_f(v) : af[k] * gelu_grad_f(v);
+      if (BGRAD) acc[k] += (DT == kBF16) ? bf2f(f2bf(xf[k])) : xf[k];
     }
 #pragma unroll
     for (int v8 = 0; v8 < W / 8; ++v8)
       LS8<DT>::store8(out, i + 8 * v8, xf + 8 * v8);
+  }
+  if (BGRAD) {
+#pragma unroll
+    for (int v8 = 0; v8 < W / 8; ++v8)
+      LS8<kF32>::store8(ws, i0 + 8 * v8, acc + 8 * v8);
   }
 }
 
@@ -276,6 +287,37 @@
   }
 }
 
+static int64_t gcd64(int64_t a, int64_t b) { while (b) { int64_t t = a % b; a = b; b = t; } return a; }
+
+int bias_gelu_bwd_db_grid(int64_t n, int64_t d) {
+  if (d % 8 != 0 || n <= 0) return 0;
+  const int W = d % 16 == 0 ? 16 : 8;
+  const int64_t cap = elementwise_grid(1LL << 40);
+  const int64_t g0 = egrid(n * d / (W / 8)).x;
+  const int64_t q = d / gcd64(d, 256 * W);
+  if (q > cap) return 0;
+  int64_t g = (g0 + q - 1) / q * q;
+  if (g > cap) g = cap / q * q;
+  return (int)g;
+}
+
+void bias_gelu_bwd_db(const void* dy, const void* x, const void* bias, void* dx,
+                      float* db, float* ws, int grid, int64_t n, int64_t d,
+                      int dtype, hipStream_t s) {
+  dim3 g((unsigned)grid);
+  if (d % 16 == 0) {
+    EDT(dtype,
+        hipLaunchKernelGGL((bias_gelu_kernel<kBF16, false, 16, true>), g, dim3(256), 0, s, dy, x, bias, dx, n, d, ws),
+        hipLaunchKernelGGL((bias_gelu_kernel<kF32, false, 16, true>), g, dim3(256), 0, s, dy, x, bias, dx, n, d, ws));
+    ws_reduce(ws, db, nullptr, (int)((int64_t)grid * 256 * 16 / d), 1, d, s);
+  } else {
+    EDT(dtype,
+        hipLaunchKernelGGL((bias_gelu_kernel<kBF16, false, 8, true>), g, dim3(256), 0, s, dy, x, bias, dx, n, d, ws),
+        hipLaunchKernelGGL((bias_gelu_kernel<kF32, false, 8, true>), g, dim3(256), 0, s, dy, x, bias, dx, n, d, ws));
+    ws_reduce(ws, db, nullptr, (int)((int64_t)grid * 256 * 8 / d), 1, d, s);
+  }
+}
+
 void swiglu_fwd(const void* x, void* y, int64_t n, int64_t d, int dtype, hipStream_t s) {
   dim3 g = egrid(n * d);
   EDT(dtype,
diff --git a/csrc/kernels/flash_attn.hip b/csrc/kernels/flash_attn.hip
--- a/csrc/kernels/flash_attn.hip
+++ b/csrc/kernels/flash_attn.hip
@@ -231,25 +231,71 @@
                                     long long rows,
                                     long long do_sb, long long do_sh, long long do_ss,
                                     long long o_sb, long long o_sh, long long o_ss) {
-  long long wid = ((long long)blockIdx.x * blockDim.x + threadIdx.x) >> 6;
-  int lane = threadIdx.x & 63;
-  long long nwaves = ((long long)gridDim.x * blockDim.x) >> 6;
-  for (long long r = wid; r < rows; r += nwaves) {
-    int sq = (int)(r % Sq);
-    int h = (int)((r / Sq) % H);
-    int b = (int)(r / ((long long)Sq * H));
-    const long long dob = b * do_sb + h * do_sh + sq * do_ss;
-    const long long ob = b * o_sb + h * o_sh + sq * o_ss;
-    float acc = 0.f;
-    for (int j = lane * 8; j < D; j += 64 * 8) {
-      shortx8 a = *reinterpret_cast<const shortx8*>(dog + dob + j);
-      shortx8 bb = *reinterpret_cast<const shortx8*>(og + ob + j);
-#pragma unroll
-      for (int k = 0; k < 8; ++k) acc += bf2f(a[k]) * bf2f(bb[k]);
-    }
-    acc = wave_reduce(acc, SumOp());
-    if (lane == 0) delta[r] = acc;
-  }
+  constexpr int LPR = D / 8, RPP = 256 / LPR, UNR = 4;
+  const int sub = threadIdx.x % LPR;
+  const int rin = threadIdx.x / LPR;
+  const bool h_fast = do_sh < do_ss;
+  for (long long r0 = (long long)blockIdx.x * (RPP * UNR); r0 < rows;
+       r0 += (long long)gridDim.x * (RPP * UNR)) {
+    shortx8 a[UNR], bb[UNR];
+    long long di[UNR];
+#pragma unroll
+    for (int u = 0; u < UNR; ++u) {
+      const long long r = r0 + u * RPP + rin;
+      di[u] = -1;
+      if (r < rows) {
+        int sq, h, b;
+        if (h_fast) {
+          h = (int)(r % H);
+          sq = (int)((r / H) % Sq);
+        } else {
+          sq = (int)(r % Sq);
+          h = (int)((r / Sq) % H);
+        }
+        b = (int)(r / ((long long)Sq * H));
+        di[u] = ((long long)b * H + h) * Sq + sq;
+        a[u] = *reinterpret_cast<const shortx8*>(
+            dog + b * do_sb + h * do_sh + sq * do_ss + sub * 8);
+        bb[u] = *reinterpret_cast<const shortx8*>(
+            og + b * o_sb + h * o_sh + sq * o_ss + sub * 8);
+      }
+    }
+#pragma unroll
+    for (int u = 0; u < UNR; ++u) {
+      float acc = 0.f;
+      if (di[u] >= 0) {
+#pragma unroll
+        for (int k = 0; k < 8; ++k) acc += bf2f(a[u][k]) * bf2f(bb[u][k]);
+      }
+#pragma unroll
+      for (int off = LPR / 2; off > 0; off >>= 1) acc += __shfl_xor(acc, off, WAVE);
+      if (sub == 0 && di[u] >= 0) delta[di[u]] = acc;
+    }
+  }
+}
+
+static void fa_bwd_delta(const void* dout, const void* o, float* delta,
+                         int64_t bh_h, int64_t sq, long long rows, int64_t dh,
+                         long long do_sb, long long do_sh, long long do_ss,
+                         long long o_sb, long long o_sh, long long o_ss,
+                         hipStream_t s) {
+  const int rows_per_iter = (256 / (int)(dh / 8)) * 4;
+  dim3 dgrid((unsigned)hmin<long long>(2048LL, (rows + rows_per_iter - 1) / rows_per_iter));
+  if (dh == 128)
+    hipLaunchKernelGGL((fa_bwd_delta_kernel<128>), dgrid, dim3(256), 0, s,
+                       (const short*)dout, (const short*)o, delta, (int)bh_h,
+                       (int)sq, rows, do_sb, do_sh, do_ss, o_sb, o_sh, o_ss);
+  else
+    hipLaunchKernelGGL((fa_bwd_delta_kernel<64>), dgrid, dim3(256), 0, s,
+                       (const short*)dout, (const short*)o, delta, (int)bh_h,
+                       (int)sq, rows, do_sb, do_sh, do_ss, o_sb, o_sh, o_ss);
+}
+
+void flash_attn_bwd_delta(const void* dout, const void* o, float* delta,
+                          int64_t b, int64_t h, int64_t sq, int64_t dh,
+                          const int64_t* dos, const int64_t* os, hipStream_t s) {
+  fa_bwd_delta(dout, o, delta, h, sq, b * h * sq, dh, dos[0], dos[1], dos[2],
+               os[0], os[1], os[2], s);
 }
 
 template <int D, bool CAUSAL>
@@ -691,16 +737,8 @@
                     const int64_t* os, const int64_t* dqs, const int64_t* dks,
                     const void* mask, const int64_t* ms, float pdrop,
                     uint64_t seed, uint64_t offset, hipStream_t s) {
-  long long rows = b * h * sq;
-  dim3 dgrid((unsigned)hmin<long long>(2048LL, (rows + 3) / 4));
-  if (dh == 128)
-    hipLaunchKernelGGL((fa_bwd_delta_kernel<128>), dgrid, dim3(256), 0, s,
-                       (const short*)dout, (const short*)o, delta, (int)h,
-                       (int)sq, rows, dos[0], dos[1], dos[2], os[0], os[1], os[2]);
-  else
-    hipLaunchKernelGGL((fa_bwd_delta_kernel<64>), dgrid, dim3(256), 0, s,
-                       (const short*)dout, (const short*)o, delta, (int)h,
-                       (int)sq, rows, dos[0], dos[1], dos[2], os[0], os[1], os[2]);
+  fa_bwd_delta(dout, o, delta, h, sq, b * h * sq, dh, dos[0], dos[1], dos[2],
+               os[0], os[1], os[2], s);
 
   dim3 gkv((unsigned)(b * h), (unsigned)cdiv((int)skv, 128));
   dim3 gq((unsigned)cdiv((int)sq, 128), (unsigned)(b * h));
@@ -740,17 +778,9 @@
                            const int* cu_q, const int* cu_k, const int* qbmap,
                            const int* kvbmap, float pdrop, uint64_t seed,
                            uint64_t offset, hipStream_t s) {
-  long long rows = h * total_q;
-  dim3 dgrid((unsigned)hmin<long long>(2048LL, (rows + 3) / 4));
   const long long ss = h * dh;
-  if (dh == 128)
-    hipLaunchKernelGGL((fa_bwd_delta_kernel<128>), dgrid, dim3(256), 0, s,
-                       (const short*)dout, (const short*)o, delta, (int)h,
-                       (int)total_q, rows, 0, dh, ss, 0, dh, ss);
-  else
-    hipLaunchKernelGGL((fa_bwd_delta_kernel<64>), dgrid, dim3(256), 0, s,
-                       (const short*)dout, (const short*)o, delta, (int)h,
-                       (int)total_q, rows, 0, dh, ss, 0, dh, ss);
+  fa_bwd_delta(dout, o, delta, h, total_q, h * total_q, dh, 0, dh, ss, 0, dh,
+               ss, s);
   flash_attn_varlen_bwd32(dout, q, k, v, lse, delta, dq, dk, dv, h, total_q,
                           total_k, dh, scale, causal, nqblocks, nkvblocks,
                           cu_q, cu_k, qbmap, kvbmap, pdrop, seed, offset, s);
diff --git a/csrc/kernels/norms.hip b/csrc/kernels/norms.hip
--- a/csrc/kernels/norms.hip
+++ b/csrc/kernels/norms.hip
@@ -46,6 +46,57 @@
     ((float*)p)[idx] = f;
   }
 };
+
+__device__ __forceinline__ float pin(float v) {
+  asm("" : "+v"(v));
+  return v;
+}
+
+template <int DT>
+__device__ __forceinline__ float round_t(float v) {
+  if (DT == kBF16) return bf2f(f2bf(v));
+  return pin(v);
+}
+
+__device__ __forceinline__ float row_shift8(const float* f0) {
+#pragma clang fp reassociate(off)
+  float s = ((((((f0[0] + f0[1]) + f0[2]) + f0[3]) + f0[4]) + f0[5]) + f0[6]) + f0[7];
+  return s * 0.125f;
+}
+
+__device__ __forceinline__ void ln_moments(float f, float shift, float& sum,
+                                           float& sumc, float& sumsq) {
+#pragma clang fp reassociate(off)
+  float c = f - shift;
+  sum += f;
+  sumc += c;
+  sumsq += pin(c * c);
+}
+
+__device__ __forceinline__ float ln_y(float f, float mu, float rstd, float w, float b) {
+#pragma clang fp reassociate(off)
+  return __builtin_fmaf(pin(w * rstd), f - mu, b);
+}
+
+__device__ __forceinline__ float ln_xhat(float x, float mu, float rs) {
+  return pin((x - mu) * rs);
+}
+
+__device__ __forceinline__ void ln_bwd_sums(float gy, float w, float xh,
+                                            float& s1, float& s2) {
+#pragma clang fp reassociate(off)
+  float g = pin(gy * w);
+  s1 = __builtin_fmaf(g, xh, s1);
+  s2 += g;
+}
+
+__device__ __forceinline__ float ln_bwd_dx1(float gy, float w, float xh, float c1,
+                                            float c2, float rs) {
+#pragma clang fp reassociate(off)
+  float g = pin(gy * w);
+  float a = pin(g - c2);
+  return rs * __builtin_fmaf(-xh, c1, a);
+}
 
 template <int DT>
 __global__ void ln_fwd_kernel(const void* __restrict__ x, const void* __restrict__ w,
@@ -59,20 +110,14 @@
     {
       float f0[8];
       VIO<DT>::load8(x, base, f0);
-      shift = ((f0[0] + f0[1]) + (f0[2] + f0[3]) + (f0[4] + f0[5]) + (f0[6] + f0[7])) * 0.125f;
+      shift = row_shift8(f0);
     }
     float sum = 0.f, sumc = 0.f, sumsq = 0.f;
     for (int64_t i = threadIdx.x * 8; i < d; i += blockDim.x * 8) {
       float f[8];
       VIO<DT>::load8(x, base + i, f);
 #pragma unroll
-      for (int k = 0; k < 8; ++k) {
-#pragma clang fp reassociate(off)
-        float c = f[k] - shift;
-        sum += f[k];
-        sumc += c;
-        sumsq += c * c;
-      }
+      for (int k = 0; k < 8; ++k) ln_moments(f[k], shift, sum, sumc, sumsq);
     }
     float ts = block_reduce_256(sum, SumOp(), red, 0.f);
     float tsc = block_reduce_256(sumc, SumOp(), red + 4, 0.f);
@@ -89,7 +134,7 @@
       if (b) VIO<DT>::load8(b, i, bf);
 #pragma unroll
       for (int k = 0; k < 8; ++k)
-        f[k] = (f[k] - mu) * rstd * wf[k] + (b ? bf[k] : 0.f);
+        f[k] = ln_y(f[k], mu, rstd, wf[k], b ? bf[k] : 0.f);
       VIO<DT>::store8(y, base + i, f);
     }
     __syncthreads();
@@ -112,28 +157,22 @@
       VIO<DT>::load8(x, base + i, xf);
       VIO<DT>::load8(w, i, wf);
 #pragma unroll
-      for (int k = 0; k < 8; ++k) {
-        float g = gy[k] * wf[k];
-        float xh = (xf[k] - mu) * rs;
-        s1 += g * xh;
-        s2 += g;
-      }
+      for (int k = 0; k < 8; ++k)
+        ln_bwd_sums(gy[k], wf[k], ln_xhat(xf[k], mu, rs), s1, s2);
     }
     float t1 = block_reduce_256(s1, SumOp(), red, 0.f);
     __syncthreads();
     float t2 = block_reduce_256(s2, SumOp(), red + 4, 0.f);
     const float inv_d = 1.f / d;
+    const float c1 = pin(t1 * inv_d), c2 = pin(t2 * inv_d);
     for (int64_t i = threadIdx.x * 8; i < d; i += blockDim.x * 8) {
       float gy[8], xf[8], wf[8];
       VIO<DT>::load8(dy, base + i, gy);
       VIO<DT>::load8(x, base + i, xf);
       VIO<DT>::load8(w, i, wf);
 #pragma unroll
-      for (int k = 0; k < 8; ++k) {
-        float g = gy[k] * wf[k];
-        float xh = (xf[k] - mu) * rs;
-        gy[k] = rs * (g - t2 * inv_d - xh * t1 * inv_d);
-      }
+      for (int k = 0; k < 8; ++k)
+        gy[k] = ln_bwd_dx1(gy[k], wf[k], ln_xhat(xf[k], mu, rs), c1, c2, rs);
       VIO<DT>::store8(dx, base + i, gy);
     }
     __syncthreads();
@@ -193,6 +232,155 @@
     }
 }
 
+template <int DT, int NS>
+__global__ __launch_bounds__(256) void add_ln_fwd_kernel(
+    const void* __restrict__ x, const void* __restrict__ res,
+    const void* __restrict__ w, const void* __restrict__ b,
+    void* __restrict__ h, void* __restrict__ y, float* __restrict__ mean_out,
+    float* __restrict__ rstd_out, int64_t n, int64_t d, float eps) {
+  __shared__ float red[12];
+  const int64_t c0 = threadIdx.x * 8;
+  for (int64_t row = blockIdx.x; row < n; row += gridDim.x) {
+    const int64_t base = row * d;
+    float shift;
+    {
+      float f0[8], r0[8];
+      VIO<DT>::load8(x, base, f0);
+      VIO<DT>::load8(res, base, r0);
+#pragma unroll
+      for (int k = 0; k < 8; ++k) f0[k] = round_t<DT>(f0[k] + r0[k]);
+      shift = row_shift8(f0);
+    }
+    float hf[NS][8];
+    float sum = 0.f, sumc = 0.f, sumsq = 0.f;
+#pragma unroll
+    for (int j = 0; j < NS; ++j) {
+      const int64_t c = c0 + (int64_t)j * 2048;
+      if (c < d) {
+        float rf[8];
+        VIO<DT>::load8(x, base + c, hf[j]);
+        VIO<DT>::load8(res, base + c, rf);
+#pragma unroll
+        for (int k = 0; k < 8; ++k) hf[j][k] = round_t<DT>(hf[j][k] + rf[k]);
+        VIO<DT>::store8(h, base + c, hf[j]);
+#pragma unroll
+        for (int k = 0; k < 8; ++k) ln_moments(hf[j][k], shift, sum, sumc, sumsq);
+      }
+    }
+    float ts = block_reduce_256(sum, SumOp(), red, 0.f);
+    float tsc = block_reduce_256(sumc, SumOp(), red + 4, 0.f);
+    float tss = block_reduce_256(sumsq, SumOp(), red + 8, 0.f);
+    float mu = ts / d;
+    float dmu = tsc / d;
+    float var = fmaxf(tss / d - dmu * dmu, 0.f);
+    float rstd = rsqrtf(var + eps);
+    if (threadIdx.x == 0) { mean_out[row] = mu; rstd_out[row] = rstd; }
+#pragma unroll
+    for (int j = 0; j < NS; ++j) {
+      const int64_t c = c0 + (int64_t)j * 2048;
+      if (c < d) {
+        float wf[8], bf[8], f[8];
+        VIO<DT>::load8(w, c, wf);
+        if (b) VIO<DT>::load8(b, c, bf);
+#pragma unroll
+        for (int k = 0; k < 8; ++k)
+          f[k] = ln_y(hf[j][k], mu, rstd, wf[k], b ? bf[k] : 0.f);
+        VIO<DT>::store8(y, base + c, f);
+      }
+    }
+    __syncthreads();
+  }
+}
+
+template <int DT, int NS, bool HAS_DRES>
+__global__ __launch_bounds__(256) void ln_bwd_fused_kernel(
+    const void* __restrict__ dy, const void* __restrict__ x,
+    const void* __restrict__ w, const float* __restrict__ mean,
+    const float* __restrict__ rstd, const void* __restrict__ dres,
+    void* __restrict__ dx, float* __restrict__ ws, int64_t n, int64_t d) {
+  __shared__ float red[8];
+  const int64_t c0 = threadIdx.x * 8;
+  float wf[NS][8], aw[NS][8], ab[NS][8];
+#pragma unroll
+  for (int j = 0; j < NS; ++j) {
+    const int64_t c = c0 + (int64_t)j * 2048;
+#pragma unroll
+    for (int k = 0; k < 8; ++k) { wf[j][k] = 0.f; aw[j][k] = 0.f; ab[j][k] = 0.f; }
+    if (c < d) VIO<DT>::load8(w, c, wf[j]);
+  }
+  for (int64_t row = blockIdx.x; row < n; row += gridDim.x) {
+    const int64_t base = row * d;
+    const float mu = mean[row], rs = rstd[row];
+    float gy[NS][8], xh[NS][8];
+    float s1 = 0.f, s2 = 0.f;
+#pragma unroll
+    for (int j = 0; j < NS; ++j) {
+      const int64_t c = c0 + (int64_t)j * 2048;
+      if (c < d) {
+        VIO<DT>::load8(dy, base + c, gy[j]);
+        VIO<DT>::load8(x, base + c, xh[j]);
+#pragma unroll
+        for (int k = 0; k < 8; ++k) {
+          xh[j][k] = ln_xhat(xh[j][k], mu, rs);
+          ln_bwd_sums(gy[j][k], wf[j][k], xh[j][k], s1, s2);
+        }
+      }
+    }
+    float t1 = block_reduce_256(s1, SumOp(), red, 0.f);
+    __syncthreads();
+    float t2 = block_reduce_256(s2, SumOp(), red + 4, 0.f);
+    const float inv_d = 1.f / d;
+    const float c1 = pin(t1 * inv_d), c2 = pin(t2 * inv_d);
+#pragma unroll
+    for (int j = 0; j < NS; ++j) {
+      const int64_t c = c0 + (int64_t)j * 2048;
+      if (c < d) {
+        float o[8], rf[8];
+        if (HAS_DRES) VIO<DT>::load8(dres, base + c, rf);
+#pragma unroll
+        for (int k = 0; k < 8; ++k) {
+          o[k] = ln_bwd_dx1(gy[j][k], wf[j][k], xh[j][k], c1, c2, rs);
+          if (HAS_DRES) o[k] = round_t<DT>(o[k]) + rf[k];
+          aw[j][k] += gy[j][k] * xh[j][k];
+          ab[j][k] += gy[j][k];
+        }
+        VIO<DT>::store8(dx, base + c, o);
+      }
+    }
+    __syncthreads();
+  }
+  float* wrow = ws + (int64_t)blockIdx.x * 2 * d;
+#pragma unroll
+  for (int j = 0; j < NS; ++j) {
+    const int64_t c = c0 + (int64_t)j * 2048;
+    if (c < d) {
+      VIO<kF32>::store8(wrow, c, aw[j]);
+      VIO<kF32>::store8(wrow, d + c, ab[j]);
+    }
+  }
+}
+
+__global__ __launch_bounds__(1024) void ws_reduce_kernel(
+    const float* __restrict__ ws, float* __restrict__ out0,
+    float* __restrict__ out1, int parts, int nout, int64_t d) {
+  __shared__ float lds[16][64];
+  const int lane = threadIdx.x & 63, wv = threadIdx.x >> 6;
+  const int64_t c = (int64_t)blockIdx.x * 64 + lane;
+  const int o = blockIdx.y;
+  float acc = 0.f;
+  if (c < d)
+    for (int p = wv; p < parts; p += 16)
+      acc += ws[((int64_t)p * nout + o) * d + c];
+  lds[wv][lane] = acc;
+  __syncthreads();
+  if (wv == 0 && c < d) {
+    float s = 0.f;
+#pragma unroll
+    for (int i = 0; i < 16; ++i) s += lds[i][lane];
+    (o == 0 ? out0 : out1)[c] = s;
+  }
+}
+
 __global__ void dwdb_reduce_kernel(const float* __restrict__ ws, float* __restrict__ dw,
                                    float* __restrict__ db, int chunks, int64_t d) {
   int64_t c = (int64_t)blockIdx.x * blockDim.x + threadIdx.x;
@@ -325,6 +513,54 @@
                        dim3(256), 0, s, ws, dw, db, chunks, d);
 }
 
+#define NS_SWITCH(d, ...)                                            \
+  switch (cdiv((int)(d), 2048)) {                                    \
+    case 1: { constexpr int NS = 1; __VA_ARGS__; break; }            \
+    case 2: { constexpr int NS = 2; __VA_ARGS__; break; }            \
+    case 3: { constexpr int NS = 3; __VA_ARGS__; break; }            \
+    default: { constexpr int NS = 4; __VA_ARGS__; break; }           \
+  }
+
+bool ln_fused_ok(int64_t d) { return d % 8 == 0 && d <= kLnFusedMaxD; }
+
+int ln_bwd_fused_grid(int64_t n, int cap) {
+  if (cap <= 0) cap = kLnBwdGridCap;
+  return (int)hmin<int64_t>(n, cap);
+}
+
+void ws_reduce(const float* ws, float* out0, float* out1, int parts, int nout,
+               int64_t d, hipStream_t s) {
+  dim3 grid((unsigned)((d + 63) / 64), out1 ? 2 : 1);
+  hipLaunchKernelGGL(ws_reduce_kernel, grid, dim3(1024), 0, s, ws, out0, out1,
+                     parts, nout, d);
+}
+
+void add_layer_norm_fwd(const void* x, const void* residual, const void* w,
+                        const void* b, void* h, void* y, float* mean,
+                        float* rstd, int64_t n, int64_t d, float eps, int dtype,
+                        hipStream_t s) {
+  DT_SWITCH(dtype, NS_SWITCH(d, hipLaunchKernelGGL(
+      (add_ln_fwd_kernel<DT, NS>), dim3(norm_grid(n)), dim3(256), 0, s, x,
+      residual, w, b, h, y, mean, rstd, n, d, eps)));
+}
+
+void layer_norm_bwd_fused(const void* dy, const void* x, const void* w,
+                          const float* mean, const float* rstd,
+                          const void* dres, void* dx, float* dw, float* db,
+                          float* ws, int grid, int64_t n, int64_t d, int dtype,
+                          hipStream_t s) {
+  if (dres) {
+    DT_SWITCH(dtype, NS_SWITCH(d, hipLaunchKernelGGL(
+        (ln_bwd_fused_kernel<DT, NS, true>), dim3(grid), dim3(256), 0, s, dy, x,
+        w, mean, rstd, dres, dx, ws, n, d)));
+  } else {
+    DT_SWITCH(dtype, NS_SWITCH(d, hipLaunchKernelGGL(
+        (ln_bwd_fused_kernel<DT, NS, false>), dim3(grid), dim3(256), 0, s, dy, x,
+        w, mean, rstd, dres, dx, ws, n, d)));
+  }
+  ws_reduce(ws, dw, db, grid, 2, d, s);
+}
+
 void rms_norm_fwd(const void* x, const void* residual, const void* w, void* y,
                   void* res_out, float* rstd, int64_t n, int64_t d, float eps,
                   int dtype, hipStream_t s) {
diff --git a/paddle_amd/models/gpt.py b/paddle_amd/models/gpt.py
--- a/paddle_amd/models/gpt.py
+++ b/paddle_amd/models/gpt.py
@@ -114,9 +114,33 @@
         self.mlp = GPTMLP(cfg)
         self.dropout = cfg.hidden_dropout
 
-    def forward(self, x):
-        h = hot.dropout_add(self.attn(self.ln1(x)), x, self.dropout, self.training)
-        return hot.dropout_add(self.mlp(self.ln2(h)), h, self.dropout, self.training)
+    def _add_ln(self, x, residual, ln):
+        return hot.add_layer_norm(x, residual, ln.weight, ln.bias, ln._epsilon,
+                                  self.dropout, self.training)
+
+    def forward(self, x, residual=None, defer_add=False):
+        if residual is None:
+            y = self.ln1(x)
+        else:
+            x, y = self._add_ln(x, residual, self.ln1)
+        h, y = self._add_ln(self.attn(y), x, self.ln2)
+        m = self.mlp(y)
+        if defer_add:
+            return m, h
+        return hot.dropout_add(m, h, self.dropout, self.training)
+
+
+class GPTFinalNorm(nn.LayerNorm):
+
+    def __init__(self, cfg: GPTConfig):
+        super().__init__(cfg.hidden_size)
+        self.dropout = cfg.hidden_dropout
+
+    def forward(self, x, residual=None):
+        if residual is None:
+            return super().forward(x)
+        return hot.add_layer_norm(x, residual, self.weight, self.bias,
+                                  self._epsilon, self.dropout, self.training)[1]
 
 
 class GPTModel(nn.Layer):
@@ -125,19 +149,19 @@
         self.cfg = cfg
         self.embeddings = GPTEmbeddings(cfg)
         self.layers = nn.LayerList([GPTDecoderLayer(cfg) for _ in range(cfg.num_layers)])
-        self.final_norm = nn.LayerNorm(cfg.hidden_size)
+        self.final_norm = GPTFinalNorm(cfg)
 
     def forward(self, input_ids, position_ids=None):
         x = self.embeddings(input_ids, position_ids)
-        use_rc = self.cfg.use_recompute and self.training
-        if use_rc:
+        if self.cfg.use_recompute and self.training:
             from ..distributed.fleet.recompute import recompute
+            for layer in self.layers:
+                x = recompute(layer, x) if x.requires_grad else layer(x)
+            return self.final_norm(x)
+        res = None
         for layer in self.layers:
-            if use_rc and x.requires_grad:
-                x = recompute(layer, x)
-            else:
-                x = layer(x)
-        return self.final_norm(x)
+            x, res = layer(x, res, defer_add=True)
+        return self.final_norm(x, res)
 
 
 class GPTForPretraining(nn.Layer):
diff --git a/paddle_amd/ops/functional.py b/paddle_amd/ops/functional.py
--- a/paddle_amd/ops/functional.py
+++ b/paddle_amd/ops/functional.py
@@ -148,6 +148,79 @@
     return _LayerNorm.apply(x, weight, bias, epsilon)
 
 
+def _add_ln_native_ok(x, residual, w, b=None, p=0.0, training=True):
+    if p != 0 and training:
+        return False
+    if not (isinstance(x, torch.Tensor) and isinstance(residual, torch.Tensor)):
+        return False
+    return _kernel_ok(x, last_mult=8, same=(residual,), vecs=(w, b),
+                      contiguous=(x, residual))
+
+
+class _AddLayerNorm(torch.autograd.Function):
+
+    @staticmethod
+    def forward(ctx, x, residual, w, b, eps):
+        ctx.set_materialize_grads(False)
+        ctx.native = _ext.use_native(x)
+        ctx.w_dtype = w.dtype
+        ctx.b_dtype = b.dtype if b is not None else w.dtype
+        ctx.has_bias = b is not None
+        if ctx.native:
+            C = _ext.get_ext()
+            w = _as_dtype(w, x.dtype)
+            h, y, mean, rstd = C.add_layer_norm_fwd(x, residual, w,
+                                                    _as_dtype(b, x.dtype), eps)
+        else:
+            h = x.clone() + residual
+            hf = h.float()
+            mean = hf.mean(-1).reshape(-1)
+            var = hf.var(-1, unbiased=False).reshape(-1)
+            rstd = torch.rsqrt(var + eps)
+            xhat = (hf - mean.view(*h.shape[:-1], 1)) * rstd.view(*h.shape[:-1], 1)
+            y = xhat * w.float() + (b.float() if b is not None else 0.0)
+            y = y.to(h.dtype)
+        ctx.save_for_backward(h, w, mean, rstd)
+        return h, y
+
+    @staticmethod
+    def backward(ctx, dh, dy):
+        if dy is None:
+            return dh, dh, None, None, None
+        h, w, mean, rstd = ctx.saved_tensors
+        if ctx.native:
+            C = _ext.get_ext()
+            dres = None if dh is None else dh.to(h.dtype).contiguous()
+            dx, dw, db = C.layer_norm_bwd(dy.to(h.dtype).contiguous(), h, w,
+                                          mean, rstd, ctx.has_bias, dres)
+            dw, db = dw.to(ctx.w_dtype), db.to(ctx.b_dtype)
+        else:
+            d = h.shape[-1]
+            hf = h.float()
+            dyf = dy.float()
+            mu = mean.view(*h.shape[:-1], 1)
+            rs = rstd.view(*h.shape[:-1], 1)
+            xhat = (hf - mu) * rs
+            g = dyf * w.float()
+            s1 = (g * xhat).mean(-1, keepdim=True)
+            s2 = g.mean(-1, keepdim=True)
+            dx = (rs * (g - s2 - xhat * s1)).to(h.dtype)
+            if dh is not None:
+                dx = dx + dh
+            dw = (dyf * xhat).reshape(-1, d).sum(0).to(w.dtype)
+            db = dyf.reshape(-1, d).sum(0).to(ctx.b_dtype)
+        return dx, dx, dw, (db if ctx.has_bias else None), None
+
+
+def add_layer_norm(x, residual, weight, bias=None, epsilon=1e-5, p=0.0,
+                   training=True):
+    if (not _tracing() and _add_ln_native_ok(x, residual, weight, bias, p, training)
+            and _ext.use_native(x)):
+        return _AddLayerNorm.apply(x, residual, weight, bias, epsilon)
+    h = dropout_add(x, residual, p, training)
+    return h, layer_norm(h, weight, bias, epsilon)
+
+
 class _RMSNorm(torch.autograd.Function):
     @staticmethod
     def forward(ctx, x, w, eps):
@@ -299,6 +372,9 @@
     return loss
 
 
+_BIAS_GELU_DB_FUSE_MIN = 1 << 20
+
+
 class _BiasGelu(torch.autograd.Function):
     @staticmethod
     def forward(ctx, x, bias):
@@ -317,9 +393,14 @@
         b = bias if ctx.has_bias else None
         if ctx.native:
             C = _ext.get_ext()
-            dx = C.bias_gelu_bwd(dy.to(x.dtype).contiguous(), x.contiguous(),
-                                 _as_dtype(b, x.dtype))
-            db = C.colsum(dx).to(b.dtype) if ctx.has_bias else None
+            if ctx.has_bias and x.numel() >= _BIAS_GELU_DB_FUSE_MIN:
+                dx, db = C.bias_gelu_bwd_db(dy.to(x.dtype).contiguous(),
+                                            x.contiguous(), _as_dtype(b, x.dtype))
+                db = db.to(b.dtype)
+            else:
+                dx = C.bias_gelu_bwd(dy.to(x.dtype).contiguous(), x.contiguous(),
+                                     _as_dtype(b, x.dtype))
+                db = C.colsum(dx).to(b.dtype) if ctx.has_bias else None
         else:
             v = x.float() + (b.float() if b is not None else 0.0)
             cdf = 0.5 * (1.0 + torch.erf(v * 0.7071067811865476))
```

Result: faster. 24860 tokens/s, median of 6 (+3.4%).
